# lionl1106/Clip-Neural-image-conpression

Hardware: AMD Instinct MI355X
Metric: images/sec @256px 50-step DDIM, batch=8/GPU (higher is better)
Workload: dtype bf16; 1 GPU; 256px base=128 ch_mult=(1, 2, 2) 50-step DDIM (eta=0), batch=8/GPU, key-seeded synthetic weights (out.* x0.1), synthetic z / x_T; global_batch=8, parallelism=dp1 (independent batches, no collective in the loop), graph=hipGraph, one replay per step, steps_in_flight=1

## Files before the change

clip-neural-image-conpression_amd/csrc/ccn_api.hip:

```cpp
#include "../../include/ccn_hip.h"
#include "ccn_internal.h"
#include "ccn_arch.h"

#include <algorithm>
#include <cmath>
#include <cstdio>
#include <cstdlib>
#include <cstring>
#include <map>
#include <memory>
#include <string>
#include <vector>

using namespace ccn;

namespace {

thread_local std::string g_err;
int fail(int code, const std::string& msg) { g_err = msg; return code; }
#define HIPCHK(expr)                                                                                     \
    do {                                                                                                 \
        hipError_t e_ = (expr);                                                                          \
        if (e_ != hipSuccess)                                                                            \
            return fail(CCN_EHIP, std::string(#expr) + ": " + hipGetErrorString(e_));                    \
    } while (0)

}
extern "C" void ccn_internal_set_error(const char* msg) { g_err = msg ? msg : ""; }
namespace {

inline size_t align_up(size_t v, size_t a) { return (v + a - 1) / a * a; }
inline int ceil_div(int a, int b) { return (a + b - 1) / b; }

uint16_t f2bf_host(float f)
{
    uint32_t u;
    std::memcpy(&u, &f, 4);
    if ((u & 0x7fffffffu) > 0x7f800000u) return (uint16_t)((u >> 16) | 0x40);
    u += 0x7fffu + ((u >> 16) & 1u);
    return (uint16_t)(u >> 16);
}

struct ConvW : ArchConv {
    ConvW() {}
    ConvW(const ArchConv& c) : ArchConv(c) {}
    int Cin_pad = 0, Cout_pad = 0, BN = 0, ntaps_w = 0;
    void* w = nullptr;
    void* wfrag = nullptr;
    float* bias = nullptr;
    bool split = false;
    float inv_scale = 1.f;
    int nphase = 1;
    void* w_ph[7] = {};
    void* wfrag_ph[7] = {};
};
struct NormW { int C = 0; float* gamma = nullptr; float* beta = nullptr; };
struct ResW { NormW n1, n2; };

constexpr size_t kNone = ~(size_t)0;
struct TensorRef {
    std::string name;
    size_t off = kNone;
    int C = 0, H = 0, W = 0;
    size_t part = kNone;
    int n_sp = 0, n_nt = 0, bn = 0;
    bool pr = false;
    int prod = -1;
};

struct StepCtx {
    int step = 0;
    const float* x_in = nullptr;
    float* x_state = nullptr;
    float* eps_out = nullptr;
    int do_ddim = 0;
    float c[4] = {0, 0, 0, 0};
    const float* noise = nullptr;
    float sigma = 0.f;
    float* x0_hist = nullptr;
    float c4 = 0.f;
};

const char* kFamilies[] = {"conv3x3_s1_igemm", "conv3x3_s2_igemm", "convT4x4_s2_igemm", "stem_conv_igemm",
                           "head_conv_ddim", "gn_finalize", "conditioning", "gn_silu_prepass"};
enum { F_C3S1 = 0, F_C3S2, F_CT4, F_STEM, F_HEAD, F_GNF, F_COND, F_LAYOUT, F_COUNT };

enum Op { OP_CONV = 0, OP_HEAD2, OP_GN_FINALIZE, OP_GN_ACT, OP_GN_ACT_FUSED };
struct Launch {
    Op op = OP_CONV; int family = 0; double flops = 0, bytes = 0;
    int conv = -1;
    bool frag = false;
    int film_off = -1;
    ConvArgs a{};
    size_t in = kNone, out = kNone, res = kNone, part = kNone, kpart = kNone, kflag = kNone, gs_part = kNone, gn_ab = kNone,
           fin_ab = kNone, fin_counter = kNone, scratch = kNone;
    int C = 0, HW = 0, G = 0, cpg = 0, n_sp = 0, n_nt = 0, bn = 0;
    double count = 0; const float* gamma = nullptr; const float* beta = nullptr;
};

constexpr int kMaxNorms = 128;

struct RouteRec {
    std::string name;
    int kind = 0;
    const char* kernel = "";
    int th = 0, ksplit = 1, n_nt = 1;
    const char* gn = "none";
    bool film = false, res = false;
    int ops = -1;
};

struct Region { std::string name; size_t off, bytes; };
struct ShapePlan {
    int B = 0, H = 0, W = 0, steps = 0;
    std::vector<Region> regions; size_t total = 0;
    std::vector<std::pair<size_t, size_t>> zero;
    size_t ts_dev = 0, temb = 0, t1 = 0, tp = 0, zp = 0, film = 0, zbuf = 0, xstate = 0;
    int film_stride = 0;
    size_t counters = 0;
    int n_counters = 0, max_counters = 0;
    std::vector<Launch> ops;
    std::map<std::string, TensorRef> named;
    std::vector<RouteRec> routes;
};

struct GraphEntry {
    int steps = 0;
    std::vector<int32_t> ts;
    std::vector<float> coef;
    std::vector<float> sigma;
    const float* noise = nullptr;
    bool guided = false;
    float w = 0.f;
    const float* eps = nullptr;
    std::vector<float> c4;
    const float* hist = nullptr;
    hipGraph_t graph = nullptr;
    hipGraphExec_t exec = nullptr;
    void destroy() { if (exec) (void)hipGraphExecDestroy(exec); if (graph) (void)hipGraphDestroy(graph); }
};

constexpr size_t kMaxGraphsPerBinding = 4;
struct Binding {
    const ShapePlan* plan = nullptr;
    char* ws = nullptr;
    std::vector<int32_t> ts_keep;
    std::vector<GraphEntry> graphs;
    ~Binding() { for (auto& g : graphs) g.destroy(); }
};

}

struct ccn_handle_s {
    ccn_config_t cfg{};
    bool split = false;
    int elem = 4;
    Arch arch;
    std::map<std::string, std::vector<float>> host;
    bool committed = false;
    std::vector<void*> dev_allocs;
    std::vector<ConvW> convs;
    std::vector<ResW> res;
    NormW out_norm;
    float *tp0_w = nullptr, *tp0_b = nullptr, *tp2_w = nullptr, *tp2_b = nullptr, *zp_w = nullptr, *zp_b = nullptr;
    float *film_w = nullptr, *film_b = nullptr;
    float* head_w_f32 = nullptr;
    int G = 8;
    int weight_rounding = CCN_ROUND_DIFFUSED_PHASES;
    int nphase = 1;
    std::vector<std::unique_ptr<ShapePlan>> shape_plans;
    std::vector<std::unique_ptr<Binding>> bindings;
    hipStream_t cap_stream = nullptr;
    unsigned* err_host = nullptr;
    unsigned* err_dev = nullptr;
    bool profiling = false;
    std::vector<hipEvent_t> ev_pool;
    struct Rec { int family; double flops, bytes; int e0, e1; };
    std::vector<Rec> recs;
    size_t ev_used = 0;
    std::vector<std::string> fam_names;
};

namespace {

int upload(ccn_handle_s* h, const void* src, size_t bytes, void** dst)
{
    void* p = nullptr;
    HIPCHK(hipMalloc(&p, bytes ? bytes : 4));
    h->dev_allocs.push_back(p);
    if (bytes) HIPCHK(hipMemcpy(p, src, bytes, hipMemcpyHostToDevice));
    *dst = p;
    return CCN_OK;
}
const std::vector<float>& host_param(const ccn_handle_s* h, int i) { return h->host.at(h->arch.params[i].name); }
int upload_f32(ccn_handle_s* h, int param, float** dst)
{
    const auto& v = host_param(h, param);
    return upload(h, v.data(), v.size() * 4, (void**)dst);
}

float bf16_value(float f)
{
    const uint32_t u = (uint32_t)f2bf_host(f) << 16;
    float r;
    std::memcpy(&r, &u, 4);
    return r;
}

void diffuse_round_conv(float* w, int O, int I, int taps)
{
    for (int o = 0; o < O; ++o) {
        double err = 0.0;
        float* row = w + (size_t)o * I * taps;
        for (size_t k = 0; k < (size_t)I * taps; ++k) {
            const double t = (double)row[k] + err;
            const float r = bf16_value((float)t);
            err = t - (double)r;
            row[k] = r;
        }
    }
}
void diffuse_round_convT(float* w, int I, int O)
{
    static const int kk2[2][2] = {{1, 3}, {0, 2}};
    for (int o = 0; o < O; ++o)
        for (int par = 0; par < 4; ++par) {
            double err = 0.0;
            for (int i = 0; i < I; ++i)
                for (int t = 0; t < 4; ++t) {
                    const int wt = kk2[par >> 1][t >> 1] * 4 + kk2[par & 1][t & 1];
                    float& v = w[((size_t)i * O + o) * 16 + wt];
                    const double tt = (double)v + err;
                    const float r = bf16_value((float)tt);
                    err = tt - (double)r;
                    v = r;
                }
        }
}

int phases_for(const ccn_handle_s* h)
{
    size_t total = 0;
    for (auto& p : h->arch.params) if (p.shape.size() == 4) total += p.numel();
    return total > (size_t)100000000 ? 4 : 8;
}
void round_version(const float* w, size_t n, bool convT, int O, int I, int taps, int k, double* sum, float* out)
{
    for (size_t i = 0; i < n; ++i) out[i] = (float)((double)(k + 1) * (double)w[i] - sum[i]);
    if (convT) diffuse_round_convT(out, I, O); else diffuse_round_conv(out, O, I, taps);
    for (size_t i = 0; i < n; ++i) sum[i] += (double)out[i];
}

}
extern "C" int ccn_internal_round_weights(const float* w, int O, int I, int taps, int convT, int phases, float* out)
{
    if (!w || !out || O <= 0 || I <= 0 || phases < 1 || phases > 8 || (convT && taps != 16)) return 1;
    const size_t n = (size_t)O * I * taps;
    std::vector<double> sum(n, 0.0);
    for (int k = 0; k < phases; ++k) round_version(w, n, convT != 0, O, I, taps, k, sum.data(), out + (size_t)k * n);
    return 0;
}
extern "C" int ccn_internal_split_weights(const float* w, size_t n, float* scale, uint16_t* hi, uint16_t* lo)
{
    if ((!w && n) || !scale || ((!hi || !lo) && n)) return 1;
    float mx = 0.f;
    for (size_t i = 0; i < n; ++i) { const float v = std::fabs(w[i]); if (v > mx) mx = v; }
    int e = 0;
    float s = 1.f;
    if (mx > 0.f && std::isfinite(mx)) { (void)std::frexp(mx, &e); s = std::ldexp(1.f, std::min(14 - e, 126)); }
    *scale = s;
    for (size_t i = 0; i < n; ++i) {
        const float ws = w[i] * s;
        const _Float16 h = (_Float16)ws;
        const _Float16 l = (_Float16)(ws - (float)h);
        std::memcpy(hi + i, &h, 2);
        std::memcpy(lo + i, &l, 2);
    }
    return 0;
}
namespace {

template <typename F>
int pack_and_upload(ccn_handle_s* h, ConvW& cw, int taps, F&& at, void** dw)
{
    cw.BN = conv_bn_for(cw.Cout, cw.kind);
    cw.Cout_pad = (int)align_up(cw.Cout, cw.BN);
    cw.ntaps_w = taps;
    const size_t n = (size_t)taps * cw.Cout_pad * cw.Cin_pad;
    if (h->cfg.dtype == CCN_DTYPE_BF16) {
        std::vector<uint16_t> buf(n, 0);
        for (int t = 0; t < taps; ++t)
            for (int o = 0; o < cw.Cout; ++o)
                for (int i = 0; i < cw.Cin_pad; ++i) buf[((size_t)t * cw.Cout_pad + o) * cw.Cin_pad + i] = f2bf_host(at(t, o, i));
        return upload(h, buf.data(), n * 2, dw);
    }
    std::vector<float> buf(n, 0.f);
    for (int t = 0; t < taps; ++t)
        for (int o = 0; o < cw.Cout; ++o)
            for (int i = 0; i < cw.Cin_pad; ++i) buf[((size_t)t * cw.Cout_pad + o) * cw.Cin_pad + i] = at(t, o, i);
    cw.split = h->split && conv_ws_enabled() && conv_ws_supported(cw.kind, cw.BN);
    cw.inv_scale = 1.f;
    if (cw.split) {
        std::vector<uint16_t> hi(n), lo(n), rows(2 * n);
        float s = 1.f;
        if (ccn_internal_split_weights(buf.data(), n, &s, hi.data(), lo.data())) return fail(CCN_EINVAL, "weight split failed");
        cw.inv_scale = 1.f / s;
        for (size_t i = 0; i < n; ++i) {
            const size_t row = i / 32, c = i % 32;
            rows[row * 64 + c] = hi[i];
            rows[row * 64 + 32 + c] = lo[i];
        }
        return upload(h, rows.data(), n * 4, dw);
    }
    return upload(h, buf.data(), n * 4, dw);
}

int pack_conv3(ccn_handle_s* h, ConvW& cw, const float* w, void** dw, void** dfrag)
{
    const int cke = conv_cin_chunk(h->cfg.dtype);
    cw.Cin_pad = (int)align_up(cw.Cin, cke);
    const int I = cw.Cin;
    int rc = pack_and_upload(h, cw, 9, [&](int t, int o, int i) { return i < I ? w[((size_t)o * I + i) * 9 + t] : 0.f; }, dw);
    if (rc) return rc;
    if (cw.kind == KIND_C3S2 && cw.BN == 128 && h->cfg.dtype == CCN_DTYPE_BF16) {
        const int nch = cw.Cin_pad / cke, n32 = cw.Cout_pad / 32, O = cw.Cout;
        std::vector<uint16_t> fr((size_t)nch * 5 * n32 * 2 * 4 * 64 * 8, 0);
        for (int o = 0; o < O; ++o)
            for (int i = 0; i < I; ++i)
                for (int ps = 0; ps < 10; ++ps) {
                    const int tp = prs2_tap(ps >> 1, ps & 1);
                    if (tp >= 0) fr[prs2_frag_index(ps >> 1, ps & 1, o, i, cw.Cout_pad)] = f2bf_host(w[((size_t)o * I + i) * 9 + tp]);
                }
        return upload(h, fr.data(), fr.size() * 2, dfrag);
    }
    if (cw.kind == KIND_C3S1 && cw.BN == 128 && h->cfg.dtype == CCN_DTYPE_BF16) {
        const int nch = cw.Cin_pad / cke, n32 = cw.Cout_pad / 32, O = cw.Cout;
        std::vector<uint16_t> fr((size_t)nch * n32 * 36 * 64 * 8, 0);
        for (int o = 0; o < O; ++o)
            for (int i = 0; i < I; ++i)
                for (int t = 0; t < 9; ++t) fr[pr3_frag_index(o, i, t, cw.Cout_pad)] = f2bf_host(w[((size_t)o * I + i) * 9 + t]);
        return upload(h, fr.data(), fr.size() * 2, dfrag);
    }
    return CCN_OK;
}
int pack_convT(ccn_handle_s* h, ConvW& cw, const float* w, void** dw, void** dfrag)
{
    const int cke = conv_cin_chunk(h->cfg.dtype);
    cw.Cin_pad = (int)align_up(cw.Cin, cke);
    const int I = cw.Cin, O = cw.Cout;
    int rc = pack_and_upload(h, cw, 16, [&](int t, int o, int i) { return i < I ? w[((size_t)i * O + o) * 16 + t] : 0.f; }, dw);
    if (rc) return rc;
    if (cw.BN == 128 && h->cfg.dtype == CCN_DTYPE_BF16) {
        const int nch = cw.Cin_pad / cke, n32 = cw.Cout_pad / 32;
        std::vector<uint16_t> fr((size_t)4 * nch * n32 * 4 * 4 * 64 * 8, 0);
        for (int o = 0; o < O; ++o)
            for (int i = 0; i < I; ++i)
                for (int pt = 0; pt < 16; ++pt)
                    fr[prct_frag_index(pt >> 2, pt & 3, o, i, cw.Cout_pad, nch)] = f2bf_host(w[((size_t)i * O + o) * 16 + prct_tap(pt >> 2, pt & 3)]);
        return upload(h, fr.data(), fr.size() * 2, dfrag);
    }
    return CCN_OK;
}
int pack_stem(ccn_handle_s* h, ConvW& cw, const float* w, const float* bias, void** dw, void** dfrag)
{
    const int cke = conv_cin_chunk(h->cfg.dtype);
    cw.Cin_pad = cke;
    const int K = cw.Cin * 9;
    int rc = pack_and_upload(h, cw, 1, [&](int, int o, int k) { return k < K ? w[(size_t)o * K + k] : 0.f; }, dw);
    if (rc) return rc;
    if (stem2_supported(h->cfg.dtype, cw.Cin, cw.Cout, h->G)) {
        const int nt = cw.Cout / 32;
        std::vector<uint16_t> fr((size_t)nt * 2 * 64 * 8, 0);
        for (int j = 0; j < nt; ++j)
            for (int s = 0; s < 2; ++s)
                for (int ln = 0; ln < 64; ++ln)
                    for (int e = 0; e < 8; ++e) {
                        const int o = j * 32 + (ln & 31), k = 16 * s + 8 * (ln >> 5) + e;
                        const float v = k < K ? w[(size_t)o * K + k] : (k == K ? bias[o] : 0.f);
                        fr[(((size_t)j * 2 + s) * 64 + ln) * 8 + e] = f2bf_host(v);
                    }
        return upload(h, fr.data(), fr.size() * 2, dfrag);
    }
    return CCN_OK;
}
int pack_conv(ccn_handle_s* h, ConvW& cw, const float* w, const float* bias, void** dw, void** dfrag)
{
    if (cw.kind == KIND_STEM) return pack_stem(h, cw, w, bias, dw, dfrag);
    return cw.kind == KIND_CT4 ? pack_convT(h, cw, w, dw, dfrag) : pack_conv3(h, cw, w, dw, dfrag);
}

struct ConvOpts {
    int film_off = -1;
    const TensorRef* res = nullptr;
    bool want_part = false;
    size_t gn_ab = kNone;
    const NormW* in_norm = nullptr;
    const char* pre_pass = nullptr;
};

struct PlanBuilder {
    ccn_handle_s* h; ShapePlan& pl; const int B;
    size_t off = 0;
    PlanBuilder(ccn_handle_s* h_, ShapePlan& p) : h(h_), pl(p), B(p.B) {}

    size_t take(const std::string& name, size_t bytes)
    {
        pl.regions.push_back({name, align_up(off, 256), bytes});
        off = pl.regions.back().off + bytes;
        return off - bytes;
    }
    TensorRef new_tensor(const std::string& name, int C, int H, int W)
    {
        TensorRef t; t.name = name; t.C = C; t.H = H; t.W = W;
        t.off = take(name, (size_t)B * H * W * C * h->elem);
        return t;
    }
    int groups_for(int C) const { return C < h->G ? C : h->G; }
    void take_counters(int n) { pl.max_counters = n; pl.counters = take("counters", (size_t)n * B * 4); pl.zero.push_back({pl.counters, (size_t)n * B * 4}); }

    ConvRoute route(const ConvW& cw, int Hin, int Win, bool gn_ab, bool res, bool film) const
    {
        static const ConvPolicy policy{true, 128, false, !diag_env("CCN_NO_SPLITK"), diag_env("CCN_SPLITK_S1") != nullptr, true};
        return conv_route({h->cfg.dtype, cw.kind, false, cw.BN, cw.Cin, cw.Cin_pad, cw.Cout, cw.Cout_pad, B, Hin, Win, h->G, cw.wfrag != nullptr,
                           gn_ab, res, film}, policy);
    }

    void conv(int ci, const TensorRef& in, TensorRef& out, const ConvOpts& o)
    {
        const ConvW& cw = h->convs[ci];
        size_t gn_ab = o.gn_ab;
        const ConvRoute r = route(cw, in.H, in.W, gn_ab != kNone, o.res != nullptr, o.film_off >= 0);
        const ConvGeom& g = r.g;
        Launch L;
        static_assert(F_C3S1 == KIND_C3S1 && F_C3S2 == KIND_C3S2 && F_CT4 == KIND_CT4 && F_STEM == KIND_STEM && F_HEAD == KIND_HEAD, "family = kind");
        L.family = cw.kind; L.conv = ci; L.film_off = o.film_off; L.frag = r.uses_frag() && cw.wfrag;
        L.in = in.off; L.out = out.off; L.res = o.res ? o.res->off : kNone;
        ConvArgs& a = L.a;
        r.fill(a);
        a.bias = cw.bias; a.ops = cw.split ? 1 : 0; a.wscale_inv = cw.inv_scale;
        RouteRec rec;
        if (h->split) rec.ops = a.ops;
        rec.name = out.name; rec.kind = cw.kind; rec.th = r.th; rec.ksplit = r.ksplit; rec.n_nt = r.n_nt;
        rec.film = o.film_off >= 0; rec.res = o.res != nullptr;
        rec.gn = gn_ab != kNone ? "prologue" : "none";
        static const bool no_instat = diag_env("CCN_NO_INSTAT") != nullptr;
        if (o.in_norm) {
            const int G_in = groups_for(cw.Cin), cpg_in = cw.Cin / G_in;
            if (r.gs_ok && !no_instat && in.C == cw.Cin && conv_in_kernel_stats(h->cfg.dtype, in.C, G_in, in.n_sp, in.bn)) {
                L.gs_part = in.part; a.gs_gamma = o.in_norm->gamma; a.gs_beta = o.in_norm->beta;
                a.gs_inv_count = 1.0 / ((double)cpg_in * in.H * in.W);
                a.gs_nsp = in.n_sp; a.gs_nnt = in.n_nt; a.gs_bn = in.bn; a.gs_cpg = cpg_in;
                rec.gn = "instat";
            } else { gn_ab = gn(in, *o.in_norm); rec.gn = "prologue"; }
        }
        if (o.pre_pass) rec.gn = o.pre_pass;
        L.gn_ab = gn_ab;
        rec.kernel = conv_kernel_name(conv_kernel_for(cw.kind, cw.BN, a));
        pl.routes.push_back(rec);
        if (r.ksplit == 2) {
            L.kpart = take(out.name + ".kpart", (size_t)B * g.Hout * g.Wout * cw.Cout * h->elem);
            const size_t fbytes = (size_t)B * r.fin_blocks * 4 * sizeof(unsigned);
            L.kflag = take(out.name + ".kflag", fbytes);
            pl.zero.push_back({L.kflag, fbytes});
        }
        a.film_bstride = pl.film_stride; a.err = h->err_dev;
        if (o.want_part) {
            out.part = take(out.name + ".part", (size_t)B * a.G * a.nslot * sizeof(float2));
            out.n_sp = r.part_nsp; out.n_nt = r.part_nnt; out.bn = r.part_bn;
            if (r.pr || r.stem2) out.pr = true;
            out.prod = (int)pl.ops.size();
        }
        L.part = out.part;
        const double macs = (double)B * g.Hout * g.Wout * cw.Cout * (double)(cw.kind == KIND_CT4 ? 4 : 9) * cw.Cin;
        L.flops = 2.0 * macs;
        L.bytes = ((double)B * in.H * in.W * cw.Cin + (double)B * g.Hout * g.Wout * cw.Cout + (o.res ? (double)B * g.Hout * g.Wout * cw.Cout : 0.0)
                   + (double)(cw.kind == KIND_CT4 ? 16 : 9) * cw.Cin * cw.Cout) * h->elem;
        if (cw.kind == KIND_STEM) L.bytes = (double)B * in.H * in.W * cw.Cin * 4 + ((double)B * g.Hout * g.Wout * cw.Cout + 9.0 * cw.Cin * cw.Cout) * h->elem;
        if (cw.kind == KIND_HEAD) L.bytes = ((double)B * in.H * in.W * cw.Cin + 9.0 * cw.Cin * cw.Cout) * h->elem + 3.0 * (double)B * g.Hout * g.Wout * cw.Cout * 4;
        pl.ops.push_back(L);
    }
    Launch norm_launch(Op op, int family, double bytes, const TensorRef& t, const NormW& n) const
    {
        Launch L;
        L.op = op; L.family = family; L.bytes = bytes;
        L.C = t.C; L.HW = t.H * t.W; L.G = groups_for(t.C); L.cpg = t.C / L.G; L.count = (double)L.cpg * t.H * t.W;
        L.in = t.off; L.part = t.part; L.n_sp = t.n_sp; L.n_nt = t.n_nt; L.bn = t.bn; L.gamma = n.gamma; L.beta = n.beta;
        return L;
    }

    size_t gn(const TensorRef& t, const NormW& n)
    {
        const size_t ab = take(t.name + ".ab", (size_t)B * t.C * sizeof(float2));
        Launch L = norm_launch(OP_GN_FINALIZE, F_GNF, (double)B * groups_for(t.C) * t.n_sp * t.n_nt * 8.0 + (double)B * t.C * 8.0, t, n);
        static const bool fuse = diag_env("CCN_FUSED_FINALIZE") != nullptr;
        if (fuse && t.prod >= 0 && !t.pr && pl.n_counters < pl.max_counters) {
            Launch& p = pl.ops[t.prod];
            p.fin_counter = pl.counters + (size_t)pl.n_counters * B * sizeof(unsigned);
            pl.n_counters++;
            p.a.fin_gamma = n.gamma; p.a.fin_beta = n.beta; p.fin_ab = ab; p.a.fin_count = L.count;
            return ab;
        }
        L.gn_ab = ab;
        pl.ops.push_back(L);
        return ab;
    }

    TensorRef preact(const TensorRef& t, const NormW& n, size_t ab)
    {
        TensorRef o = new_tensor(t.name + ".act", t.C, t.H, t.W);
        Launch L = norm_launch(ab == kNone ? OP_GN_ACT_FUSED : OP_GN_ACT, F_LAYOUT, 2.0 * B * t.H * t.W * (double)t.C * h->elem, t, n);
        L.out = o.off; L.gn_ab = ab;
        pl.ops.push_back(L);
        return o;
    }

    TensorRef resblock(int ri, const TensorRef& x, bool out_feeds_gn, int film_off)
    {
        const ArchRes& r = h->arch.res[ri];
        const ConvW& c1 = h->convs[r.c1];
        const NormW &n1 = h->res[ri].n1, &n2 = h->res[ri].n2;
        static const bool preact_pr = diag_env("CCN_PREACT_PR") != nullptr;
        const bool pre = conv_wants_preact(c1.kind, c1.BN, c1.Cout_pad / c1.BN) && r.C / (h->elem == 2 ? 8 : 4) <= 256 &&
                         (preact_pr || c1.Cout_pad / c1.BN >= 6 || !route(c1, x.H, x.W, false, false, false).pr);
        static const bool fuse_act = !diag_env("CCN_NO_FUSED_GNACT");
        const bool f1 = pre && fuse_act && x.n_sp > 0, f2 = pre && fuse_act;
        ConvOpts o1, o2;
        o1.film_off = film_off; o1.want_part = true; o1.pre_pass = f1 ? "preact_fused" : (pre ? "preact" : nullptr);
        o2.res = &x; o2.want_part = out_feeds_gn; o2.pre_pass = f2 ? "preact_fused" : (pre ? "preact" : nullptr);
        TensorRef y = new_tensor(r.prefix + ".film", r.C, x.H, x.W);
        if (pre) conv(r.c1, preact(x, n1, f1 ? kNone : gn(x, n1)), y, o1);
        else { o1.in_norm = &n1; conv(r.c1, x, y, o1); }
        pl.named[y.name] = y;
        TensorRef o = new_tensor(r.prefix, r.C, x.H, x.W);
        if (pre) conv(r.c2, preact(y, n2, f2 ? kNone : gn(y, n2)), o, o2);
        else { o2.in_norm = &n2; conv(r.c2, y, o, o2); }
        pl.named[o.name] = o;
        return o;
    }
};

int build_plan(ccn_handle_s* h, ShapePlan& pl)
{
    const ccn_config_t& c = h->cfg;
    PlanBuilder pb(h, pl);
    const int B = pl.B, H = pl.H, W = pl.W, S = pl.steps;
    const int TR = B > S ? B : S, FR = S * B > B ? S * B : B;
    pl.film_stride = h->arch.F;
    pl.ts_dev = pb.take("ts", (size_t)S * 4);
    pl.temb = pb.take("temb", (size_t)TR * c.time_dim * 4);
    pl.t1 = pb.take("t1", (size_t)TR * c.time_dim * 4 * 4);
    pl.tp = pb.take("tp", (size_t)TR * c.time_dim * 4);
    pl.zp = pb.take("zp", (size_t)B * c.time_dim * 4);
    pl.film = pb.take("film", (size_t)FR * h->arch.F * 4);
    pl.zbuf = pb.take("z", (size_t)B * c.z_dim * 4);
    pl.xstate = pb.take("x_state", (size_t)B * c.img_ch * H * W * 4);
    pb.take_counters(kMaxNorms);

    TensorRef x, img; img.C = c.img_ch; img.H = H; img.W = W;
    std::vector<TensorRef> skips;
    const std::vector<ArchLayer>& layers = h->arch.layers; const size_t nl = layers.size();
    for (size_t li = 0; li < nl; ++li) {
        const ArchLayer& L = layers[li];
        ConvOpts o;
        o.want_part = li + 1 < nl && (layers[li + 1].type == L_RES || layers[li + 1].type == L_HEAD);
        if (L.type == L_RES) { x = pb.resblock(L.idx, x, o.want_part, h->arch.res[L.idx].film_off); continue; }
        const ConvW& cw = h->convs[L.idx];
        if (L.type == L_HEAD) {
            o.gn_ab = pb.gn(x, h->out_norm); o.want_part = false;
            static const bool no_head2 = diag_env("CCN_NO_HEAD2") != nullptr;
            if (no_head2 || !head2_supported(c.dtype, cw.Cin, cw.Cout, h->G)) {
                TensorRef none; none.name = L.name;
                pb.conv(L.idx, x, none, o);
                continue;
            }
            Launch Lh;
            Lh.op = OP_HEAD2; Lh.family = F_HEAD; Lh.conv = L.idx; Lh.in = x.off; Lh.gn_ab = o.gn_ab;
            ConvArgs& a = Lh.a;
            a.bias = cw.bias; a.B = B; a.Hin = H; a.Win = W; a.Cin = cw.Cin; a.Cout = cw.Cout; a.Hout = H; a.Wout = W;
            Lh.scratch = pb.take(L.name + ".scratch", head2_scratch_bytes(B, x.C));
            const double macs = (double)B * H * W * cw.Cout * 9.0 * cw.Cin;
            Lh.flops = 2.0 * macs;
            Lh.bytes = ((double)B * H * W * x.C + 9.0 * x.C * cw.Cout) * h->elem + 3.0 * (double)B * H * W * cw.Cout * 4;
            pl.ops.push_back(Lh);
            RouteRec rec;
            rec.name = L.name; rec.kind = KIND_HEAD; rec.kernel = "head2"; rec.th = 8; rec.gn = "weights";
            if (h->split) rec.ops = 0;
            pl.routes.push_back(rec);
            continue;
        }
        TensorRef sk;
        if (L.type == L_DOWN) skips.push_back(x);
        if (L.type == L_UP) { sk = skips.back(); skips.pop_back(); o.res = &sk; }
        const TensorRef& in = L.type == L_STEM ? img : x;
        const int up = L.type == L_UP ? 2 : 1, down = L.type == L_DOWN ? 2 : 1;
        TensorRef out = pb.new_tensor(L.name, cw.Cout, in.H * up / down, in.W * up / down);
        if (o.res && (sk.C != cw.Cout || sk.H != out.H || sk.W != out.W)) return fail(CCN_EINVAL, "skip shape mismatch");
        pb.conv(L.idx, in, out, o);
        pl.named[L.name] = x = out;
    }
    pl.total = align_up(pb.off, 256);
    return CCN_OK;
}

hipError_t launch(const ccn_handle_s* h, const ShapePlan& pl, const Launch& L, char* ws, hipStream_t s, const StepCtx& c)
{
    auto at = [ws](size_t o) -> char* { return o == kNone ? nullptr : ws + o; };
    const int dtype = h->cfg.dtype;
    switch (L.op) {
        case OP_GN_FINALIZE:
            return launch_gn_finalize((const float2*)at(L.part), pl.B, L.G, L.n_sp, L.n_nt, L.bn, L.cpg, L.C, L.count, L.gamma, L.beta, 1e-5f,
                                      (float2*)at(L.gn_ab), s);
        case OP_GN_ACT: return launch_gn_act(dtype, at(L.in), (const float2*)at(L.gn_ab), at(L.out), pl.B, L.HW, L.C, s);
        case OP_GN_ACT_FUSED:
            return launch_gn_act_fused(dtype, at(L.in), at(L.out), pl.B, L.HW, L.C, (const float2*)at(L.part), L.G, L.n_sp, L.n_nt, L.bn, L.cpg,
                                       L.count, L.gamma, L.beta, 1e-5f, s);
        default: break;
    }
    const ConvW& cw = h->convs[L.conv];
    ConvArgs k = L.a;
    k.in = cw.kind == KIND_STEM ? (const void*)c.x_in : at(L.in);
    if (cw.kind == KIND_HEAD) {
        k.x_state = c.x_state; k.eps_out = c.eps_out; k.do_ddim = c.do_ddim;
        k.c0 = c.c[0]; k.c1 = c.c[1]; k.c2 = c.c[2]; k.c3 = c.c[3]; k.noise = c.noise; k.sigma = c.sigma;
        k.x0_hist = c.x0_hist; k.c4 = c.c4;
    }
    if (L.op == OP_HEAD2) return launch_head2(k, (const float2*)at(L.gn_ab), h->head_w_f32, at(L.scratch), c.step, s);
    const int v = c.step % cw.nphase;
    k.w = v ? cw.w_ph[v - 1] : cw.w;
    k.wfrag = !L.frag ? nullptr : (v ? cw.wfrag_ph[v - 1] : cw.wfrag);
    k.out = at(L.out); k.res = at(L.res); k.part = (float2*)at(L.part); k.gn_ab = (const float2*)at(L.gn_ab);
    k.gs_part = (const float2*)at(L.gs_part); k.kpart = at(L.kpart); k.kflag = (unsigned*)at(L.kflag);
    k.fin_ab = (float2*)at(L.fin_ab); k.fin_counter = (unsigned*)at(L.fin_counter);
    if (L.film_off >= 0) k.film = (const float*)at(pl.film) + (size_t)c.step * pl.B * k.film_bstride + L.film_off;
    return launch_conv(dtype, cw.kind, cw.BN, k, s);
}

int check_shape(const ccn_handle_s* h, int B, int H, int W, int steps)
{
    if (B <= 0 || H <= 0 || W <= 0 || steps <= 0) return fail(CCN_EINVAL, "B, H, W, steps must be positive");
    const int div = 1 << h->cfg.n_mult;
    if (H % div || W % div) return fail(CCN_EINVAL, "H and W must be divisible by 2^len(ch_mult)");
    return CCN_OK;
}

void drop_bindings(ccn_handle_s* h, size_t keep_newest)
{
    if (h->bindings.size() <= keep_newest) return;
    (void)hipDeviceSynchronize();
    while (h->bindings.size() > keep_newest) h->bindings.erase(h->bindings.begin());
}

int shape_plan(ccn_handle_s* h, int B, int H, int W, int steps, const ShapePlan** out)
{
    if (int rc = check_shape(h, B, H, W, steps)) return rc;
    for (auto& p : h->shape_plans)
        if (p->B == B && p->H == H && p->W == W && p->steps == steps) { *out = p.get(); return CCN_OK; }
    std::unique_ptr<ShapePlan> p(new ShapePlan);
    p->B = B; p->H = H; p->W = W; p->steps = steps;
    if (int rc = build_plan(h, *p)) return rc;
    if (h->shape_plans.size() >= 64) { drop_bindings(h, 0); h->shape_plans.clear(); }
    *out = p.get();
    h->shape_plans.push_back(std::move(p));
    return CCN_OK;
}

int get_binding(ccn_handle_s* h, int B, int H, int W, int steps, void* ws, size_t ws_bytes, Binding** out)
{
    const ShapePlan* pl = nullptr;
    if (int rc = shape_plan(h, B, H, W, steps, &pl)) return rc;
    if (!ws || ((uintptr_t)ws & 255)) return fail(CCN_EWORKSPACE, "workspace must be non-null and 256-byte aligned");
    if (ws_bytes < pl->total) return fail(CCN_EWORKSPACE, "workspace too small: need " + std::to_string(pl->total));
    for (size_t i = 0; i < h->bindings.size(); ++i) {
        Binding* b = h->bindings[i].get();
        if (b->plan == pl && b->ws == ws) {
            std::rotate(h->bindings.begin() + (long)i, h->bindings.begin() + (long)i + 1, h->bindings.end());
            *out = b;
            return CCN_OK;
        }
    }
    std::unique_ptr<Binding> b(new Binding);
    b->plan = pl; b->ws = (char*)ws;
    for (auto& z : pl->zero) HIPCHK(hipMemset(b->ws + z.first, 0, z.second));
    if (h->bindings.size() >= 8) drop_bindings(h, 7);
    *out = b.get();
    h->bindings.push_back(std::move(b));
    return CCN_OK;
}

}
int ccn_release_workspace(ccn_handle_t h, void* workspace_dev)
{
    if (!h) return fail(CCN_EINVAL, "null handle");
    auto lives_there = [&](const std::unique_ptr<Binding>& b) { return b->ws == workspace_dev; };
    if (std::none_of(h->bindings.begin(), h->bindings.end(), lives_there)) return CCN_OK;
    HIPCHK(hipDeviceSynchronize());
    h->bindings.erase(std::remove_if(h->bindings.begin(), h->bindings.end(), lives_there), h->bindings.end());
    return CCN_OK;
}
namespace {

template <typename F>
int timed(ccn_handle_s* h, int family, double flops, double bytes, hipStream_t s, F&& go)
{
    if (!h->profiling) { HIPCHK(go()); return CCN_OK; }
    for (hipEvent_t e; h->ev_pool.size() < h->ev_used + 2; h->ev_pool.push_back(e)) HIPCHK(hipEventCreate(&e));
    const int e0 = (int)h->ev_used, e1 = e0 + 1;
    h->ev_used += 2;
    HIPCHK(hipEventRecord(h->ev_pool[e0], s));
    HIPCHK(go());
    HIPCHK(hipEventRecord(h->ev_pool[e1], s));
    h->recs.push_back({family, flops, bytes, e0, e1});
    return CCN_OK;
}

int run_ops(ccn_handle_s* h, const Binding* b, hipStream_t s, const StepCtx& c)
{
    for (const Launch& L : b->plan->ops) {
        if (int rc = timed(h, L.family, L.flops, L.bytes, s, [&] { return launch(h, *b->plan, L, b->ws, s, c); })) return rc;
    }
    return CCN_OK;
}

int run_conditioning(ccn_handle_s* h, const Binding* b, hipStream_t s, const int64_t* t_i64, int TR, int FR, int a_div)
{
    const ccn_config_t& c = h->cfg; const ShapePlan& p = *b->plan;
    const int td = c.time_dim, B = p.B, F = h->arch.F;
    auto f32 = [b](size_t off) { return (float*)(b->ws + off); };
    float *temb = f32(p.temb), *t1 = f32(p.t1), *tp = f32(p.tp), *zp = f32(p.zp);
    int rc;
    if ((rc = timed(h, F_COND, 0, 0, s, [&] {
            return t_i64 ? launch_temb_i64(t_i64, temb, TR, td, s) : launch_temb_i32((const int32_t*)(b->ws + p.ts_dev), temb, TR, td, s); }))) return rc;
    if ((rc = timed(h, F_COND, 2.0 * TR * td * 4.0 * td, 0, s, [&] { return launch_linear(temb, nullptr, 1, TR, h->tp0_w, h->tp0_b, t1, TR, td, 4 * td, 1, s); }))) return rc;
    if ((rc = timed(h, F_COND, 2.0 * TR * td * 4.0 * td, 0, s, [&] { return launch_linear(t1, nullptr, 1, TR, h->tp2_w, h->tp2_b, tp, TR, 4 * td, td, 0, s); }))) return rc;
    if ((rc = timed(h, F_COND, 2.0 * B * c.z_dim * td, 0, s, [&] { return launch_linear(f32(p.zbuf), nullptr, 1, B, h->zp_w, h->zp_b, zp, B, c.z_dim, td, 1, s); }))) return rc;
    return timed(h, F_COND, 2.0 * FR * td * (double)F, 0, s, [&] { return launch_linear(tp, zp, a_div, B, h->film_w, h->film_b, f32(p.film), FR, td, F, 0, s); });
}

struct Guide { const float* z_null; float w; float* eps; };
struct MultiStep { const float* c4; float* hist; };

int run_steps(ccn_handle_s* h, const Binding* b, hipStream_t s, int steps, const float* coef, const float* sigma = nullptr, const float* noise = nullptr,
              const Guide* gd = nullptr, const MultiStep* ms = nullptr)
{
    const ShapePlan& p = *b->plan;
    const size_t img = (size_t)(gd ? p.B / 2 : p.B) * h->cfg.img_ch * p.H * p.W;
    float* xstate = (float*)(b->ws + p.xstate);
    for (int i = 0; i < steps; ++i) {
        const bool noisy = sigma && noise && sigma[i] > 0.f;
        StepCtx c;
        c.step = i; c.x_in = xstate;
        if (gd) { c.x_state = nullptr; c.eps_out = gd->eps; c.do_ddim = 0; }
        else {
            c.x_state = xstate; c.eps_out = nullptr; c.do_ddim = 1;
            for (int k = 0; k < 4; ++k) c.c[k] = coef[i * 4 + k];
            if (noisy) { c.noise = noise + (size_t)i * img; c.sigma = sigma[i]; }
            if (ms) { c.x0_hist = ms->hist; c.c4 = ms->c4[i]; }
        }
        if (int rc = run_ops(h, b, s, c)) return rc;
        if (gd && ms) {
            const float* cf = coef + i * 4;
            const float c4 = ms->c4[i];
            if (int rc = timed(h, F_HEAD, 0, (double)img * 4 * (c4 != 0.f ? 7 : 6), s, [&] {
                    return launch_cfg_ms_step(xstate, xstate + img, ms->hist, gd->eps, gd->eps + img, gd->w, cf[0], cf[1], cf[2], cf[3], c4,
                                              (int64_t)img, s); })) return rc;
        } else if (gd) {
            const float* cf = coef + i * 4;
            const float* nz = noisy ? noise + (size_t)i * img : nullptr;
            if (int rc = timed(h, F_HEAD, 0, (double)img * 4 * (nz ? 6 : 5), s, [&] {
                    return launch_cfg_ddim_step(xstate, xstate + img, gd->eps, gd->eps + img, nz, gd->w, cf[0], cf[1], cf[2], cf[3],
                                                noisy ? sigma[i] : 0.f, (int64_t)img, s); })) return rc;
        }
    }
    return CCN_OK;
}

int check_device_errors(ccn_handle_s* h)
{
    if (!h->err_host) return CCN_OK;
    const unsigned e = __atomic_exchange_n(h->err_host, 0u, __ATOMIC_RELAXED);
    if (e & 1u)
        return fail(CCN_EHIP, "device-side hand-off timeout: a split-K partial tile never arrived; the results of the launches enqueued "
                              "since the last successful check are invalid");
    if (e & 2u)
        return fail(CCN_EHIP, "split-K partners ran on different XCDs (the hand-off took the agent-scope path: results are valid, but the "
                              "placement assumption of launch_conv_pr does not hold on this device / partition mode)");
    if (e & 4u)
        return fail(CCN_EHIP, "f16x3: an activation left the fp16 operand range (|x| >= 65520) and was saturated; the results of the "
                              "launches enqueued since the last successful check are not fp32-grade: use dtype fp32 for this model");
    if (e) return fail(CCN_EHIP, "device-side error word " + std::to_string(e));
    return CCN_OK;
}

int copy_report(const std::string& text, char* buf, size_t cap)
{
    if (buf && cap) {
        const size_t n = std::min(text.size(), cap - 1);
        std::memcpy(buf, text.data(), n);
        buf[n] = 0;
    }
    return (int)text.size();
}

std::string routes_text(const ShapePlan& pl)
{
    static const char* kinds[] = {"C3S1", "C3S2", "CT4", "STEM", "HEAD"};
    std::string text;
    for (const RouteRec& r : pl.routes) {
        char line[256];
        std::snprintf(line, sizeof(line), "%s %s %s th=%d ksplit=%d n_nt=%d gn=%s film=%d res=%d", r.name.c_str(), kinds[r.kind], r.kernel,
                      r.th, r.ksplit, r.n_nt, r.gn, r.film ? 1 : 0, r.res ? 1 : 0);
        text += std::string(line) + (r.ops < 0 ? "" : r.ops ? " ops=f16x3" : " ops=f32") + "\n";
    }
    return text;
}

int check_ready(ccn_handle_s* h)
{
    if (!h) return fail(CCN_EINVAL, "null handle");
    if (!h->committed) return fail(CCN_ESTATE, "ccn_commit_params has not succeeded on this handle");
    return check_device_errors(h);
}

}

extern "C" {

const char* ccn_last_error(void) { return g_err.c_str(); }
#ifdef CCN_DIAG
const char* ccn_version(void) { return "ccn_hip 0.3 (gfx950, diagnostics build)"; }
#else
const char* ccn_version(void) { return "ccn_hip 0.3 (gfx950)"; }
#endif

int ccn_create(const ccn_config_t* cfg, ccn_handle_t* out)
{
    if (!cfg || !out) return fail(CCN_EINVAL, "null argument");
    if (cfg->n_mult < 1 || cfg->n_mult > CCN_MAX_MULT) return fail(CCN_EINVAL, "n_mult out of range");
    if (cfg->dtype != CCN_DTYPE_F32 && cfg->dtype != CCN_DTYPE_BF16 && cfg->dtype != CCN_DTYPE_F16X3) return fail(CCN_EINVAL, "unknown dtype");
    if (cfg->base <= 0 || cfg->base % 8) return fail(CCN_EINVAL, "base must be a positive multiple of 8");
    if (cfg->img_ch < 1 || cfg->img_ch * 9 > 32) return fail(CCN_EINVAL, "img_ch must be 1..3");
    if (cfg->time_dim <= 0 || cfg->z_dim <= 0 || cfg->groups <= 0) return fail(CCN_EINVAL, "bad dims");
    int ch = cfg->base;
    for (int i = 0; i < cfg->n_mult; ++i) {
        if (cfg->ch_mult[i] < 1) return fail(CCN_EINVAL, "ch_mult entries must be >= 1");
        if ((long)ch * cfg->ch_mult[i] > (1 << 16)) return fail(CCN_EINVAL, "channel width (running product of ch_mult, models/unet.py:64) above 65536");
        ch *= cfg->ch_mult[i];
    }
    int ndev = 0;
    HIPCHK(hipGetDeviceCount(&ndev));
    if (ndev <= 0) return fail(CCN_EHIP, "no HIP device");
    std::unique_ptr<ccn_handle_s> h(new ccn_handle_s);
    h->cfg = *cfg;
    h->split = cfg->dtype == CCN_DTYPE_F16X3;
    if (h->split) h->cfg.dtype = CCN_DTYPE_F32;
    h->elem = cfg->dtype == CCN_DTYPE_BF16 ? 2 : 4;
    h->G = cfg->groups;
    h->arch = build_arch(h->cfg);
    h->convs.assign(h->arch.convs.begin(), h->arch.convs.end());
    h->res.resize(h->arch.res.size());
    for (auto& r : h->arch.res)
        if (r.C % (r.C < h->G ? r.C : h->G)) return fail(CCN_EINVAL, "channel count not divisible by GroupNorm groups");
    HIPCHK(conv_prepare());
    HIPCHK(hipStreamCreateWithFlags(&h->cap_stream, hipStreamNonBlocking));
    HIPCHK(hipHostMalloc((void**)&h->err_host, 64, hipHostMallocMapped));
    *h->err_host = 0u;
    HIPCHK(hipHostGetDevicePointer((void**)&h->err_dev, h->err_host, 0));
    for (int i = 0; i < F_COUNT; ++i) h->fam_names.push_back(kFamilies[i]);
    *out = h.release();
    return CCN_OK;
}

int ccn_destroy(ccn_handle_t h)
{
    if (!h) return CCN_OK;
    (void)hipDeviceSynchronize();
    h->bindings.clear();
    for (void* p : h->dev_allocs) (void)hipFree(p);
    for (auto e : h->ev_pool) (void)hipEventDestroy(e);
    if (h->cap_stream) (void)hipStreamDestroy(h->cap_stream);
    if (h->err_host) (void)hipHostFree(h->err_host);
    delete h;
    return CCN_OK;
}

int ccn_num_params(ccn_handle_t h, int32_t* n)
{
    if (!h || !n) return fail(CCN_EINVAL, "null argument");
    *n = (int32_t)h->arch.params.size();
    return CCN_OK;
}

int ccn_param_info(ccn_handle_t h, int32_t i, const char** name, int64_t shape[4], int32_t* ndim)
{
    if (!h || !name || !shape || !ndim) return fail(CCN_EINVAL, "null argument");
    if (i < 0 || i >= (int32_t)h->arch.params.size()) return fail(CCN_EINVAL, "parameter index out of range");
    const ArchParam& p = h->arch.params[i];
    *name = p.name.c_str();
    *ndim = (int32_t)p.shape.size();
    for (size_t k = 0; k < 4; ++k) shape[k] = k < p.shape.size() ? p.shape[k] : 1;
    return CCN_OK;
}

int ccn_load_param(ccn_handle_t h, const char* name, const float* data, const int64_t* shape, int32_t ndim)
{
    if (!h || !name || !data || !shape) return fail(CCN_EINVAL, "null argument");
    const ArchParam* pi = nullptr;
    for (auto& p : h->arch.params) if (p.name == name) { pi = &p; break; }
    if (!pi) return fail(CCN_EWEIGHTS, std::string("Unexpected key in state_dict: ") + name);
    if ((size_t)ndim != pi->shape.size()) return fail(CCN_EWEIGHTS, std::string("size mismatch for ") + name);
    for (int k = 0; k < ndim; ++k)
        if (shape[k] != pi->shape[k]) return fail(CCN_EWEIGHTS, std::string("size mismatch for ") + name);
    std::vector<float> buf(pi->numel());
    hipPointerAttribute_t attr;
    const hipError_t pe = hipPointerGetAttributes(&attr, data);
    if (pe == hipSuccess && attr.type == hipMemoryTypeDevice) {
        HIPCHK(hipMemcpy(buf.data(), data, buf.size() * 4, hipMemcpyDeviceToHost));
    } else {
        (void)hipGetLastError();
        std::memcpy(buf.data(), data, buf.size() * 4);
    }
    h->host[name] = std::move(buf);
    h->committed = false;
    return CCN_OK;
}

int ccn_set_weight_rounding(ccn_handle_t h, int32_t mode)
{
    if (!h) return fail(CCN_EINVAL, "null handle");
    if (mode != CCN_ROUND_NEAREST && mode != CCN_ROUND_DIFFUSED && mode != CCN_ROUND_DIFFUSED_PHASES) return fail(CCN_EINVAL, "unknown weight rounding mode");
    h->weight_rounding = mode;
    return CCN_OK;
}

int ccn_commit_params(ccn_handle_t h)
{
    if (!h) return fail(CCN_EINVAL, "null handle");
    const Arch& a = h->arch;
    std::string missing;
    for (auto& p : a.params)
        if (!h->host.count(p.name)) missing += (missing.empty() ? "" : ", ") + p.name;
    if (!missing.empty()) return fail(CCN_EWEIGHTS, "Missing key(s) in state_dict: " + missing);
    drop_bindings(h, 0);
    h->shape_plans.clear();
    for (void* p : h->dev_allocs) (void)hipFree(p);
    h->dev_allocs.clear();
    const ccn_config_t& c = h->cfg;
    int rc;
    const bool diffuse = c.dtype == CCN_DTYPE_BF16 && h->weight_rounding != CCN_ROUND_NEAREST;
    h->nphase = diffuse && h->weight_rounding == CCN_ROUND_DIFFUSED_PHASES ? phases_for(h) : 1;
    for (size_t ci = 0; ci < a.convs.size(); ++ci) {
        ConvW& cw = h->convs[ci] = ConvW(a.convs[ci]);
        const std::vector<float>&w = host_param(h, cw.pw), &b = host_param(h, cw.pb);
        if ((rc = upload_f32(h, cw.pb, &cw.bias))) return rc;
        const bool dif = diffuse && cw.kind != KIND_HEAD;
        cw.nphase = dif ? h->nphase : 1;
        std::vector<double> sum(dif ? w.size() : 0, 0.0);
        std::vector<float> wk(dif ? w.size() : 0);
        for (int k = 0; k < cw.nphase; ++k) {
            if (dif) round_version(w.data(), w.size(), cw.kind == KIND_CT4, cw.Cout, cw.Cin, cw.kind == KIND_CT4 ? 16 : 9, k, sum.data(), wk.data());
            if ((rc = pack_conv(h, cw, dif ? wk.data() : w.data(), b.data(), k ? &cw.w_ph[k - 1] : &cw.w, k ? &cw.wfrag_ph[k - 1] : &cw.wfrag))) return rc;
        }
        if (cw.kind == KIND_HEAD && (rc = upload_f32(h, cw.pw, &h->head_w_f32))) return rc;
    }
    for (size_t ri = 0; ri < a.res.size(); ++ri) {
        const ArchRes& r = a.res[ri];
        ResW& rw = h->res[ri];
        rw.n1.C = rw.n2.C = r.C;
        if ((rc = upload_f32(h, r.n1.pg, &rw.n1.gamma))) return rc;
        if ((rc = upload_f32(h, r.n1.pb, &rw.n1.beta))) return rc;
        if ((rc = upload_f32(h, r.n2.pg, &rw.n2.gamma))) return rc;
        if ((rc = upload_f32(h, r.n2.pb, &rw.n2.beta))) return rc;
    }
    h->out_norm.C = a.out_norm.C;
    if ((rc = upload_f32(h, a.out_norm.pg, &h->out_norm.gamma))) return rc;
    if ((rc = upload_f32(h, a.out_norm.pb, &h->out_norm.beta))) return rc;
    if ((rc = upload_f32(h, a.tp0.pw, &h->tp0_w))) return rc;
    if ((rc = upload_f32(h, a.tp0.pb, &h->tp0_b))) return rc;
    if ((rc = upload_f32(h, a.tp2.pw, &h->tp2_w))) return rc;
    if ((rc = upload_f32(h, a.tp2.pb, &h->tp2_b))) return rc;
    if ((rc = upload_f32(h, a.zp.pw, &h->zp_w))) return rc;
    if ((rc = upload_f32(h, a.zp.pb, &h->zp_b))) return rc;
    std::vector<float> fw((size_t)a.F * c.time_dim), fb((size_t)a.F);
    for (auto& r : a.res) {
        const ArchLin* parts[2] = {&r.fs, &r.fh};
        for (int q = 0; q < 2; ++q) {
            const auto& w = host_param(h, parts[q]->pw);
            const auto& b = host_param(h, parts[q]->pb);
            std::memcpy(&fw[(size_t)(r.film_off + q * r.C) * c.time_dim], w.data(), w.size() * 4);
            std::memcpy(&fb[(size_t)(r.film_off + q * r.C)], b.data(), b.size() * 4);
        }
    }
    if ((rc = upload(h, fw.data(), fw.size() * 4, (void**)&h->film_w))) return rc;
    if ((rc = upload(h, fb.data(), fb.size() * 4, (void**)&h->film_b))) return rc;
    HIPCHK(hipDeviceSynchronize());
    h->host.clear();
    h->committed = true;
    return CCN_OK;
}

int ccn_workspace_bytes(ccn_handle_t h, int32_t B, int32_t H, int32_t W, int32_t steps, size_t* bytes)
{
    int rc = check_ready(h);
    if (rc) return rc;
    if (!bytes) return fail(CCN_EINVAL, "null argument");
    const ShapePlan* pl = nullptr;
    if ((rc = shape_plan(h, B, H, W, steps, &pl))) return rc;
    *bytes = pl->total;
    return CCN_OK;
}

int ccn_forward(ccn_handle_t h, const float* x_dev, const float* z_dev, const int64_t* t_dev, float* eps_dev,
                int32_t B, int32_t H, int32_t W, void* workspace_dev, size_t workspace_bytes, void* stream)
{
    int rc = check_ready(h);
    if (rc) return rc;
    if (!x_dev || !z_dev || !t_dev || !eps_dev) return fail(CCN_EINVAL, "null tensor pointer");
    Binding* b = nullptr;
    if ((rc = get_binding(h, B, H, W, 1, workspace_dev, workspace_bytes, &b))) return rc;
    hipStream_t s = (hipStream_t)stream;
    HIPCHK(hipMemcpyAsync(b->ws + b->plan->zbuf, z_dev, (size_t)B * h->cfg.z_dim * 4, hipMemcpyDeviceToDevice, s));
    if ((rc = run_conditioning(h, b, s, t_dev, B, B, 1))) return rc;
    StepCtx c;
    c.step = 0; c.x_in = x_dev; c.x_state = nullptr; c.eps_out = eps_dev; c.do_ddim = 0;
    return run_ops(h, b, s, c);
}

static int sample_impl(ccn_handle_t h, const float* z_dev, const float* x_T_dev, float* x_out_dev, int32_t B, int32_t H, int32_t W,
                       int32_t steps, const int32_t* ts_host, const float* coef_host, const float* sigma_host, const float* noise_dev,
                       void* workspace_dev, size_t workspace_bytes, void* stream, int32_t use_graph, const Guide* gd = nullptr,
                       const MultiStep* ms = nullptr)
{
    int rc = check_ready(h);
    if (rc) return rc;
    if (!z_dev || !x_T_dev || !x_out_dev || !ts_host || !coef_host) return fail(CCN_EINVAL, "null pointer");
    if (gd && (B <= 0 || B > INT32_MAX / 2)) return fail(CCN_EINVAL, "B, H, W, steps must be positive");
    const int PB = gd ? 2 * B : B;
    Binding* p = nullptr;
    if ((rc = get_binding(h, PB, H, W, steps, workspace_dev, workspace_bytes, &p))) return rc;
    hipStream_t s = (hipStream_t)stream;
    const size_t img_bytes = (size_t)B * h->cfg.img_ch * H * W * 4, z_row = (size_t)h->cfg.z_dim * 4;
    float* xstate = (float*)(p->ws + p->plan->xstate);
    char* zbuf = p->ws + p->plan->zbuf;
    HIPCHK(hipMemcpyAsync(zbuf, z_dev, (size_t)B * z_row, hipMemcpyDeviceToDevice, s));
    if (gd && !gd->z_null) HIPCHK(hipMemsetAsync(zbuf + (size_t)B * z_row, 0, (size_t)B * z_row, s));
    if (gd && gd->z_null) {
        char* zn = zbuf + (size_t)B * z_row;
        HIPCHK(hipMemcpyAsync(zn, gd->z_null, z_row, hipMemcpyDeviceToDevice, s));
        for (int have = 1; have < B; have *= 2)
            HIPCHK(hipMemcpyAsync(zn + (size_t)have * z_row, zn, (size_t)std::min(have, B - have) * z_row, hipMemcpyDeviceToDevice, s));
    }
    if (x_T_dev != xstate) HIPCHK(hipMemcpyAsync(xstate, x_T_dev, img_bytes, hipMemcpyDeviceToDevice, s));
    if (gd) HIPCHK(hipMemcpyAsync((char*)xstate + img_bytes, xstate, img_bytes, hipMemcpyDeviceToDevice, s));

    if (p->ts_keep.size() != (size_t)steps || std::memcmp(p->ts_keep.data(), ts_host, (size_t)steps * 4)) {
        HIPCHK(hipStreamSynchronize(s));
        p->ts_keep.assign(ts_host, ts_host + steps);
        HIPCHK(hipMemcpy(p->ws + p->plan->ts_dev, p->ts_keep.data(), (size_t)steps * 4, hipMemcpyHostToDevice));
    }
    if (use_graph && !h->profiling) {
        GraphEntry* ge = nullptr;
        for (auto& g : p->graphs)
            if (g.steps == steps && !std::memcmp(g.ts.data(), ts_host, (size_t)steps * 4) &&
                !std::memcmp(g.coef.data(), coef_host, (size_t)steps * 16) && g.noise == noise_dev &&
                g.sigma.size() == (sigma_host ? (size_t)steps : 0) &&
                (!sigma_host || !std::memcmp(g.sigma.data(), sigma_host, (size_t)steps * 4)) &&
                g.guided == (gd != nullptr) && (!gd || (g.w == gd->w && g.eps == gd->eps)) &&
                g.hist == (ms ? ms->hist : nullptr) && g.c4.size() == (ms ? (size_t)steps : 0) &&
                (!ms || !std::memcmp(g.c4.data(), ms->c4, (size_t)steps * 4))) { ge = &g; break; }
        if (!ge) {
            GraphEntry g;
            g.steps = steps; g.ts.assign(ts_host, ts_host + steps); g.coef.assign(coef_host, coef_host + steps * 4);
            if (sigma_host) g.sigma.assign(sigma_host, sigma_host + steps);
            g.noise = noise_dev;
            if (gd) { g.guided = true; g.w = gd->w; g.eps = gd->eps; }
            if (ms) { g.c4.assign(ms->c4, ms->c4 + steps); g.hist = ms->hist; }
            HIPCHK(hipStreamBeginCapture(h->cap_stream, hipStreamCaptureModeRelaxed));
            rc = run_conditioning(h, p, h->cap_stream, nullptr, steps, steps * PB, PB);
            if (!rc) rc = run_steps(h, p, h->cap_stream, steps, coef_host, sigma_host, noise_dev, gd, ms);
            hipGraph_t graph = nullptr;
            const hipError_t ce = hipStreamEndCapture(h->cap_stream, &graph);
            if (rc) { if (graph) (void)hipGraphDestroy(graph); return rc; }
            if (ce != hipSuccess) return fail(CCN_EHIP, std::string("hipStreamEndCapture: ") + hipGetErrorString(ce));
            g.graph = graph;
            HIPCHK(hipGraphInstantiate(&g.exec, g.graph, nullptr, nullptr, 0));
            if (p->graphs.size() >= kMaxGraphsPerBinding) {
                HIPCHK(hipDeviceSynchronize());
                p->graphs.front().destroy();
                p->graphs.erase(p->graphs.begin());
            }
            p->graphs.push_back(g);
            ge = &p->graphs.back();
        } else if (ge != &p->graphs.back()) {
            std::rotate(p->graphs.begin() + (ge - p->graphs.data()), p->graphs.begin() + (ge - p->graphs.data()) + 1, p->graphs.end());
            ge = &p->graphs.back();
        }
        HIPCHK(hipGraphLaunch(ge->exec, s));
    } else {
        if ((rc = run_conditioning(h, p, s, nullptr, steps, steps * PB, PB))) return rc;
        if ((rc = run_steps(h, p, s, steps, coef_host, sigma_host, noise_dev, gd, ms))) return rc;
    }
    if (x_out_dev != xstate) HIPCHK(hipMemcpyAsync(x_out_dev, xstate, img_bytes, hipMemcpyDeviceToDevice, s));
    return CCN_OK;
}

int ccn_sample(ccn_handle_t h, const float* z_dev, const float* x_T_dev, float* x_out_dev, int32_t B, int32_t H, int32_t W,
               int32_t steps, const int32_t* ts_host, const float* coef_host, void* workspace_dev, size_t workspace_bytes,
               void* stream, int32_t use_graph)
{
    return sample_impl(h, z_dev, x_T_dev, x_out_dev, B, H, W, steps, ts_host, coef_host, nullptr, nullptr, workspace_dev, workspace_bytes, stream, use_graph);
}

int ccn_sample_eta(ccn_handle_t h, const float* z_dev, const float* x_T_dev, float* x_out_dev, int32_t B, int32_t H, int32_t W,
                   int32_t steps, const int32_t* ts_host, const float* coef_host, const float* sigma_host, const float* noise_dev,
                   void* workspace_dev, size_t workspace_bytes, void* stream, int32_t use_graph)
{
    if (!sigma_host || !noise_dev) return fail(CCN_EINVAL, "null sigma / noise");
    return sample_impl(h, z_dev, x_T_dev, x_out_dev, B, H, W, steps, ts_host, coef_host, sigma_host, noise_dev, workspace_dev, workspace_bytes, stream, use_graph);
}

int ccn_sample_guided(ccn_handle_t h, const float* z_dev, const float* z_null_dev, const float* x_T_dev, float* x_out_dev, int32_t B,
                      int32_t H, int32_t W, int32_t steps, const int32_t* ts_host, const float* coef_host, const float* sigma_host,
                      const float* noise_dev, float w, float* eps_scratch_dev, void* workspace_dev, size_t workspace_bytes, void* stream,
                      int32_t use_graph)
{
    if (!sigma_host != !noise_dev) return fail(CCN_EINVAL, "sigma and noise must be given together");
    if (!std::isfinite(w)) return fail(CCN_EINVAL, "the guidance scale must be finite");
    if (!eps_scratch_dev || ((uintptr_t)eps_scratch_dev & 15)) return fail(CCN_EINVAL, "the eps scratch must be non-null and 16-byte aligned");
    const Guide gd{z_null_dev, w, eps_scratch_dev};
    return sample_impl(h, z_dev, x_T_dev, x_out_dev, B, H, W, steps, ts_host, coef_host, sigma_host, noise_dev, workspace_dev, workspace_bytes, stream,
                       use_graph, &gd);
}

static int split_ms_table(int32_t steps, const float* coef_host, const float* x0_hist_dev, std::vector<float>& coef4, std::vector<float>& c4)
{
    if (!coef_host || steps <= 0) return fail(CCN_EINVAL, "null pointer");
    if (!x0_hist_dev || ((uintptr_t)x0_hist_dev & 15)) return fail(CCN_EINVAL, "the x0 history must be non-null and 16-byte aligned");
    coef4.resize((size_t)steps * 4); c4.resize((size_t)steps);
    for (int i = 0; i < steps; ++i) {
        for (int k = 0; k < 5; ++k)
            if (!std::isfinite(coef_host[i * 5 + k])) return fail(CCN_EINVAL, "non-finite sampler coefficient");
        for (int k = 0; k < 4; ++k) coef4[(size_t)i * 4 + k] = coef_host[i * 5 + k];
        c4[i] = coef_host[i * 5 + 4];
    }
    if (c4[0] != 0.f) return fail(CCN_EINVAL, "c4 must be 0 on step 0: there is no x0 history yet");
    return CCN_OK;
}

int ccn_sample_ms(ccn_handle_t h, const float* z_dev, const float* x_T_dev, float* x_out_dev, int32_t B, int32_t H, int32_t W, int32_t steps,
                  const int32_t* ts_host, const float* coef_host, float* x0_hist_dev, void* workspace_dev, size_t workspace_bytes,
                  void* stream, int32_t use_graph)
{
    std::vector<float> coef4, c4;
    if (int rc = split_ms_table(steps, coef_host, x0_hist_dev, coef4, c4)) return rc;
    const MultiStep ms{c4.data(), x0_hist_dev};
    return sample_impl(h, z_dev, x_T_dev, x_out_dev, B, H, W, steps, ts_host, coef4.data(), nullptr, nullptr, workspace_dev, workspace_bytes, stream,
                       use_graph, nullptr, &ms);
}

int ccn_sample_guided_ms(ccn_handle_t h, const float* z_dev, const float* z_null_dev, const float* x_T_dev, float* x_out_dev, int32_t B,
                         int32_t H, int32_t W, int32_t steps, const int32_t* ts_host, const float* coef_host, float w, float* eps_scratch_dev,
                         float* x0_hist_dev, void* workspace_dev, size_t workspace_bytes, void* stream, int32_t use_graph)
{
    if (!std::isfinite(w)) return fail(CCN_EINVAL, "the guidance scale must be finite");
    if (!eps_scratch_dev || ((uintptr_t)eps_scratch_dev & 15)) return fail(CCN_EINVAL, "the eps scratch must be non-null and 16-byte aligned");
    std::vector<float> coef4, c4;
    if (int rc = split_ms_table(steps, coef_host, x0_hist_dev, coef4, c4)) return rc;
    const Guide gd{z_null_dev, w, eps_scratch_dev};
    const MultiStep ms{c4.data(), x0_hist_dev};
    return sample_impl(h, z_dev, x_T_dev, x_out_dev, B, H, W, steps, ts_host, coef4.data(), nullptr, nullptr, workspace_dev, workspace_bytes, stream,
                       use_graph, &gd, &ms);
}

int ccn_ms_step(float* x_dev, float* x0_hist_dev, const float* eps_dev, float c0, float c1, float c2, float c3, float c4, int64_t n, void* stream)
{
    if (!x_dev || !x0_hist_dev || !eps_dev || n < 0) return fail(CCN_EINVAL, "bad argument");
    if (n == 0) return CCN_OK;
    HIPCHK(launch_ms_step(x_dev, x0_hist_dev, eps_dev, c0, c1, c2, c3, c4, n, (hipStream_t)stream));
    return CCN_OK;
}

int ccn_cfg_ms_step(float* x_dev, float* x_dup_dev, float* x0_hist_dev, const float* eps_c_dev, const float* eps_u_dev, float w,
                    float c0, float c1, float c2, float c3, float c4, int64_t n, void* stream)
{
    if (!x_dev || !x0_hist_dev || !eps_c_dev || !eps_u_dev || n < 0) return fail(CCN_EINVAL, "bad argument");
    if (n == 0) return CCN_OK;
    HIPCHK(launch_cfg_ms_step(x_dev, x_dup_dev, x0_hist_dev, eps_c_dev, eps_u_dev, w, c0, c1, c2, c3, c4, n, (hipStream_t)stream));
    return CCN_OK;
}

int ccn_cfg_ddim_step(float* x_dev, float* x_dup_dev, const float* eps_c_dev, const float* eps_u_dev, const float* noise_dev, float w,
                      float c0, float c1, float c2, float c3, float sigma, int64_t n, void* stream)
{
    if (!x_dev || !eps_c_dev || !eps_u_dev || n < 0) return fail(CCN_EINVAL, "bad argument");
    if (n == 0) return CCN_OK;
    HIPCHK(launch_cfg_ddim_step(x_dev, x_dup_dev, eps_c_dev, eps_u_dev, noise_dev, w, c0, c1, c2, c3, sigma, n, (hipStream_t)stream));
    return CCN_OK;
}

int ccn_ddim_step(float* x_dev, const float* eps_dev, const float* noise_dev, float c0, float c1, float c2, float c3,
                  float sigma, int64_t n, void* stream)
{
    if (!x_dev || !eps_dev || n < 0) return fail(CCN_EINVAL, "bad argument");
    if (n == 0) return CCN_OK;
    HIPCHK(launch_ddim_step(x_dev, eps_dev, noise_dev, c0, c1, c2, c3, sigma, n, (hipStream_t)stream));
    return CCN_OK;
}

int ccn_q_sample(float* out_dev, const float* x0_dev, const float* noise_dev, const float* a_dev, const float* s_dev,
                 int32_t B, int64_t per_sample, void* stream)
{
    if (!out_dev || !x0_dev || !noise_dev || !a_dev || !s_dev || B <= 0 || per_sample <= 0) return fail(CCN_EINVAL, "bad argument");
    HIPCHK(launch_q_sample(out_dev, x0_dev, noise_dev, a_dev, s_dev, B, per_sample, (hipStream_t)stream));
    return CCN_OK;
}

int ccn_predict_x0(float* out_dev, const float* x_t_dev, const float* eps_dev, const float* a_dev, const float* s_dev,
                   int32_t B, int64_t per_sample, void* stream)
{
    if (!out_dev || !x_t_dev || !eps_dev || !a_dev || !s_dev || B <= 0 || per_sample <= 0) return fail(CCN_EINVAL, "bad argument");
    HIPCHK(launch_predict_x0(out_dev, x_t_dev, eps_dev, a_dev, s_dev, B, per_sample, (hipStream_t)stream));
    return CCN_OK;
}

int ccn_timestep_embedding(const int64_t* t_dev, float* out_dev, int32_t n, int32_t dim, void* stream)
{
    if (!t_dev || !out_dev || n <= 0 || dim <= 0) return fail(CCN_EINVAL, "bad argument");
    HIPCHK(launch_temb_i64(t_dev, out_dev, n, dim, (hipStream_t)stream));
    return CCN_OK;
}

int ccn_film_forward(const float* x_dev, const float* h_dev, const float* ws_dev, const float* bs_dev, const float* wh_dev,
                     const float* bh_dev, float* y_dev, int32_t B, int32_t C, int32_t H, int32_t W, int32_t D,
                     float* scratch_dev, void* stream)
{
    if (!x_dev || !h_dev || !ws_dev || !bs_dev || !wh_dev || !bh_dev || !y_dev || !scratch_dev) return fail(CCN_EINVAL, "null pointer");
    if (B <= 0 || C <= 0 || H <= 0 || W <= 0 || D <= 0) return fail(CCN_EINVAL, "bad shape");
    hipStream_t s = (hipStream_t)stream;
    float* sc = scratch_dev; float* sh = scratch_dev + (size_t)B * C;
    HIPCHK(launch_linear(h_dev, nullptr, 1, B, ws_dev, bs_dev, sc, B, D, C, 0, s));
    HIPCHK(launch_linear(h_dev, nullptr, 1, B, wh_dev, bh_dev, sh, B, D, C, 0, s));
    HIPCHK(launch_film_nchw(x_dev, sc, sh, y_dev, B, C, (int64_t)H * W, s));
    return CCN_OK;
}

int ccn_resblock_forward(ccn_handle_t h, const char* prefix, const float* x_dev, const float* cond_dev, float* y_dev,
                         int32_t B, int32_t H, int32_t W, void* workspace_dev, size_t workspace_bytes, void* stream)
{
    int rc = check_ready(h);
    if (rc) return rc;
    if (!prefix || !x_dev || !cond_dev || !y_dev || !workspace_dev) return fail(CCN_EINVAL, "null pointer");
    if (B <= 0 || H <= 0 || W <= 0) return fail(CCN_EINVAL, "bad shape");
    const ArchRes* r = nullptr;
    for (auto& q : h->arch.res) if (q.prefix == prefix) { r = &q; break; }
    if (!r) return fail(CCN_EINVAL, std::string("no ResBlock with prefix ") + prefix);
    if ((uintptr_t)workspace_dev & 255) return fail(CCN_EWORKSPACE, "workspace must be 256-byte aligned");
    hipStream_t s = (hipStream_t)stream;
    const int G = (r->C < h->G ? r->C : h->G), cpg = r->C / G;
    int nslot = (H * W + 1023) / 1024; if (nslot < 1) nslot = 1;
    ShapePlan pl; pl.B = B; pl.H = H; pl.W = W; pl.steps = 1;
    PlanBuilder pb(h, pl);
    pl.film_stride = 2 * r->C;
    pl.film = pb.take("film", (size_t)B * 2 * r->C * 4);
    pb.take_counters(8);
    TensorRef x = pb.new_tensor("x", r->C, H, W);
    x.part = pb.take("x.part", (size_t)B * G * nslot * sizeof(float2));
    x.n_sp = nslot; x.n_nt = 1; x.bn = 1 << 30;
    const TensorRef o = pb.resblock((int)(r - h->arch.res.data()), x, false, 0);
    if (pb.off > workspace_bytes) return fail(CCN_EWORKSPACE, "workspace too small: need " + std::to_string(pb.off));
    char* ws = (char*)workspace_dev;
    for (auto& z : pl.zero) HIPCHK(hipMemsetAsync(ws + z.first, 0, z.second, s));
    HIPCHK(launch_nchw_to_nhwc(h->cfg.dtype, x_dev, ws + x.off, B, r->C, H, W, s));
    HIPCHK(launch_gn_partials(h->cfg.dtype, ws + x.off, (float2*)(ws + x.part), B, H * W, r->C, cpg, G, nslot, s));
    HIPCHK(launch_linear(cond_dev, nullptr, 1, B, h->film_w + (size_t)r->film_off * h->cfg.time_dim, h->film_b + r->film_off,
                         (float*)(ws + pl.film), B, h->cfg.time_dim, 2 * r->C, 0, s));
    StepCtx c;
    for (const Launch& L : pl.ops) HIPCHK(launch(h, pl, L, ws, s, c));
    HIPCHK(launch_nhwc_to_nchw(h->cfg.dtype, ws + o.off, y_dev, B, r->C, H, W, s));
    return CCN_OK;
}

int ccn_read_activation(ccn_handle_t h, const char* name, float* out_dev, size_t out_elems, void* stream)
{
    int rc = check_ready(h);
    if (rc) return rc;
    if (!name || !out_dev) return fail(CCN_EINVAL, "null pointer");
    if (h->bindings.empty()) return fail(CCN_ESTATE, "no forward has run yet");
    const Binding* b = h->bindings.back().get();
    auto it = b->plan->named.find(name);
    if (it == b->plan->named.end()) return fail(CCN_EINVAL, std::string("unknown activation ") + name);
    const TensorRef& t = it->second;
    if (out_elems < (size_t)b->plan->B * t.C * t.H * t.W) return fail(CCN_EINVAL, "output buffer too small");
    hipStream_t s = (hipStream_t)stream;
    HIPCHK(launch_nhwc_to_nchw(h->cfg.dtype, b->ws + t.off, out_dev, b->plan->B, t.C, t.H, t.W, s));
    HIPCHK(hipStreamSynchronize(s));
    return CCN_OK;
}

extern "C" int ccn_internal_plan_routes(ccn_handle_t h, char* buf, size_t cap)
{
    if (!h || h->bindings.empty()) return -1;
    return copy_report(routes_text(*h->bindings.back()->plan), buf, cap);
}
extern "C" int ccn_internal_plan_routes_of(ccn_handle_t h, int32_t B, int32_t H, int32_t W, int32_t steps, char* buf, size_t cap)
{
    const ShapePlan* pl;
    if (!h || !h->committed || shape_plan(h, B, H, W, steps, &pl)) return -1;
    return copy_report(routes_text(*pl), buf, cap);
}
extern "C" int ccn_internal_plan_layout(ccn_handle_t h, int32_t B, int32_t H, int32_t W, int32_t steps, char* buf, size_t cap)
{
    const ShapePlan* pl;
    if (!h || !h->committed || shape_plan(h, B, H, W, steps, &pl)) return -1;
    std::string text;
    for (const Region& r : pl->regions) text += r.name + " off=" + std::to_string(r.off) + " bytes=" + std::to_string(r.bytes) + "\n";
    text += "total=" + std::to_string(pl->total) + "\n";
    return copy_report(text, buf, cap);
}

int ccn_poll_errors(ccn_handle_t h)
{
    if (!h) return fail(CCN_EINVAL, "null handle");
    return check_device_errors(h);
}

int ccn_profile_enable(ccn_handle_t h, int32_t on)
{
    if (!h) return fail(CCN_EINVAL, "null handle");
    h->profiling = on != 0;
    h->recs.clear();
    h->ev_used = 0;
    return CCN_OK;
}

int ccn_profile_read(ccn_handle_t h, const char** names, float* ms, int32_t* calls, double* flops, double* bytes,
                     int32_t cap, int32_t* n)
{
    if (!h || !names || !ms || !calls || !flops || !bytes || !n) return fail(CCN_EINVAL, "null pointer");
    HIPCHK(hipDeviceSynchronize());
    std::vector<double> t(F_COUNT, 0.0), fl(F_COUNT, 0.0), by(F_COUNT, 0.0);
    std::vector<int> cnt(F_COUNT, 0);
    for (auto& r : h->recs) {
        float e = 0.f;
        HIPCHK(hipEventElapsedTime(&e, h->ev_pool[r.e0], h->ev_pool[r.e1]));
        t[r.family] += e; fl[r.family] += r.flops; by[r.family] += r.bytes; cnt[r.family]++;
    }
    int k = 0;
    for (int f = 0; f < F_COUNT && k < cap; ++f) {
        if (!cnt[f]) continue;
        names[k] = h->fam_names[f].c_str(); ms[k] = (float)t[f]; calls[k] = cnt[f]; flops[k] = fl[f]; bytes[k] = by[f];
        ++k;
    }
    *n = k;
    h->recs.clear();
    h->ev_used = 0;
    return CCN_OK;
}

int ccn_algorithmic_work(ccn_handle_t h, int32_t B, int32_t H, int32_t W, double* flops, double* bytes)
{
    int rc = check_ready(h);
    if (rc) return rc;
    if (!flops || !bytes) return fail(CCN_EINVAL, "null pointer");
    const ShapePlan* pl = nullptr;
    if ((rc = shape_plan(h, B, H, W, 1, &pl))) return rc;
    double f = 0, b = 0;
    for (auto& L : pl->ops) if (L.family <= F_HEAD) { f += L.flops; b += L.bytes; }
    const ccn_config_t& c = h->cfg;
    f += 2.0 * B * ((double)c.time_dim * 4 * c.time_dim * 2 + (double)c.z_dim * c.time_dim + (double)c.time_dim * h->arch.F);
    *flops = f; *bytes = b;
    return CCN_OK;
}

}
```

clip-neural-image-conpression_amd/csrc/ccn_conv_pr.hip:

```cpp
#include "ccn_device.h"
#include <cstdio>
#include <cstdlib>
#include <cstring>
#include <vector>
#include <algorithm>

namespace ccn {

namespace {

#define CCN_FDIV(x, m, d) ((m) ? (int)__umulhi((unsigned)(x), (m)) : (int)(x))

template <int TH_> struct PrLdsT {
    static constexpr int HROWS = TH_ + 2, HPITCH = 34;
    static constexpr int A_BYTES = HROWS * HPITCH * 128;
    static constexpr int SP = 272;
    static constexpr int STG_BYTES = TH_ * 32 * SP;
    static constexpr int CHS_BYTES = 4 * 128 * 2 * 4;
    static constexpr int TOTAL = 2 * A_BYTES + STG_BYTES + CHS_BYTES;
};
typedef PrLdsT<8> PrLds;
static_assert(PrLds::TOTAL <= 160 * 1024, "LDS budget");

}

template <int NTAPS, int D, int MODE, int TH = 8, int GS = 0, bool P4 = false>
__global__ __launch_bounds__(512) void conv_pr_kernel(const ConvArgs a, const int grid_tiles)
{
    static_assert(TH == 8 || (TH == 4 && NTAPS == 9), "4-row tiles: 3x3 stride-1 form only");
    static_assert(!P4 || (NTAPS == 4 && MODE != 2), "plane passes of 2x2 taps: the 4-tap consumers, no split-K");
    constexpr bool RES = MODE == 1;
    constexpr bool RR = MODE != 0;
    typedef __bf16 T;
    constexpr int MF = 4, NF = 2;
    constexpr int BN = 128;
    constexpr int HROWS = TH + 2;
    constexpr int OSC = (NTAPS == 4 && !P4) ? 2 : 1, NPARC = (NTAPS == 4 && !P4) ? 4 : 1;
    constexpr int EPC = 8, CKE = 64;
    constexpr int NSTEP = NTAPS * 4;
    constexpr bool S2 = NTAPS == 2;
    constexpr int NPASS = S2 ? 5 : (P4 ? 4 : 1);
    constexpr int IS = (S2 || P4) ? 2 : 1;
    static_assert(NSTEP % D == 0, "the register ring must wrap at the chunk boundary");
    using L = PrLdsT<TH>;
    constexpr int HPITCH = L::HPITCH;
    extern __shared__ __attribute__((aligned(16))) unsigned char smem[];
    unsigned char* const stg = smem + 2 * L::A_BYTES;

    const int tid = threadIdx.x, lane = tid & 63, wave = tid >> 6;
    const int r = lane & 31, h = lane >> 5;

    const int grid = (int)gridDim.x;
    const int vb = (grid & 7) == 0 ? ((int)blockIdx.x & 7) * (grid >> 3) + ((int)blockIdx.x >> 3) : (int)blockIdx.x;
    const int ntiles = grid_tiles;
    const int my_tiles = (ntiles - vb + grid - 1) / grid;
    auto vt = [&](int ti) __attribute__((always_inline)) { return vb + ti * grid; };
    const int ks = (MODE == 2 && a.ksplit == 2) ? 2 : 1;
    const unsigned xcc_id = MODE == 2 ? (unsigned)__builtin_amdgcn_s_getreg((3 << 11) | 20) : 0u;
    const int nck = a.nchunk / ks;
    const int ktotal = my_tiles * nck;
    auto vt_tile = [&](int v) __attribute__((always_inline)) { return ks == 2 ? (v >> 1) : v; };
    auto vt_kh = [&](int v) __attribute__((always_inline)) { return ks == 2 ? (v & 1) : 0; };

    const unsigned char* const inb = (const unsigned char*)a.in;
    constexpr bool gstat = GS == 1;
    static_assert(GS != 1 || (NTAPS == 9 && MODE != 2), "in-kernel statistics: 3x3 stride-1 layers without split-K");
    const bool gn = NTAPS == 9 && GS != 2 && !CCN_DBG_BIT(a, 32);
    constexpr unsigned OOB = 0x7FFFFFF0u;
    auto raw_barrier = [&]() __attribute__((always_inline)) {
        asm volatile("s_waitcnt lgkmcnt(0)" ::: "memory");
        __builtin_amdgcn_s_barrier();
        asm volatile("" ::: "memory");
    };
    auto stamp = [&](int slot) __attribute__((always_inline)) {
        if (CCN_STAMPS_PTR(a) && lane == 0 && (wave == 0 || wave == 4))
            CCN_STAMPS_PTR(a)[((size_t)blockIdx.x * 2 + (wave == 0 ? 0 : 1)) * 8 + slot] = __builtin_amdgcn_s_memrealtime();
    };
    [[maybe_unused]] unsigned long long t_bar = 0, t_a = 0, t_b = 0, t_w = 0, t_r = 0;
    const unsigned long long t_begin = CCN_STAMPS_PTR(a) ? __builtin_amdgcn_s_memtime() : 0;
    auto timed_barrier = [&]() __attribute__((always_inline)) {
        if (CCN_STAMPS_PTR(a)) { const unsigned long long t0 = __builtin_amdgcn_s_memtime(); raw_barrier(); t_bar += __builtin_amdgcn_s_memtime() - t0; }
        else raw_barrier();
    };
    auto stamp_cycles = [&]() __attribute__((always_inline)) {
        if (CCN_STAMPS_PTR(a) && lane == 0 && (wave == 0 || wave == 4)) {
            unsigned long long* st = CCN_STAMPS_PTR(a) + ((size_t)blockIdx.x * 2 + (wave == 0 ? 0 : 1)) * 8;
            st[3] = t_bar; st[4] = __builtin_amdgcn_s_memtime() - t_begin; st[5] = t_a; st[6] = t_b; st[7] = t_r;
        }
    };
    stamp(0);

    const int etid = tid & 255, ew = wave & 3;
    const int o16 = etid & 15, pr = etid >> 4;
    unsigned char* const outb = (unsigned char*)a.out;
    const unsigned char* const resb = (const unsigned char*)a.res;
    const unsigned out_bytes = (unsigned)((size_t)a.B * a.Hout * a.Wout * a.Cout * sizeof(T));
    float* const chs = (float*)(stg + L::STG_BYTES) + ew * 256;
    constexpr int NQ = TH / 2;
    u32x4 rr[RR ? 2 : 1][4];
    f32x4 fb[2], fs[RES ? 1 : 2], ft[RES ? 1 : 2];
    int e_b = 0, e_ty = 0, e_tx = 0, e_nt = 0, e_par = 0, e_kh = 0, e_tile = 0;
    bool pd_on = false;
    int pd_b = 0, pd_slot = 0, pd_n0 = 0;
    unsigned char* const kpartb = (unsigned char*)a.kpart;
    unsigned e_base = 0;
    int e_rows = 0;
    unsigned e_m0 = OOB, e_m1 = OOB;
    auto item_off = [&](unsigned eb, int it) __attribute__((always_inline)) -> unsigned {
        const unsigned rmask = (it >> 1) < e_rows ? 0u : OOB;
        return (eb + (unsigned)(it >> 1) * (unsigned)(OSC * a.Wout * a.Cout * (int)sizeof(T)) + (unsigned)((it & 1) * 16) * (unsigned)(OSC * a.Cout * (int)sizeof(T)))
               | ((it & 1) ? e_m1 : e_m0) | rmask;
    };
    auto epi_setup = [&](int v) __attribute__((always_inline)) {
        const int tile = vt_tile(v);
        e_kh = vt_kh(v); e_tile = tile;
        const int t2 = CCN_FDIV(tile, a.fd_nt, a.n_nt);
        e_nt = tile - t2 * a.n_nt;
        e_par = t2 % NPARC;
        const int sp = t2 / NPARC;
        {
            const int row = CCN_FDIV(sp, a.fd_tx, a.n_tx);
            e_tx = sp - row * a.n_tx;
            e_b = CCN_FDIV(sp, a.fd_sp, a.n_tx * a.n_ty);
            e_ty = row - e_b * a.n_ty;
        }
        const int nb = e_nt * BN + o16 * 8;
        const bool nvalid = nb < a.Cout;
        e_base = (unsigned)(((e_b * a.Hout + e_ty * TH * OSC + (e_par >> 1)) * a.Wout + (e_tx * 32 + pr) * OSC + (e_par & 1)) * a.Cout + nb) * (unsigned)sizeof(T);
        e_rows = a.MH - e_ty * TH;
        e_m0 = (nvalid && e_tx * 32 + pr < a.MW) ? 0u : OOB;
        e_m1 = (nvalid && e_tx * 32 + pr + 16 < a.MW) ? 0u : OOB;
    };
    auto res_on = [&]() __attribute__((always_inline)) -> bool { return RES || (MODE == 2 && ks == 2 && e_kh == 1); };
    auto res_batch = [&](int q, u32x4* dst) __attribute__((always_inline)) {
        if constexpr (RR) {
            if (res_on()) {
                const auto srd = __builtin_amdgcn_make_buffer_rsrc((void*)((ks == 2 && e_kh == 1) ? kpartb : (resb ? resb : outb)), 0, out_bytes, 0x00020000);
                unsigned eb = e_base; asm volatile("" : "+v"(eb));
                if (ks == 2 && e_kh == 1) {
#pragma unroll
                    for (int i = 0; i < 4; ++i) dst[i] = __builtin_amdgcn_raw_buffer_load_b128(srd, item_off(eb, q * 4 + i), 0, 1);
                } else {
#pragma unroll
                    for (int i = 0; i < 4; ++i) {
                        if (!CCN_DBG_BIT(a, 16384)) dst[i] = __builtin_amdgcn_raw_buffer_load_b128(srd, item_off(eb, q * 4 + i), 0, 2);
                        else dst[i] = __builtin_amdgcn_raw_buffer_load_b128(srd, item_off(eb, q * 4 + i), 0, 0);
                    }
                }
            }
        }
    };
    auto epi_request = [&](int q0, int q1) __attribute__((always_inline)) {
        if (ks == 2 && e_kh == 1) {
            unsigned* const fl = a.kflag + (size_t)e_tile * 4 + ew;
            unsigned seen = 0u;
            if (lane == 0) {
                int spins = 0;
                while ((seen = __hip_atomic_load(fl, __ATOMIC_RELAXED, __HIP_MEMORY_SCOPE_AGENT)) == 0u && ++spins < (1 << 22)) __builtin_amdgcn_s_sleep(2);
                if (spins >= (1 << 22) && a.err) __hip_atomic_fetch_or(a.err, 1u, __ATOMIC_RELAXED, __HIP_MEMORY_SCOPE_SYSTEM);
                __hip_atomic_store(fl, 0u, __ATOMIC_RELAXED, __HIP_MEMORY_SCOPE_AGENT);
            }
            seen = (unsigned)__builtin_amdgcn_readfirstlane((int)seen);
            if (seen != 0u && seen != xcc_id + 1u) {
                __builtin_amdgcn_fence(__ATOMIC_ACQUIRE, "agent");
                if (lane == 0 && a.err) __hip_atomic_fetch_or(a.err, 2u, __ATOMIC_RELAXED, __HIP_MEMORY_SCOPE_SYSTEM);
            }
            asm volatile("" ::: "memory");
        }
        const int nb = e_nt * BN + o16 * 8;
        const int nbs = nb < a.Cout ? nb : 0;
        fb[0] = *(const f32x4*)(a.bias + nbs); fb[1] = *(const f32x4*)(a.bias + nbs + 4);
        if constexpr (!RES) {
            if (a.film) {
                const float* fp = a.film + (size_t)e_b * a.film_bstride;
                fs[0] = *(const f32x4*)(fp + nbs); fs[1] = *(const f32x4*)(fp + nbs + 4);
                ft[0] = *(const f32x4*)(fp + a.Cout + nbs); ft[1] = *(const f32x4*)(fp + a.Cout + nbs + 4);
            }
        }
        res_batch(q0, rr[q0 & 1]);
        if constexpr (RR) { if (q0 + 1 < q1) res_batch(q0 + 1, rr[(q0 + 1) & 1]); }
    };
    auto epilogue = [&](int q0, int q1) __attribute__((always_inline)) {
        const bool first = ks == 2 && e_kh == 0, second = ks == 2 && e_kh == 1;
        float f1[RES ? 1 : 8], f2[8];
#pragma unroll
        for (int e = 0; e < 8; ++e) {
            f2[e] = second ? 0.f : fb[e >> 2][e & 3];
            if constexpr (!RES) {
                f1[e] = 1.f;
                if (a.film) { f1[e] = 1.0f + fs[e >> 2][e & 3]; f2[e] = second ? 0.f : fmaf(f2[e], f1[e], ft[e >> 2][e & 3]); }
            }
        }
        const auto osrd_c = __builtin_amdgcn_make_buffer_rsrc((void*)(first ? kpartb : outb), 0, out_bytes, 0x00020000);
        const bool radd = res_on();
        float s1[8], s2[8];
#pragma unroll
        for (int e = 0; e < 8; ++e) { s1[e] = 0.f; s2[e] = 0.f; }
#pragma unroll
        for (int q = 0; q < NQ; ++q) {
            if (q < q0 || q >= q1) continue;
            unsigned eb = e_base; asm volatile("" : "+v"(eb));
            int sbase = pr * L::SP + o16 * 16; asm volatile("" : "+v"(sbase));
#pragma unroll
            for (int i = 0; i < 4; ++i) {
                const int it = q * 4 + i;
                const unsigned off = item_off(eb, it);
                const u32x4 sv = *(const u32x4*)(stg + sbase + ((it >> 1) * 32 + (it & 1) * 16) * L::SP);
                const bool live = off < OOB;
                float x[8];
                Vec16<T>::unpack(sv, x);
                if constexpr (RES) {
                    float rv[8];
                    Vec16<T>::unpack(rr[q & 1][i], rv);
#pragma unroll
                    for (int e = 0; e < 8; ++e) x[e] = (x[e] + f2[e]) + rv[e];
                } else {
#pragma unroll
                    for (int e = 0; e < 8; ++e) x[e] = fmaf(x[e], f1[e], f2[e]);
                    if constexpr (MODE == 2) {
                        if (radd) {
                            float rv[8];
                            Vec16<T>::unpack(rr[q & 1][i], rv);
#pragma unroll
                            for (int e = 0; e < 8; ++e) x[e] += rv[e];
                        }
                    }
                }
                __builtin_amdgcn_raw_buffer_store_b128(Vec16<T>::pack(x), osrd_c, off, 0, 0);
                if (live) {
#pragma unroll
                    for (int e = 0; e < 8; ++e) { s1[e] += x[e]; s2[e] = fmaf(x[e], x[e], s2[e]); }
                }
                asm volatile("" : "+v"(s1[0]), "+v"(s1[1]), "+v"(s1[2]), "+v"(s1[3]), "+v"(s1[4]), "+v"(s1[5]), "+v"(s1[6]), "+v"(s1[7]));
                asm volatile("" : "+v"(s2[0]), "+v"(s2[1]), "+v"(s2[2]), "+v"(s2[3]), "+v"(s2[4]), "+v"(s2[5]), "+v"(s2[6]), "+v"(s2[7]));
                __builtin_amdgcn_sched_barrier(0);
            }
            if constexpr (RR) { if (q + 2 < q1) res_batch(q + 2, rr[q & 1]); }
        }
        if (first) {
            asm volatile("s_waitcnt vmcnt(0)" ::: "memory");
            if (lane == 0) __hip_atomic_store(a.kflag + (size_t)e_tile * 4 + ew, xcc_id + 1u, __ATOMIC_RELAXED, __HIP_MEMORY_SCOPE_AGENT);
        }
        if (a.part && !first) {
#pragma unroll
            for (int s = 16; s < 64; s <<= 1)
#pragma unroll
                for (int e = 0; e < 8; ++e) { s1[e] += __shfl_xor(s1[e], s); s2[e] += __shfl_xor(s2[e], s); }
            if (lane < 16) {
#pragma unroll
                for (int e = 0; e < 8; ++e) { chs[(lane * 8 + e) * 2] = s1[e]; chs[(lane * 8 + e) * 2 + 1] = s2[e]; }
            }
            pd_on = true; pd_b = e_b; pd_n0 = e_nt * BN;
            pd_slot = ((e_ty * a.n_tx + e_tx) * NPARC + e_par) * a.n_nt + e_nt;
        }
    };
    auto combine = [&]() __attribute__((always_inline)) {
        if (!pd_on) return;
        pd_on = false;
        const float* const all = (const float*)(stg + L::STG_BYTES);
        const int n0 = pd_n0;
        if (n0 >= a.Cout) return;
        const int nend = min(n0 + BN, a.Cout);
        const int g1 = CCN_FDIV(nend - 1, a.fd_cpg, a.cpg);
        for (int g = CCN_FDIV(n0, a.fd_cpg, a.cpg) + ew; g <= g1; g += 4) {
            const int clo = max(g * a.cpg, n0), chi = min((g + 1) * a.cpg, nend);
            float t1 = 0.f, t2 = 0.f;
            const float* const wa = all + (lane >> 4) * 256;
            for (int c = clo + (lane & 15); c < chi; c += 16) {
                t1 += wa[(c - n0) * 2]; t2 += wa[(c - n0) * 2 + 1];
            }
#pragma unroll
            for (int m = 32; m >= 1; m >>= 1) { t1 += __shfl_xor(t1, m); t2 += __shfl_xor(t2, m); }
            if (lane == 0) part_store(a.part + (size_t)(pd_b * a.G + g) * a.nslot + pd_slot, t1, t2);
        }
    };

    const int ptid = tid & 255;
    const int ck = ptid & 7, pcol = ptid >> 3;
    const int xrow = pcol >> 1, xcol = 32 + (pcol & 1);
    const bool xthr = ptid < HROWS * 16;
    constexpr int AIT = HROWS + 1;
    u32x4 areg[AIT];
    GnCoef<T> gk;
    unsigned rowm = 0;
    bool colv = false, xv = false;
    int rq_ti = 0, rq_c = 0;
    GnCoef<T> gkn;
    int q_b = 0, q_iy0 = 0, q_ix0 = 0, q_c = 0;
    bool q_tv = false;
    float st_mean = 0.f, st_rstd = 1.f, qn_mean = 0.f, qn_rstd = 1.f;
    int st_b = -1;
    f32x4 qn_g[2], qn_bt[2];
    unsigned svmask = 0u;
    float2 sv[8];
    auto stats_issue = [&](int b) __attribute__((always_inline)) {
        const int g = lane >> 3, sub = lane & 7;
        const int cpg = a.gs_cpg, pnt = a.gs_nnt, nsp = a.gs_nsp;
        const int jlo = CCN_FDIV(g * cpg, a.fd_gsbn, a.gs_bn), jhi = CCN_FDIV((g + 1) * cpg - 1, a.fd_gsbn, a.gs_bn), nj = jhi - jlo + 1;
        const float2* const base = a.gs_part + (size_t)(b * 8 + g) * ((size_t)nsp * pnt) + jlo;
        int off[8];
        svmask = 0u;
#pragma unroll
        for (int u = 0; u < 8; ++u) {
            const int e = sub + 8 * u;
            const int jj = CCN_FDIV(e, a.fd_gsnsp, nsp), sp = e - jj * nsp;
            const bool ok = jj < nj;
            off[u] = ok ? sp * pnt + jj : 0;
            svmask |= ok ? (1u << u) : 0u;
        }
#pragma unroll
        for (int u = 0; u < 8; ++u) sv[u] = base[off[u]];
    };
    auto stats_reduce = [&]() __attribute__((always_inline)) {
        double s1 = 0.0, s2 = 0.0;
#pragma unroll
        for (int u = 0; u < 8; ++u) { const bool ok = (svmask >> u) & 1u; s1 += ok ? (double)sv[u].x : 0.0; s2 += ok ? (double)sv[u].y : 0.0; }
#pragma unroll
        for (int m = 1; m < 8; m <<= 1) { s1 += __shfl_xor(s1, m); s2 += __shfl_xor(s2, m); }
        const double mean = s1 * a.gs_inv_count;
        double var = s2 * a.gs_inv_count - mean * mean;
        if (var < 0.0) var = 0.0;
        st_mean = (float)mean;
        st_rstd = __builtin_amdgcn_rsqf((float)(var + 1e-5));
    };
    int q_cbs = 0; bool q_cv = false, q_cv_i = false;
    auto decode = [&]() __attribute__((always_inline)) -> bool {
        const int v = vt(rq_ti);
        if (rq_c == 0) {
            q_tv = rq_ti < my_tiles;
            const int tile = vt_tile(q_tv ? v : vt(0));
            const int sp = CCN_FDIV(tile, a.fd_ntp, a.n_nt * NPARC);
            const int row = CCN_FDIV(sp, a.fd_tx, a.n_tx);
            const int tx = sp - row * a.n_tx;
            q_b = CCN_FDIV(sp, a.fd_sp, a.n_tx * a.n_ty);
            const int ty = row - q_b * a.n_ty;
            q_iy0 = ty * TH - 1; q_ix0 = tx * 32 - 1;
        }
        q_c = vt_kh(v) * nck + rq_c;
        const int cb = (q_c / NPASS) * CKE + ck * EPC;
        q_cv = q_tv && cb < a.Cin;
        q_cbs = q_cv ? cb : 0;
        const bool fresh = gstat && rq_c == 0 && q_tv && q_b != st_b;
        if (++rq_c == nck) { rq_c = 0; ++rq_ti; }
        return fresh;
    };
    auto coef_loads = [&]() __attribute__((always_inline)) {
        if (gstat) {
            qn_g[0] = *(const f32x4*)(a.gs_gamma + q_cbs); qn_g[1] = *(const f32x4*)(a.gs_gamma + q_cbs + 4);
            qn_bt[0] = *(const f32x4*)(a.gs_beta + q_cbs); qn_bt[1] = *(const f32x4*)(a.gs_beta + q_cbs + 4);
        } else gkn.load(a.gn_ab + (size_t)q_b * a.Cin + q_cbs, gn && q_cv);
    };
    auto coef_sel = [&]() __attribute__((always_inline)) {
        if (gstat) {
            const int src = CCN_FDIV(q_cbs, a.fd_gscpg, a.gs_cpg) * 8;
            qn_mean = __shfl(st_mean, src); qn_rstd = __shfl(st_rstd, src);
        }
    };
    auto prep = [&]() __attribute__((always_inline)) {
        const bool fresh = decode();
        coef_loads();
        if (fresh) { stats_issue(q_b); stats_reduce(); st_b = q_b; }
        coef_sel();
    };
    auto adopt = [&]() __attribute__((always_inline)) {
        if (gstat) gk.from_raw(qn_g, qn_bt, qn_mean, qn_rstd, gn && q_cv_i);
        else gk = gkn;
    };
    auto issue_loads = [&](int r0 = 0, int r1 = TH + 2, bool with_x = true) __attribute__((always_inline)) {
        const int b = __builtin_amdgcn_readfirstlane(q_b), iy0 = __builtin_amdgcn_readfirstlane(q_iy0), ix0 = __builtin_amdgcn_readfirstlane(q_ix0);
        const int cc = __builtin_amdgcn_readfirstlane(q_c / NPASS);
        const int pass = q_c - cc * NPASS;
        const int py = S2 ? (pass <= 2 ? 1 : 0) : (P4 ? (pass < 2 ? 1 : 0) : 0);
        const int px = S2 ? ((pass <= 1 || pass == 3) ? 1 : 0) : (P4 ? ((pass & 1) ? 0 : 1) : 0);
        const int cb = cc * CKE + ck * EPC;
        const bool cv = q_tv && cb < a.Cin;
        q_cv_i = cv;
        const unsigned img_bytes = (unsigned)(a.Hin * a.Win * a.Cin) * (unsigned)sizeof(T);
        const unsigned coff = (unsigned)(((q_tv && cc * CKE < a.Cin) ? cc : 0) * CKE) * (unsigned)sizeof(T);
        const auto srd = __builtin_amdgcn_make_buffer_rsrc((void*)(inb + (size_t)b * img_bytes + coff), 0, img_bytes - coff, 0x00020000);
        const int rs = IS * a.Win * a.Cin * (int)sizeof(T);
        const int ixr = IS * (ix0 + pcol) + px;
        colv = cv && ixr >= 0 && ixr < a.Win;
        const unsigned cmask = colv ? 0u : OOB;
        const int base = ((IS * iy0 + py) * a.Win + ixr) * a.Cin * (int)sizeof(T) + ck * 16;
        const int first = IS * iy0 + py;
        const int r_lo = first < 0 ? (-first + IS - 1) / IS : 0;
        int r_hi = (a.Hin - first + IS - 1) / IS; r_hi = r_hi > HROWS ? HROWS : (r_hi < 0 ? 0 : r_hi);
        rowm = q_tv ? (((1u << r_hi) - 1u) & ~((1u << r_lo) - 1u)) : 0u;
#pragma unroll
        for (int i = 0; i < HROWS; ++i) {
            if (i < r0 || i >= r1) continue;
            areg[i] = __builtin_amdgcn_raw_buffer_load_b128(srd, (unsigned)(base + i * rs) | cmask, 0, 0);
        }
        {
            const int iyr = IS * (iy0 + xrow) + py, ixx = IS * (ix0 + xcol) + px;
            xv = xthr && cv && iyr >= 0 && iyr < a.Hin && ixx >= 0 && ixx < a.Win;
            const int off = (iyr * a.Win + ixx) * a.Cin * (int)sizeof(T) + ck * 16;
            if (with_x) areg[HROWS] = __builtin_amdgcn_raw_buffer_load_b128(srd, (unsigned)off | (xv ? 0u : OOB), 0, 0);
        }
    };
    auto issue = [&]() __attribute__((always_inline)) { issue_loads(); adopt(); };
    auto request = [&]() __attribute__((always_inline)) { prep(); issue(); };
    auto request_first = [&](int r0, int r1, bool with_x) __attribute__((always_inline)) {
        const bool fresh = decode();
        if (fresh) stats_issue(q_b);
        coef_loads();
        issue_loads(r0, r1, with_x);
        if (fresh) { stats_reduce(); st_b = q_b; }
        coef_sel();
        adopt();
    };
    auto dump = [&](int buf, int r0 = 0, int r1 = TH + 2, bool with_x = true) __attribute__((always_inline)) {
        unsigned char* const As = smem + buf * L::A_BYTES;
        int pc = pcol; asm volatile("" : "+v"(pc));
#pragma unroll
        for (int i = 0; i < AIT; ++i) {
            if (i < HROWS ? (i < r0 || i >= r1) : !with_x) continue;
            const int px = i < HROWS ? i * HPITCH + pc : (pc >> 1) * HPITCH + 32 + (pc & 1);
            const int sw = i < HROWS ? (NTAPS == 9 ? (pc >> 1) & 3 : (pc >> 1)) : 0;
            u32x4 v = areg[i];
            const bool ok = i < HROWS ? (((rowm >> i) & 1u) && colv) : xv;
            if (gn) {
                const u32x4 tr = gk.template apply<true>(v);
                v = u32x4{0u, 0u, 0u, 0u};
                if (ok) v = tr;
            }
            if (i < HROWS || xthr) *(u32x4*)(As + px * 128 + (((ck ^ sw) & 7) << 4)) = v;
            if ((i & 1) == 1) __builtin_amdgcn_sched_barrier(0);
        }
    };

    constexpr int HSPLIT = HROWS / 2;

    if (wave >= 4) {
        if (a.prod_first) __builtin_amdgcn_s_setprio(3);
        if (CCN_DBG_BIT(a, 128)) __builtin_amdgcn_s_setprio(1);
        if (CCN_DBG_BIT(a, 256)) __builtin_amdgcn_s_setprio(3);
        request_first(0, HSPLIT, true);
        dump(0, 0, HSPLIT, true);
        request();
        raw_barrier();
        stamp(1);
        int c = 0, ti = 0;
        for (int k = 0; k < ktotal; ++k) {
            unsigned long long t0 = CCN_STAMPS_PTR(a) ? __builtin_amdgcn_s_memtime() : 0;
            if (CCN_STAMPS_PTR(a)) {
                asm volatile("s_waitcnt vmcnt(0)" ::: "memory");
                const unsigned long long t1 = __builtin_amdgcn_s_memtime(); t_w += t1 - t0; t0 = t1;
            }
            if (k + 1 < ktotal) { prep(); dump((k + 1) & 1); }
            if (CCN_STAMPS_PTR(a)) { const unsigned long long t1 = __builtin_amdgcn_s_memtime(); t_a += t1 - t0; t0 = t1; }
            const bool epi = c == 0 && ti > 0;
            if (epi) epi_request(0, NQ);
            if (k + 1 < ktotal) issue();
            if (c == nck - 1) epi_setup(vt(ti));
            if (CCN_STAMPS_PTR(a)) { const unsigned long long t1 = __builtin_amdgcn_s_memtime(); t_r += t1 - t0; t0 = t1; }
            if (epi) epilogue(0, NQ);
            if (CCN_STAMPS_PTR(a)) t_b += __builtin_amdgcn_s_memtime() - t0;
            const bool early = k + 1 == ktotal && !(ks == 2 && e_kh == 1);
            if (early) epi_request(0, NQ);
            timed_barrier();
            combine();
            if (++c == nck) { c = 0; ++ti; }
        }
        if (ks == 2 && e_kh == 1) epi_request(0, NQ);
        epilogue(0, NQ);
        if (pd_on) {
            raw_barrier();
            combine();
        }
        stamp(2); stamp_cycles();
        return;
    }

    if (!CCN_DBG_BIT(a, 16)) __builtin_amdgcn_s_setprio(2);
    if constexpr (NTAPS == 9) {
        constexpr int NROW = HROWS, NSG = 2 * NROW;
        constexpr int NG = 6;
        constexpr int WIN = 6, PF = 4;
        static_assert((NG * NSG) % WIN == 0, "static window indexing");
        f32x16 acc[TH];
        const int n32 = a.Cout_pad / 32;
        constexpr unsigned COLB = 36 * 1024;
        const unsigned wtotal = (unsigned)((size_t)a.nchunk * n32 * COLB);
        const auto wsrd = __builtin_amdgcn_make_buffer_rsrc((void*)a.wfrag, 0, wtotal, 0x00020000);
        const unsigned lane16 = (unsigned)lane * 16u;
        auto wbase_of = [&](int tile, int chunk) __attribute__((always_inline)) -> unsigned {
            const int nt = tile - CCN_FDIV(tile, a.fd_nt, a.n_nt) * a.n_nt;
            return (unsigned)__builtin_amdgcn_readfirstlane((int)((unsigned)(chunk * n32 + nt * 4 + wave) * COLB));
        };
        const int px16 = lane & 15, g4 = lane >> 4;
        int b16x[3];
#pragma unroll
        for (int d = 0; d < 3; ++d) { const int hx = px16 + d; b16x[d] = hx * 128 + ((((g4 & 1) << 2) | ((g4 >> 1) ^ ((hx >> 1) & 3))) << 4); }
        u32x4 bq[2][3][2];
        {
            const unsigned wb = wbase_of(vt_tile(vt(0)), vt_kh(vt(0)) * nck);
#pragma unroll
            for (int f = 0; f < 6; ++f) bq[0][f >> 1][f & 1] = __builtin_amdgcn_raw_buffer_load_b128(wsrd, lane16, wb + f * 1024, 0);
        }
        const int stg_lane = px16 * L::SP + (wave * 32 + 4 * g4) * 2;
        if constexpr (HSPLIT < HROWS) {
            request_first(HSPLIT, HROWS, false);
            if (CCN_STAMPS_PTR(a)) {
                const unsigned long long r0 = CCN_STAMPS_PTR(a)[((size_t)blockIdx.x * 2) * 8];
                t_a = __builtin_amdgcn_s_memrealtime() - r0;
                asm volatile("s_waitcnt vmcnt(0)" ::: "memory");
                t_b = __builtin_amdgcn_s_memrealtime() - r0;
            }
            dump(0, HSPLIT, HROWS, false);
            if (CCN_STAMPS_PTR(a)) t_r = __builtin_amdgcn_s_memrealtime() - CCN_STAMPS_PTR(a)[((size_t)blockIdx.x * 2) * 8];
        }
        raw_barrier();
        stamp(1);
        int k = 0;
        const bool idle_w = ks == 1 && grid % a.n_nt == 0 &&
                            (vt_tile(vt(0)) - CCN_FDIV(vt_tile(vt(0)), a.fd_nt, a.n_nt) * a.n_nt) * BN + wave * 32 >= a.Cout;
        if (idle_w) { for (int kk = 0; kk < ktotal; ++kk) timed_barrier(); }
        else
        for (int ti = 0; ti < my_tiles; ++ti) {
            const int v = vt(ti), v_next = ti + 1 < my_tiles ? vt(ti + 1) : v;
            const int tile = vt_tile(v), c0 = vt_kh(v) * nck;
#pragma unroll
            for (int i = 0; i < TH; ++i)
#pragma unroll
                for (int q = 0; q < 16; ++q) acc[i][q] = 0.0f;
            for (int chunk = 0; chunk < nck; ++chunk, ++k) {
                const unsigned wb_cur = wbase_of(tile, c0 + chunk);
                const unsigned wb_nxt = chunk + 1 < nck ? wbase_of(tile, c0 + chunk + 1) : wbase_of(vt_tile(v_next), vt_kh(v_next) * nck);
                int bufoff = (k & 1) * L::A_BYTES; asm volatile("" : "+v"(bufoff));
                u32x4 rw[WIN];
                int ag = 0;
                auto rload = [&](int s_) __attribute__((always_inline)) {
                    const int g = s_ / NSG, hp = s_ % NSG;
                    if (hp == 0) ag = (bufoff + b16x[g >> 1]) ^ ((g & 1) << 5);
                    rw[s_ % WIN] = *(const u32x4*)(smem + ag + ((hp >> 1) * HPITCH + (hp & 1) * 16) * 128);
                };
                if (!CCN_DBG_BIT(a, 64)) {
#pragma unroll
                for (int s_ = 0; s_ < PF; ++s_) rload(s_);
#pragma unroll
                for (int s_ = 0; s_ < NG * NSG; ++s_) {
                    const int g = s_ / NSG, hh = (s_ % NSG) >> 1, p = s_ & 1;
                    __builtin_amdgcn_sched_barrier(0);
                    const bool wl = TH == 8 ? (p == 0 && hh >= 2 && hh <= 7) : (hh >= 1 && hh <= 3);
                    if (wl) {
                        const int f = TH == 8 ? hh - 2 : (hh - 1) * 2 + p;
                        const unsigned off = g + 1 < NG ? wb_cur + (unsigned)((g + 1) * 6 + f) * 1024u : wb_nxt + (unsigned)f * 1024u;
                        bq[(g + 1) & 1][f >> 1][f & 1] = __builtin_amdgcn_raw_buffer_load_b128(wsrd, lane16, off, 0);
                    }
                    if (s_ + PF < NG * NSG) rload(s_ + PF);
                    int nm = 0;
#pragma unroll
                    for (int q6 = 0; q6 < 6; ++q6) {
                        const int o = (s_ & 1) ? 5 - q6 : q6;
                        const int dy = o >> 1, c = o & 1;
                        const int i = hh - dy;
                        if (i >= 0 && i < TH) { mfma16q(acc[i], p * 2 + c, bq[g & 1][dy][c], rw[s_ % WIN]); ++nm; }
                    }
#pragma unroll
                    for (int m = 0; m < 6; ++m) {
                        if (m < nm) __builtin_amdgcn_sched_group_barrier(0x008, 1, 0);
                        if (m == 0) __builtin_amdgcn_sched_group_barrier(0x100, 1, 0);
                        if (m == 2 && wl) __builtin_amdgcn_sched_group_barrier(0x020, 1, 0);
                        if (m & 1) __builtin_amdgcn_sched_group_barrier(0x002, 1, 0);
                    }
                    __builtin_amdgcn_sched_barrier(0);
                }
                }
                if (chunk + 1 == nck) {
#pragma unroll
                    for (int i = 0; i < TH; ++i)
#pragma unroll
                        for (int q = 0; q < 4; ++q) {
                            const f32x16& c = acc[i];
                            typedef unsigned u32x2 __attribute__((ext_vector_type(2)));
                            const u32x2 pk = {pack_bf2(c[q * 4], c[q * 4 + 1]), pack_bf2(c[q * 4 + 2], c[q * 4 + 3])};
                            *(u32x2*)(stg + stg_lane + (i * 32 + (q >> 1) * 16) * L::SP + ((q & 1) * 16) * 2) = pk;
                        }
                }
                timed_barrier();
            }
        }
        __builtin_amdgcn_s_setprio(0);
        stamp(2); stamp_cycles();
    } else {
    static_assert(TH == 8, "the 4x2 fragment form works on 8-row tiles");
    const int wm = wave >> 1, wn = wave & 1;
    f32x16 acc[MF][NF];
    auto rbase = [&](int row_lin, int hx) __attribute__((always_inline)) { return row_lin * 128 + (((hx >> 1) & 6) << 4) + (((h ^ (hx >> 1)) & 1) << 4); };
    int prow[MF];
#pragma unroll
    for (int i = 0; i < MF; ++i) prow[i] = ((wm * MF + i) + 1) * HPITCH + r + 1;
    const int n32 = a.Cout_pad / 32;
    constexpr unsigned COLB = NSTEP * 1024;
    const unsigned wtotal = (unsigned)((size_t)NPARC * a.nchunk * n32 * COLB);
    const auto wsrd = __builtin_amdgcn_make_buffer_rsrc((void*)a.wfrag, 0, wtotal, 0x00020000);
    const unsigned lane16 = (unsigned)lane * 16u;
    auto wbase_of = [&](int tile, int chunk) __attribute__((always_inline)) -> unsigned {
        const int t2 = CCN_FDIV(tile, a.fd_nt, a.n_nt);
        const int nt = tile - t2 * a.n_nt, par = t2 % NPARC;
        return (unsigned)__builtin_amdgcn_readfirstlane((int)((unsigned)((par * a.nchunk + chunk) * n32 + nt * 4 + wn * NF) * COLB));
    };
    u32x4 bq[D][NF];
    {
        const unsigned wb = wbase_of(vt_tile(vt(0)), vt_kh(vt(0)) * nck);
#pragma unroll
        for (int s = 0; s < D - 1; ++s)
#pragma unroll
            for (int jn = 0; jn < NF; ++jn) bq[s][jn] = __builtin_amdgcn_raw_buffer_load_b128(wsrd, lane16, wb + s * 1024 + jn * COLB, 0);
    }
    const int stg_lane = (wm * 4 * 32 + r) * L::SP + (wn * 64 + 4 * h) * 2;

    if constexpr (HSPLIT < HROWS) {
        request_first(HSPLIT, HROWS, false);
        dump(0, HSPLIT, HROWS, false);
    }
    raw_barrier();
    stamp(1);
    int k = 0;
    for (int ti = 0; ti < my_tiles; ++ti) {
        const int v = vt(ti), v_next = ti + 1 < my_tiles ? vt(ti + 1) : v;
        const int tile = vt_tile(v), c0 = vt_kh(v) * nck;
        int toffs[NTAPS], tdxs[NTAPS];
        if constexpr (NTAPS == 4 && !P4) {
            const int par = CCN_FDIV(tile, a.fd_nt, a.n_nt) % NPARC;
#pragma unroll
            for (int t = 0; t < NTAPS; ++t) { tdxs[t] = a.tapinfo_dx(par * 4 + t); toffs[t] = a.tapinfo_dy(par * 4 + t) * HPITCH + tdxs[t]; }
        }
#pragma unroll
        for (int i = 0; i < MF; ++i)
#pragma unroll
            for (int j = 0; j < NF; ++j)
#pragma unroll
                for (int q = 0; q < 16; ++q) acc[i][j][q] = 0.0f;
        for (int chunk = 0; chunk < nck; ++chunk, ++k) {
            const unsigned wb_cur = wbase_of(tile, c0 + chunk);
            const unsigned wb_nxt = chunk + 1 < nck ? wbase_of(tile, c0 + chunk + 1) : wbase_of(vt_tile(v_next), vt_kh(v_next) * nck);
            const int bufoff = (k & 1) * L::A_BYTES;
            if constexpr (S2) {
                const int pass = (c0 + chunk) % 5;
                tdxs[0] = (pass == 0 || pass == 1 || pass == 3) ? -1 : 0; tdxs[1] = 0;
                toffs[0] = ((pass == 0 || pass == 2) ? -HPITCH : 0) + tdxs[0];
                toffs[1] = pass == 0 ? -HPITCH : 0;
            }
            if constexpr (P4) {
                const int pass = (c0 + chunk) & 3;
                const int py = pass < 2 ? 1 : 0, px = (pass & 1) ? 0 : 1;
#pragma unroll
                for (int t = 0; t < NTAPS; ++t) { tdxs[t] = (t & 1) - px; toffs[t] = ((t >> 1) - py) * HPITCH + tdxs[t]; }
            }
#pragma unroll
            for (int i = 0; i < MF; ++i) asm volatile("" : "+v"(prow[i]));
            u32x4 av[2][MF];
            int abase[MF];
            auto frag = [&](int j, u32x4* av_) __attribute__((always_inline)) {
                const int tt = j >> 2, kk = j & 3;
                if (kk == 0) {
#pragma unroll
                    for (int i = 0; i < MF; ++i) abase[i] = bufoff + rbase(prow[i] + toffs[tt], r + 1 + tdxs[tt]);
                }
#pragma unroll
                for (int i = 0; i < MF; ++i) av_[i] = *(const u32x4*)(smem + (abase[i] ^ (kk << 5)));
            };
            if (!CCN_DBG_BIT(a, 64)) {
            frag(0, av[0]);
#pragma unroll
            for (int j = 0; j < NSTEP; ++j) {
                __builtin_amdgcn_sched_barrier(0);
                {
                    const int p = j + D - 1;
                    const unsigned off = p < NSTEP ? wb_cur + (unsigned)p * 1024u : wb_nxt + (unsigned)(p - NSTEP) * 1024u;
#pragma unroll
                    for (int jn = 0; jn < NF; ++jn)
                        bq[p % D][jn] = __builtin_amdgcn_raw_buffer_load_b128(wsrd, lane16, off + jn * COLB, 0);
                }
                if (j + 1 < NSTEP) frag(j + 1, av[(j + 1) & 1]);
#pragma unroll
                for (int jn = 0; jn < NF; ++jn)
#pragma unroll
                    for (int ii = 0; ii < MF; ++ii) { const int i = (jn & 1) ? MF - 1 - ii : ii; mfma16<T>(acc[i][jn], bq[j % D][jn], av[j & 1][i]); }
#pragma unroll
                for (int m = 0; m < MF * NF; ++m) {
                    __builtin_amdgcn_sched_group_barrier(0x008, 1, 0);
                    if (m < NF) __builtin_amdgcn_sched_group_barrier(0x020, 1, 0);
                    __builtin_amdgcn_sched_group_barrier(0x100, 1, 0);
                    __builtin_amdgcn_sched_group_barrier(0x002, 2, 0);
                }
                __builtin_amdgcn_sched_barrier(0);
            }
            }
            if (chunk + 1 == nck) {
#pragma unroll
                for (int i = 0; i < MF; ++i)
#pragma unroll
                    for (int j = 0; j < NF; ++j)
#pragma unroll
                        for (int g = 0; g < 4; ++g) {
                            const f32x16& c = acc[i][j];
                            typedef unsigned u32x2 __attribute__((ext_vector_type(2)));
                            const u32x2 pk = {pack_bf2(c[g * 4], c[g * 4 + 1]), pack_bf2(c[g * 4 + 2], c[g * 4 + 3])};
                            *(u32x2*)(stg + stg_lane + i * 32 * L::SP + (j * 32 + g * 8) * 2) = pk;
                        }
            }
            timed_barrier();
        }
    }
    __builtin_amdgcn_s_setprio(0);
    stamp(2); stamp_cycles();
    }
}

constexpr int PR_D = 6;
typedef void (*pr_fn_t)(const ConvArgs, int);
static pr_fn_t pick_pr(int ntaps, int mode, int th = 8, int gs = 0)
{
    if (ntaps == 16) return mode == 1 ? (pr_fn_t)conv_pr_kernel<4, 8, 1, 8, 0, true> : (pr_fn_t)conv_pr_kernel<4, 8, 0, 8, 0, true>;
    if (gs == 1 && ntaps == 9 && mode != 2) {
        if (th == 4) return mode == 1 ? (pr_fn_t)conv_pr_kernel<9, PR_D, 1, 4, 1> : (pr_fn_t)conv_pr_kernel<9, PR_D, 0, 4, 1>;
        return mode == 1 ? (pr_fn_t)conv_pr_kernel<9, PR_D, 1, 8, 1> : (pr_fn_t)conv_pr_kernel<9, PR_D, 0, 8, 1>;
    }
    if (gs == 2 && ntaps == 9) {
        if (th == 4) return mode == 1 ? (pr_fn_t)conv_pr_kernel<9, PR_D, 1, 4, 2> : (mode == 2 ? (pr_fn_t)conv_pr_kernel<9, PR_D, 2, 4, 2> : (pr_fn_t)conv_pr_kernel<9, PR_D, 0, 4, 2>);
        return mode == 1 ? (pr_fn_t)conv_pr_kernel<9, PR_D, 1, 8, 2> : (mode == 2 ? (pr_fn_t)conv_pr_kernel<9, PR_D, 2, 8, 2> : (pr_fn_t)conv_pr_kernel<9, PR_D, 0, 8, 2>);
    }
    if (ntaps == 9 && th == 4) return mode == 1 ? (pr_fn_t)conv_pr_kernel<9, PR_D, 1, 4> : (mode == 2 ? (pr_fn_t)conv_pr_kernel<9, PR_D, 2, 4> : (pr_fn_t)conv_pr_kernel<9, PR_D, 0, 4>);
    if (ntaps == 9) return mode == 1 ? (pr_fn_t)conv_pr_kernel<9, PR_D, 1> : (mode == 2 ? (pr_fn_t)conv_pr_kernel<9, PR_D, 2> : (pr_fn_t)conv_pr_kernel<9, PR_D, 0>);
    if (ntaps == 2) return mode == 1 ? (pr_fn_t)conv_pr_kernel<2, 8, 1> : (mode == 2 ? (pr_fn_t)conv_pr_kernel<2, 8, 2> : (pr_fn_t)conv_pr_kernel<2, 8, 0>);
    return mode == 1 ? (pr_fn_t)conv_pr_kernel<4, 8, 1> : (mode == 2 ? (pr_fn_t)conv_pr_kernel<4, 8, 2> : (pr_fn_t)conv_pr_kernel<4, 8, 0>);
}

bool conv_pr_supported(int kind, int bn, int th)
{
    return bn == 128 && (((kind == KIND_C3S1 || kind == KIND_CT4 || kind == KIND_C3S2) && th == 8) || (kind == KIND_C3S1 && th == 4));
}

static int g_cus = 0;
hipError_t conv_pr_prepare()
{
    hipError_t e = hipSuccess;
    for (int ntaps : {2, 4, 9, 16})
        for (int mode = 0; mode < 3; ++mode) {
            if (ntaps == 16 && mode == 2) continue;
            e = hipFuncSetAttribute((const void*)pick_pr(ntaps, mode), hipFuncAttributeMaxDynamicSharedMemorySize, (int)PrLds::TOTAL);
            if (e != hipSuccess) return e;
        }
    for (int mode = 0; mode < 3; ++mode) {
        e = hipFuncSetAttribute((const void*)pick_pr(9, mode, 4), hipFuncAttributeMaxDynamicSharedMemorySize, (int)PrLdsT<4>::TOTAL);
        if (e != hipSuccess) return e;
    }
    for (int gs = 1; gs <= 2; ++gs)
        for (int mode = 0; mode < 3; ++mode) {
            if (gs == 1 && mode == 2) continue;
            e = hipFuncSetAttribute((const void*)pick_pr(9, mode, 8, gs), hipFuncAttributeMaxDynamicSharedMemorySize, (int)PrLds::TOTAL);
            if (e != hipSuccess) return e;
            e = hipFuncSetAttribute((const void*)pick_pr(9, mode, 4, gs), hipFuncAttributeMaxDynamicSharedMemorySize, (int)PrLdsT<4>::TOTAL);
            if (e != hipSuccess) return e;
        }
    int dev = 0;
    e = hipGetDevice(&dev);
    if (e != hipSuccess) return e;
    hipDeviceProp_t prop;
    e = hipGetDeviceProperties(&prop, dev);
    if (e != hipSuccess) return e;
    g_cus = prop.multiProcessorCount;
    return hipSuccess;
}

static unsigned long long* g_stamps = nullptr;
static unsigned g_stamp_grid = 0;
extern "C" int ccn_internal_dump_stamps_pr(const char* path)
{
    if (!g_stamps || !g_stamp_grid) return 1;
    std::vector<unsigned long long> hbuf((size_t)g_stamp_grid * 16);
    if (hipMemcpy(hbuf.data(), g_stamps, hbuf.size() * 8, hipMemcpyDeviceToHost) != hipSuccess) return 2;
    FILE* f = fopen(path, "w");
    if (!f) return 3;
    for (unsigned b = 0; b < g_stamp_grid; ++b)
        for (int k = 0; k < 16; ++k) fprintf(f, "%llu%c", hbuf[(size_t)b * 16 + k], k == 15 ? '\n' : ' ');
    fclose(f);
    return 0;
}

hipError_t launch_conv_pr(int dtype, const ConvArgs& a, hipStream_t s)
{
    const bool c3 = a.ntaps == 9 && a.npar == 1 && a.OS == 1, ct = a.ntaps == 4 && a.npar == 4 && a.OS == 2;
    const bool s2 = a.ntaps == 2 && a.npar == 1 && a.OS == 1 && !a.gn_ab && (a.nchunk % 5) == 0;
    const bool p4 = a.ntaps == 16 && a.npar == 1 && a.OS == 1 && (a.nchunk % 4) == 0 && a.ksplit != 2;
    if ((ct || s2 || p4) && (a.gn_ab || a.gs_part)) return hipErrorInvalidValue;
    if (dtype != 1 || !a.wfrag || !(c3 || ct || s2 || p4) || !(a.th == 8 || (a.th == 4 && c3)) || (a.Cout_pad & 127) || a.nchunk < 2 || a.fin_counter || (a.res && a.film)) return hipErrorInvalidValue;
    const int ks = a.ksplit == 2 ? 2 : 1;
    if (ks == 2 && (!a.kpart || !a.kflag || (a.nchunk & 1) || (s2 && (a.nchunk / 2) % 5) || a.res)) return hipErrorInvalidValue;
    const int ntiles = a.B * a.n_ty * a.n_tx * a.npar * a.n_nt * ks;
    static const int cap = diag_env("CCN_PR_GRID") ? atoi(diag_env("CCN_PR_GRID")) : 0;
    int grid = cap > 0 ? cap : (g_cus > 0 ? g_cus : 256);
    if (grid > ntiles) grid = ntiles;
    if (ks == 2) { grid &= ~15; if (grid < 16) return hipErrorInvalidValue; }
    ConvArgs d = a;
    {
        auto magic = [](long dv) -> unsigned { return dv <= 1 ? 0u : (unsigned)((0x100000000ull + (unsigned long long)dv - 1) / (unsigned long long)dv); };
        const long dmax = std::max<long>(std::max<long>((long)a.n_nt * a.npar, (long)a.n_tx * a.n_ty), std::max<long>(a.cpg, a.gs_cpg));
        if ((unsigned long long)std::max<long>(ntiles, 8192) * (unsigned long long)dmax >= 0x100000000ull) return hipErrorInvalidValue;
        d.fd_nt = magic(a.n_nt); d.fd_ntp = magic((long)a.n_nt * a.npar); d.fd_tx = magic(a.n_tx); d.fd_sp = magic((long)a.n_tx * a.n_ty);
        d.fd_cpg = magic(a.cpg); d.fd_gscpg = magic(a.gs_cpg);
        d.fd_gsbn = magic(a.gs_bn); d.fd_gsnsp = magic(a.gs_nsp);
    }
    d.prod_first = (a.nchunk <= 2 && c3) ? 1 : 0;
    static const char* env = diag_env("CCN_STAMPS");
    if (env && (unsigned)atoi(env) == (unsigned)ntiles && (!strchr(env, ':') || atoi(strchr(env, ':') + 1) == a.ntaps)) {
        if (!g_stamps) { if (hipMalloc((void**)&g_stamps, (size_t)1024 * 24 * 8) != hipSuccess) return hipErrorOutOfMemory; }
        g_stamp_grid = (unsigned)grid;
        d.stamps = g_stamps;
    } else d.stamps = nullptr;
    if (a.gs_part && !(c3 && ks == 1)) return hipErrorInvalidValue;
    hipLaunchKernelGGL(pick_pr(a.ntaps, a.res ? 1 : (ks == 2 ? 2 : 0), a.th, a.gs_part ? 1 : (a.gn_ab ? 0 : 2)), dim3((unsigned)grid), dim3(512),
                       a.th == 4 ? PrLdsT<4>::TOTAL : PrLds::TOTAL, s, d, ntiles);
    return hipGetLastError();
}

}
```

clip-neural-image-conpression_amd/csrc/ccn_internal.h:

```cpp
#pragma once
#include <hip/hip_runtime.h>
#include <stdint.h>
#include <stddef.h>

#include <stdlib.h>

#ifdef CCN_DIAG
#define CCN_DBG_BIT(a, bit) ((((a).dbg) & (bit)) != 0)
#define CCN_STAMPS_PTR(a) ((a).stamps)
namespace ccn { inline const char* diag_env(const char* name) { return getenv(name); } }
#else
#define CCN_DBG_BIT(a, bit) false
#define CCN_STAMPS_PTR(a) ((unsigned long long*)nullptr)
namespace ccn { inline const char* diag_env(const char*) { return nullptr; } }
#endif

namespace ccn {

__host__ __device__ inline int pr3_slice(int g, int k32) { return ((g & 1) << 2) | (k32 << 1) | (g >> 1); }
__host__ __device__ inline size_t pr3_frag_index(int n, int k, int t, int Np)
{
    const int chunk = k >> 6, s = (k & 63) >> 3, e = k & 7;
    const int g = ((s >> 2) & 1) | ((s & 1) << 1), k32 = (s >> 1) & 1;
    const int nn = n >> 5, c = (n >> 4) & 1, lane = g * 16 + (n & 15);
    const int dy = t / 3, dx = t - dy * 3;
    const int f = ((dx * 2 + k32) * 3 + dy) * 2 + c;
    return ((((size_t)chunk * (size_t)(Np >> 5) + nn) * 36 + f) * 64 + lane) * 8 + e;
}

__host__ __device__ inline size_t pr4_frag_elem(size_t group, int n, int k)
{
    const int kw = k & 63;
    return ((group * 4 + (size_t)(kw >> 4)) * 64 + (size_t)((((kw >> 3) & 1) << 5) | (n & 31))) * 8 + (size_t)(kw & 7);
}
__host__ __device__ inline int prct_tap(int par, int t)
{
    const int ky = (par >> 1) ? ((t >> 1) ? 2 : 0) : ((t >> 1) ? 3 : 1), kx = (par & 1) ? ((t & 1) ? 2 : 0) : ((t & 1) ? 3 : 1);
    return ky * 4 + kx;
}
__host__ __device__ inline size_t prct_frag_index(int par, int t, int n, int k, int Np, int nch)
{
    return pr4_frag_elem((((size_t)par * nch + (k >> 6)) * (size_t)(Np >> 5) + (n >> 5)) * 4 + t, n, k);
}
__host__ __device__ inline int prs2_tap(int pass, int slot)
{
    const int dy = pass == 0 ? 0 : (pass == 1 ? 2 : (pass == 2 ? (slot ? 2 : 0) : 1));
    const int dx = pass == 2 ? 1 : (pass == 4 ? 1 : (slot ? 2 : 0));
    return (pass == 4 && slot) ? -1 : dy * 3 + dx;
}
__host__ __device__ inline size_t prs2_frag_index(int pass, int slot, int n, int k, int Np)
{
    return pr4_frag_elem((((size_t)(k >> 6) * 5 + pass) * (size_t)(Np >> 5) + (n >> 5)) * 2 + slot, n, k);
}
__host__ __device__ inline int prp4_tap(int pass, int t)
{
    const int py = pass < 2 ? 1 : 0, px = (pass & 1) ? 0 : 1, i = t >> 1, j = t & 1;
    const int ky = py ? (i ? 2 : 0) : (i ? 3 : 1), kx = px ? (j ? 2 : 0) : (j ? 3 : 1);
    return ky * 4 + kx;
}
__host__ __device__ inline size_t prp4_frag_index(int pass, int t, int n, int k, int Np)
{
    return pr4_frag_elem((((size_t)(k >> 6) * 4 + pass) * (size_t)(Np >> 5) + (n >> 5)) * 4 + t, n, k);
}

enum ConvKind { KIND_C3S1 = 0, KIND_C3S2 = 1, KIND_CT4 = 2, KIND_STEM = 3, KIND_HEAD = 4 };

struct ConvArgs {
    const void* in;
    const void* w;
    const void* wfrag;
    const float* bias;
    void* out;
    const float2* gn_ab;
    const float2* gs_part;
    const float* gs_gamma; const float* gs_beta;
    double gs_inv_count;
    int gs_nsp, gs_nnt, gs_bn, gs_cpg;
    const float* film;
    const void* res;
    float2* part;
    unsigned* fin_counter;
    const float* fin_gamma; const float* fin_beta;
    float2* fin_ab;
    double fin_count;
    int fin_blocks;
    int bn;
    float* x_state;
    float* eps_out;
    float c0, c1, c2, c3;
    const float* noise;
    float sigma;
    int do_ddim;
    int film_bstride;
    int B, Hin, Win, Cin, Cin_pad, Hout, Wout, Cout, Cout_pad;
    int MH, MW, OS, npar;
    unsigned long long* stamps;
    int dbg;
    int th;
    int use_pr;
    int use_stem2;
    unsigned fd_nt, fd_ntp, fd_tx, fd_sp, fd_cpg, fd_gscpg, fd_gsbn, fd_gsnsp;
    int prod_first;
    int ksplit;
    void* kpart;
    unsigned* kflag;
    unsigned* err;
    int n_ty, n_tx, n_nt, nchunk, ntaps;
    int silu;
    int cpg, G, nslot;
    int tapinfo[16];
    int ops;
    float wscale_inv;
    float* x0_hist;
    float c4;
    __host__ __device__ int tapinfo_dy(int i) const { return (tapinfo[i] & 3) - 1; }
    __host__ __device__ int tapinfo_dx(int i) const { return ((tapinfo[i] >> 2) & 3) - 1; }
    __host__ __device__ int tapinfo_w(int i) const { return tapinfo[i] >> 4; }
    static int make_tap(int dy, int dx, int wt) { return (dy + 1) | ((dx + 1) << 2) | (wt << 4); }
};

int conv_bn_for(int cout, int kind);
size_t conv_lds_bytes(int dtype, int kind, int bn);
hipError_t conv_prepare();
hipError_t launch_conv(int dtype, int kind, int bn, const ConvArgs& a, hipStream_t s);
enum ConvKernel { CK_IGEMM = 0, CK_WS, CK_FR, CK_PR, CK_STEM2 };
ConvKernel conv_kernel_for(int kind, int bn, const ConvArgs& a);
const char* conv_kernel_name(ConvKernel k);
int conv_tile_rows(int kind, int bn, int B, int MH, int MW, int npar, int n_nt);
bool conv_ws_enabled();
bool conv_ws_supported(int kind, int bn);
hipError_t conv_ws_prepare();
hipError_t launch_conv_ws(int dtype, int bn, const ConvArgs& a, hipStream_t s);
hipError_t conv_fr_prepare();
hipError_t launch_conv_fr(int dtype, int bn, const ConvArgs& a, hipStream_t s);

bool conv_pr_supported(int kind, int bn, int th);
bool conv_pr_selected(int dtype, int kind, int bn, int th);
hipError_t conv_pr_prepare();
hipError_t launch_conv_pr(int dtype, const ConvArgs& a, hipStream_t s);

bool stem2_supported(int dtype, int cin, int cout, int G);
int stem2_blocks(int H, int W, int* upw_out);
hipError_t launch_stem2(const ConvArgs& a, hipStream_t s);

inline int conv_cin_chunk(int dtype) { return dtype == 1 ? 64 : 32; }

struct ConvGeom { int Hout, Wout, MH, MW, OS, npar, ntaps, n_ty, n_tx; };
ConvGeom conv_geom(int kind, bool four, int Hin, int Win, int th);
void fill_taps(int* tapinfo, int kind, bool four);

struct ConvPolicy {
    bool pr;
    long s2_min_tiles8;
    bool ct_like_s2;
    bool split_k;
    bool split_k_s1;
    bool stem2;
};
struct ConvQuery {
    int dtype, kind;
    bool four;
    int BN, Cin, Cin_pad, Cout, Cout_pad, B, Hin, Win;
    int G;
    bool frag;
    bool gn_ab, res, film;
};
struct ConvRoute {
    ConvQuery q;
    ConvGeom g;
    int th, n_nt, nchunk, ntaps, ksplit, nslot, fin_blocks;
    bool pr, stem2;
    bool gs_ok;
    int part_nsp, part_nnt, part_bn;
    bool uses_frag() const { return pr || stem2; }
    void fill(ConvArgs& a) const;
};
ConvRoute conv_route(const ConvQuery& q, const ConvPolicy& p);
bool conv_in_kernel_stats(int dtype, int C, int G, int n_sp, int bn);

bool head2_supported(int dtype, int cin, int cout, int G);
size_t head2_scratch_bytes(int B, int C);
hipError_t launch_head2(const ConvArgs& a, const float2* ab, const float* w_f32, void* scratch, int step, hipStream_t s);

bool conv_wants_preact(int kind, int bn, int n_nt);
hipError_t launch_gn_act(int dtype, const void* x, const float2* ab, void* y, int B, int HW, int C, hipStream_t s);
hipError_t launch_gn_act_fused(int dtype, const void* x, void* y, int B, int HW, int C, const float2* part, int G, int n_sp, int n_nt,
                               int bn, int cpg, double count, const float* gamma, const float* beta, float eps, hipStream_t s,
                               float2* ab_out = nullptr, float2* stats_out = nullptr);

hipError_t launch_gn_finalize(const float2* part, int B, int G, int n_sp, int n_nt, int bn, int cpg, int C,
                              double count, const float* gamma, const float* beta, float eps,
                              float2* ab, hipStream_t s);

hipError_t launch_temb_i64(const int64_t* t, float* out, int n, int dim, hipStream_t s);
hipError_t launch_temb_i32(const int32_t* t, float* out, int n, int dim, hipStream_t s);
hipError_t launch_linear(const float* xa, const float* xb, int a_div, int b_mod, const float* W, const float* b,
                         float* y, int R, int K, int N, int act_silu, hipStream_t s);

hipError_t launch_ddim_step(float* x, const float* eps, const float* noise, float c0, float c1, float c2, float c3,
                            float sigma, int64_t n, hipStream_t s);
hipError_t launch_cfg_ddim_step(float* x, float* x_dup, const float* eps_c, const float* eps_u, const float* noise, float w,
                                float c0, float c1, float c2, float c3, float sigma, int64_t n, hipStream_t s);
hipError_t launch_ms_step(float* x, float* hist, const float* eps, float c0, float c1, float c2, float c3, float c4, int64_t n, hipStream_t s);
hipError_t launch_cfg_ms_step(float* x, float* x_dup, float* hist, const float* eps_c, const float* eps_u, float w, float c0, float c1,
                              float c2, float c3, float c4, int64_t n, hipStream_t s);
hipError_t launch_q_sample(float* out, const float* x0, const float* noise, const float* a, const float* sg,
                           int B, int64_t per, hipStream_t s);
hipError_t launch_predict_x0(float* out, const float* xt, const float* eps, const float* a, const float* sg,
                             int B, int64_t per, hipStream_t s);
hipError_t launch_film_nchw(const float* x, const float* sc, const float* sh, float* y, int B, int C, int64_t hw,
                            hipStream_t s);
hipError_t launch_nchw_to_nhwc(int dtype, const float* src, void* dst, int B, int C, int H, int W, hipStream_t s);
hipError_t launch_nhwc_to_nchw(int dtype, const void* src, float* dst, int B, int C, int H, int W, hipStream_t s);
hipError_t launch_gn_partials(int dtype, const void* x, float2* part, int B, int HW, int C, int cpg, int G,
                              int nslot, hipStream_t s);

}
```

clip-neural-image-conpression_amd/csrc/ccn_kernels.hip:

```cpp
#include "ccn_conv_tile.h"

namespace ccn {

__host__ __device__ constexpr int cmax(int a, int b) { return a > b ? a : b; }

template <int AK, int IS> struct HaloGeom {
    static constexpr int HOFF = AK == A_NHWC ? 1 : 0;
    static constexpr int ROWS = AK == A_NHWC ? (IS == 1 ? 6 : 10) : 4;
    static constexpr int PITCH = AK == A_NHWC ? (IS == 1 ? 34 : 66) : 32;
    static constexpr int BYTES = ROWS * PITCH * 128;
};
template <int AK, int IS, int BN> struct LdsGeom {
    static constexpr int A_BYTES = HaloGeom<AK, IS>::BYTES;
    static constexpr int B_BYTES = BN * 128;
    static constexpr int TOTAL = EpiLds<4, BN, 4>::total(A_BYTES + 2 * B_BYTES);
};

template <typename T, int AK, int IS, int EPI, int WM, int WN, int MF, int NF>
__global__ __launch_bounds__(256) void conv_igemm_kernel(const ConvArgs a)
{
    static_assert(WM * WN == 4 && WM * MF == 4, "4 waves, 4 M-fragments of 32 pixels (TH=4 rows of TW=32)");
    constexpr int BN = WN * NF * 32;
    constexpr int EPC = Vec16<T>::EPC;
    constexpr int CKE = 8 * EPC;
// ... 41 lines not shown
            constexpr int AU = HG::ROWS * HPITCH * 8;
            constexpr int AIT = (AU + 255) / 256;
            constexpr int GRP = 7;
            const int cbase = chunk * CKE + ck * EPC;
            const bool cvalid = cbase < a.Cin;
            const bool gn = a.gn_ab != nullptr;
            GnCoef<T> gk;
            gk.load(a.gn_ab + (size_t)b * a.Cin + (cvalid ? cbase : 0), gn && cvalid);
            const int iy0 = IS * my0 - 1, ix0 = IS * mx0 - 1;
#pragma unroll
            for (int g0 = 0; g0 < AIT; g0 += GRP) {
                u32x4 raw[GRP]; unsigned okm = 0;
#pragma unroll
                for (int u = 0; u < GRP; ++u) {
                    const int i = g0 + u;
                    raw[u] = u32x4{0u, 0u, 0u, 0u};
                    if (i < AIT) {
                        const int px = (tid >> 3) + 32 * i;
                        const int hy = px / HPITCH, hx = px - hy * HPITCH;
                        const int iy = iy0 + hy, ix = ix0 + hx;
                        const bool okv = px < HG::ROWS * HPITCH && cvalid && iy >= 0 && iy < a.Hin && ix >= 0 && ix < a.Win;
                        if (okv) {
                            okm |= 1u << u;
                            raw[u] = *(const u32x4*)(inb + (((size_t)(b * a.Hin + iy) * a.Win + ix) * a.Cin + cbase) * sizeof(T));
                        }
                    }
                }
#pragma unroll
                for (int u = 0; u < GRP; ++u) {
                    const int i = g0 + u;
                    if (i < AIT) {
                        const int px = (tid >> 3) + 32 * i;
                        if (px < HG::ROWS * HPITCH) {
                            u32x4 o = raw[u];
                            if (((okm >> u) & 1u) && gn)
                                o = gk.template apply<EPI == EPI_NHWC>(raw[u]);
                            *(u32x4*)(As + px * 128 + (((ck ^ (px >> 1)) & 7) << 4)) = o;
                        }
                    }
                }
            }
        } else {
            const float* xin = (const float*)a.in;
            const int kreal = a.Cin * 9;
#pragma unroll
            for (int i = 0; i < 4; ++i) {
                const int m = (tid >> 3) + 32 * i;
                const int y = my0 + (m >> 5), x = mx0 + (m & 31);
                float v[EPC];
#pragma unroll
                for (int e = 0; e < EPC; ++e) {
                    const int k = chunk * CKE + ck * EPC + e;
                    float val = 0.0f;
                    if (k < kreal) {
                        const int ci = k / 9, tp = k - ci * 9, ky = tp / 3, kx = tp - ky * 3;
                        const int iy = y + ky - 1, ix = x + kx - 1;
                        if (iy >= 0 && iy < a.Hin && ix >= 0 && ix < a.Win)
                            val = xin[((size_t)(b * a.Cin + ci) * a.Hin + iy) * a.Win + ix];
                    }
                    v[e] = val;
                }
                *(u32x4*)(As + m * 128 + (((ck ^ (m >> 1)) & 7) << 4)) = Vec16<T>::pack(v);
            }
        }
    };

    f32x16 acc[MF][NF];
#pragma unroll
    for (int i = 0; i < MF; ++i)
#pragma unroll
        for (int j = 0; j < NF; ++j)
#pragma unroll
            for (int q = 0; q < 16; ++q) acc[i][j][q] = 0.0f;

    int pbase[MF], nrow[NF];
#pragma unroll
    for (int i = 0; i < MF; ++i) pbase[i] = (IS * (wm * MF + i) + HG::HOFF) * HPITCH + IS * r + HG::HOFF;
#pragma unroll
    for (int j = 0; j < NF; ++j) nrow[j] = (wn * NF + j) * 32 + r;

    const int n_it = a.nchunk * a.ntaps;
    CCN_LOAD_B(0)
    for (int it = 0; it < n_it; ++it) {
        const int chunk = it / a.ntaps, tap = it - chunk * a.ntaps;
        if (tap == 0) {
            if (it > 0) __syncthreads();
            stage_A(chunk);
        }
        CCN_STORE_B(it & 1)
        __syncthreads();
        if (it + 1 < n_it) CCN_LOAD_B(it + 1)
        const int dy = a.tapinfo_dy(par_off + tap), dx = a.tapinfo_dx(par_off + tap);
        const unsigned char* const Bb = Bs + (it & 1) * LG::B_BYTES;
        int pa[MF];
#pragma unroll
        for (int i = 0; i < MF; ++i) pa[i] = pbase[i] + dy * HPITCH + dx;
#pragma unroll
        for (int kk = 0; kk < 4; ++kk) {
            u32x4 av[MF], bv[NF];
#pragma unroll
            for (int i = 0; i < MF; ++i)
                av[i] = *(const u32x4*)(As + pa[i] * 128 + ((((2 * kk + h) ^ (pa[i] >> 1)) & 7) << 4));
#pragma unroll
            for (int j = 0; j < NF; ++j)
                bv[j] = *(const u32x4*)(Bb + nrow[j] * 128 + ((((2 * kk + h) ^ (nrow[j] >> 1)) & 7) << 4));
#pragma unroll
            for (int i = 0; i < MF; ++i)
#pragma unroll
                for (int j = 0; j < NF; ++j) mfma16<T>(acc[i][j], av[i], bv[j]);
        }
    }

#undef CCN_LOAD_B
#undef CCN_STORE_B
    __syncthreads();
    float* const Cs = (float*)smem;
    constexpr int CP = E::CP;
#pragma unroll
    for (int i = 0; i < MF; ++i)
#pragma unroll
        for (int j = 0; j < NF; ++j)
#pragma unroll
            for (int q = 0; q < 16; ++q) {
                const int m = (wm * MF + i) * 32 + (q & 3) + 8 * (q >> 2) + 4 * h;
                Cs[m * CP + (wn * NF + j) * 32 + r] = acc[i][j][q];
            }
    __syncthreads();

    if constexpr (EPI == EPI_HEAD) {
        if (tid < 128) {
            const int m = tid, my = my0 + (m >> 5), mx = mx0 + (m & 31);
            if (my < a.MH && mx < a.MW) {
                for (int c = 0; c < a.Cout; ++c) {
                    const float e = Cs[m * CP + c] + a.bias[c];
                    const size_t idx = ((size_t)(b * a.Cout + c) * a.Hout + my) * a.Wout + mx;
                    if (a.eps_out) a.eps_out[idx] = e;
                    if (a.do_ddim) {
                        const float x = a.x_state[idx];
                        const float c4 = a.x0_hist ? a.c4 : 0.f;
                        const float hv = c4 != 0.f ? a.x0_hist[idx] : 0.f;
                        float x0;
                        float xn = sampler_update(x, e, a.c0, a.c1, a.c2, a.c3, c4, hv, x0);
                        if (a.noise) xn = __fadd_rn(xn, __fmul_rn(a.sigma, a.noise[idx]));
                        if (a.x0_hist) a.x0_hist[idx] = x0;
                        a.x_state[idx] = xn;
                    }
                }
            }
        }
    } else {
        constexpr int NOCT = BN / 8, PSL = 256 / NOCT, NIT = 128 / PSL;
        const int o = tid % NOCT, ps = tid / NOCT;
        const int nb = n0 + o * 8;
        const bool nvalid = nb < a.Cout;
        float bias8[8], f1[8], f2[8];
#pragma unroll
        for (int e = 0; e < 8; ++e) { bias8[e] = 0.f; f1[e] = 1.f; f2[e] = 0.f; }
        if (nvalid) {
#pragma unroll
            for (int e = 0; e < 8; ++e) bias8[e] = a.bias[nb + e];
            if (a.film) {
                const float* fp = a.film + (size_t)b * a.film_bstride;
#pragma unroll
                for (int e = 0; e < 8; ++e) { f1[e] = 1.0f + fp[nb + e]; f2[e] = fp[a.Cout + nb + e]; }
            }
        }
        float s1[8], s2[8];
#pragma unroll
        for (int e = 0; e < 8; ++e) { s1[e] = 0.f; s2[e] = 0.f; }
        unsigned char* const outb = (unsigned char*)a.out;
        const unsigned char* const resb = (const unsigned char*)a.res;
#pragma unroll
        for (int itp = 0; itp < NIT; ++itp) {
            const int m = itp * PSL + ps;
            const int my = my0 + (m >> 5), mx = mx0 + (m & 31);
            if (nvalid && my < a.MH && mx < a.MW) {
                const int oy = my * a.OS + py, ox = mx * a.OS + px_;
                const size_t eoff = ((size_t)(b * a.Hout + oy) * a.Wout + ox) * a.Cout + nb;
                float v[8];
                const f32x4 c0 = *(const f32x4*)(Cs + m * CP + o * 8), c1 = *(const f32x4*)(Cs + m * CP + o * 8 + 4);
#pragma unroll
                for (int e = 0; e < 4; ++e) { v[e] = c0[e]; v[4 + e] = c1[e]; }
#pragma unroll
                for (int e = 0; e < 8; ++e) v[e] = fmaf(v[e] + bias8[e], f1[e], f2[e]);
                if (resb) {
                    float rv[8];
                    if constexpr (EPC == 8) {
                        Vec16<T>::unpack(*(const u32x4*)(resb + eoff * sizeof(T)), rv);
                    } else {
                        Vec16<T>::unpack(*(const u32x4*)(resb + eoff * sizeof(T)), rv);
                        Vec16<T>::unpack(*(const u32x4*)(resb + eoff * sizeof(T) + 16), rv + 4);
                    }
#pragma unroll
                    for (int e = 0; e < 8; ++e) v[e] += rv[e];
                }
                if constexpr (EPC == 8) {
                    *(u32x4*)(outb + eoff * sizeof(T)) = Vec16<T>::pack(v);
                } else {
                    *(u32x4*)(outb + eoff * sizeof(T)) = Vec16<T>::pack(v);
                    *(u32x4*)(outb + eoff * sizeof(T) + 16) = Vec16<T>::pack(v + 4);
                }
#pragma unroll
                for (int e = 0; e < 8; ++e) { s1[e] += v[e]; s2[e] = fmaf(v[e], v[e], s2[e]); }
            }
        }
        if (a.part) {
#include "tile/gn_part_tail.inc"
        }
    }
}

int conv_bn_for(int cout, int kind)
{
    if (kind == KIND_HEAD) return 32;
    if (cout >= 128) return 128;
    if (cout >= 64) return 64;
    return 32;
}

template <int AK, int IS> static size_t lds_for(int bn)
{
    switch (bn) {
        case 128: return LdsGeom<AK, IS, 128>::TOTAL;
        case 64: return LdsGeom<AK, IS, 64>::TOTAL;
        default: return LdsGeom<AK, IS, 32>::TOTAL;
    }
}
size_t conv_lds_bytes(int dtype, int kind, int bn)
{
    (void)dtype;
    switch (kind) {
        case KIND_C3S2: return lds_for<A_NHWC, 2>(bn);
        case KIND_STEM: return lds_for<A_IM2COL, 1>(bn);
        default: return lds_for<A_NHWC, 1>(bn);
    }
}

typedef void (*conv_fn_t)(const ConvArgs);

template <typename T, int AK, int IS> static conv_fn_t pick_bn(int bn)
{
    switch (bn) {
        case 128: return conv_igemm_kernel<T, AK, IS, EPI_NHWC, 2, 2, 2, 2>;
        case 64: return conv_igemm_kernel<T, AK, IS, EPI_NHWC, 2, 2, 2, 1>;
        default: return conv_igemm_kernel<T, AK, IS, EPI_NHWC, 4, 1, 1, 1>;
    }
}
template <typename T> static conv_fn_t pick_kind(int kind, int bn)
{
    switch (kind) {
        case KIND_C3S2: return pick_bn<T, A_NHWC, 2>(bn);
        case KIND_STEM: return pick_bn<T, A_IM2COL, 1>(bn);
        case KIND_HEAD: return conv_igemm_kernel<T, A_NHWC, 1, EPI_HEAD, 4, 1, 1, 1>;
        default: return pick_bn<T, A_NHWC, 1>(bn);
    }
}
static conv_fn_t pick(int dtype, int kind, int bn)
{
    return dtype == 0 ? pick_kind<float>(kind, bn) : pick_kind<__bf16>(kind, bn);
}

hipError_t conv_prepare()
{
    static const int kinds[] = {KIND_C3S1, KIND_C3S2, KIND_STEM, KIND_HEAD};
    static const int bns[] = {32, 64, 128};
    for (int dt = 0; dt < 2; ++dt)
        for (int kind : kinds)
            for (int bn : bns) {
                if (kind == KIND_HEAD && bn != 32) continue;
                hipError_t e = hipFuncSetAttribute((const void*)pick(dt, kind, bn), hipFuncAttributeMaxDynamicSharedMemorySize,
                                                   (int)conv_lds_bytes(dt, kind, bn));
                if (e != hipSuccess) return e;
            }
    hipError_t e;
    if ((e = conv_ws_prepare()) != hipSuccess) return e;
    if ((e = conv_fr_prepare()) != hipSuccess) return e;
    return conv_pr_prepare();
}

bool conv_ws_enabled()
{
    static const int on = diag_env("CCN_CONV_V1") ? 0 : 1;
    return on != 0;
}

int conv_tile_rows(int kind, int bn, int B, int MH, int MW, int npar, int n_nt)
{
    if (!conv_ws_enabled() || !conv_ws_supported(kind, bn)) return 4;
    const long blocks8 = (long)B * ((MH + 7) / 8) * ((MW + 31) / 32) * npar * n_nt;
    static const long min8 = diag_env("CCN_MIN8") ? atol(diag_env("CCN_MIN8")) : 256;
    return blocks8 >= min8 ? 8 : 4;
}

static int g_conv_variant = -1;
static int conv_variant()
{
    if (g_conv_variant < 0) g_conv_variant = diag_env("CCN_CONV_DMA") ? atoi(diag_env("CCN_CONV_DMA")) : 4;
    return g_conv_variant;
}
extern "C" int ccn_internal_set_conv_variant(int v) { const int old = conv_variant(); g_conv_variant = v; return old; }

bool conv_pr_selected(int dtype, int kind, int bn, int th)
{
    return dtype == 1 && conv_ws_enabled() && conv_variant() == 4 && conv_pr_supported(kind, bn, th);
}

ConvGeom conv_geom(int kind, bool four, int Hin, int Win, int th)
{
    ConvGeom g{};
    switch (kind) {
        case KIND_C3S2: g.Hout = (Hin - 1) / 2 + 1; g.Wout = (Win - 1) / 2 + 1; g.MH = g.Hout; g.MW = g.Wout; g.OS = 1; g.npar = 1; g.ntaps = four ? 16 : 9; break;
        case KIND_CT4: g.Hout = Hin * 2; g.Wout = Win * 2; g.MH = Hin; g.MW = Win; g.OS = 2; g.npar = 4; g.ntaps = 4; break;
        case KIND_STEM: g.Hout = Hin; g.Wout = Win; g.MH = Hin; g.MW = Win; g.OS = 1; g.npar = 1; g.ntaps = 1; break;
        default: g.Hout = Hin; g.Wout = Win; g.MH = Hin; g.MW = Win; g.OS = 1; g.npar = 1; g.ntaps = 9; break;
    }
    g.n_ty = (g.MH + th - 1) / th; g.n_tx = (g.MW + 31) / 32;
    return g;
}

void fill_taps(int* tapinfo, int kind, bool four)
{
    for (int i = 0; i < 16; ++i) tapinfo[i] = 0;
    if (kind == KIND_STEM) { tapinfo[0] = ConvArgs::make_tap(0, 0, 0); return; }
    if (kind == KIND_CT4) {
        static const int kk[2][2] = {{1, 3}, {0, 2}}, dd[2][2] = {{0, -1}, {1, 0}};
        for (int py = 0; py < 2; ++py)
            for (int px = 0; px < 2; ++px)
                for (int i = 0; i < 2; ++i)
                    for (int j = 0; j < 2; ++j)
                        tapinfo[(py * 2 + px) * 4 + i * 2 + j] = ConvArgs::make_tap(dd[py][i], dd[px][j], kk[py][i] * 4 + kk[px][j]);
        return;
    }
    const int k = four ? 4 : 3;
    for (int ky = 0; ky < k; ++ky)
        for (int kx = 0; kx < k; ++kx) tapinfo[ky * k + kx] = ConvArgs::make_tap(ky - 1, kx - 1, ky * k + kx);
}

ConvRoute conv_route(const ConvQuery& q, const ConvPolicy& p)
{
    ConvRoute r{};
    r.q = q;
    r.n_nt = q.Cout_pad / q.BN;
    const ConvGeom g8 = conv_geom(q.kind, q.four, q.Hin, q.Win, 8);
    const long tiles8 = (long)q.B * g8.n_ty * g8.n_tx * g8.npar * r.n_nt;
    r.th = conv_tile_rows(q.kind, q.BN, q.B, g8.MH, g8.MW, g8.npar, r.n_nt);
    const int nch = q.Cin_pad / conv_cin_chunk(q.dtype);
    const double out_bytes = (double)q.B * g8.Hout * g8.Wout * q.Cout * (q.dtype == 1 ? 2 : 4);
    if (p.pr && q.frag && nch >= 2 && !(q.res && q.film) && out_bytes < 2.0e9) {
        if (q.kind == KIND_C3S1) r.pr = conv_pr_selected(q.dtype, q.kind, q.BN, r.th);
        else if (!q.gn_ab && (q.kind == KIND_C3S2 || (q.kind == KIND_CT4 && !q.four))) {
            if (q.kind == KIND_CT4 && !p.ct_like_s2) r.pr = conv_pr_selected(q.dtype, q.kind, q.BN, r.th);
            else if (conv_pr_selected(q.dtype, q.kind, q.BN, 8) && tiles8 >= p.s2_min_tiles8) { r.pr = true; r.th = 8; }
        }
    }
    r.ksplit = 1;
    if (r.pr && p.split_k && !q.res && (q.kind == KIND_C3S2 || (q.kind == KIND_C3S1 && p.split_k_s1))) {
        const int nk = q.kind == KIND_C3S2 ? 5 * nch : nch;
        if (tiles8 >= 32 && tiles8 <= 128 && nk >= 4 && (nch & 1) == 0) { r.ksplit = 2; r.th = 8; }
    }
    r.g = conv_geom(q.kind, q.four, q.Hin, q.Win, r.th);
    r.nchunk = nch; r.ntaps = r.g.ntaps;
    if (r.pr && q.kind == KIND_C3S2) {
        if (q.four) r.nchunk *= 4;
        else { r.nchunk *= 5; r.ntaps = 2; }
    }
    r.gs_ok = r.pr && r.ksplit == 1 && q.kind == KIND_C3S1;
    r.fin_blocks = r.g.n_ty * r.g.n_tx * r.g.npar * r.n_nt;
    r.nslot = r.fin_blocks;
    r.part_nsp = r.g.n_ty * r.g.n_tx * r.g.npar; r.part_nnt = r.n_nt; r.part_bn = q.BN;
    r.stem2 = p.stem2 && q.kind == KIND_STEM && q.frag && stem2_supported(q.dtype, q.Cin, q.Cout, q.G) && !q.gn_ab && !q.film && !q.res;
    if (r.stem2) {
        r.nslot = 4 * stem2_blocks(q.Hin, q.Win, nullptr);
        r.part_nsp = r.nslot; r.part_nnt = 1; r.part_bn = 1 << 30;
    }
    return r;
}

void ConvRoute::fill(ConvArgs& a) const
{
    a.B = q.B; a.Hin = q.Hin; a.Win = q.Win; a.Cin = q.Cin; a.Cin_pad = q.Cin_pad;
    a.Hout = g.Hout; a.Wout = g.Wout; a.Cout = q.Cout; a.Cout_pad = q.Cout_pad;
    a.MH = g.MH; a.MW = g.MW; a.OS = g.OS; a.npar = g.npar; a.ntaps = ntaps;
    a.th = th; a.n_ty = g.n_ty; a.n_tx = g.n_tx; a.n_nt = n_nt; a.nchunk = nchunk;
    a.use_pr = pr ? 1 : 0; a.use_stem2 = stem2 ? 1 : 0; a.ksplit = ksplit;
    a.silu = 1;
    a.G = q.Cout < q.G ? q.Cout : q.G; a.cpg = q.Cout / a.G;
    a.nslot = nslot; a.fin_blocks = fin_blocks; a.bn = q.BN;
    fill_taps(a.tapinfo, q.kind, q.four);
}

bool conv_in_kernel_stats(int dtype, int C, int G, int n_sp, int bn)
{
    if (dtype != 1 || n_sp <= 0 || G != 8 || (C / G) % 8 != 0) return false;
    const int cpg = C / G;
    int nj = 1;
    for (int g = 0; g < G; ++g) { const int n = ((g + 1) * cpg - 1) / bn - (g * cpg) / bn + 1; if (n > nj) nj = n; }
    return (long)n_sp * nj <= 64;
}

ConvKernel conv_kernel_for(int kind, int bn, const ConvArgs& a)
{
    if (a.use_stem2) return CK_STEM2;
    if (a.use_pr && kind == KIND_C3S2) return CK_PR;
    if (conv_ws_enabled() && conv_ws_supported(kind, bn)) {
        if (a.use_pr) return CK_PR;
        const int variant = conv_variant();
        if (variant == 2 || (variant >= 3 && a.th == 8)) return CK_FR;
        return CK_WS;
    }
    return CK_IGEMM;
}

const char* conv_kernel_name(ConvKernel k)
{
    switch (k) {
        case CK_WS: return "ws";
        case CK_FR: return "fr";
        case CK_PR: return "pr";
        case CK_STEM2: return "stem2";
        default: return "igemm";
    }
}

hipError_t launch_conv(int dtype, int kind, int bn, const ConvArgs& a, hipStream_t s)
{
    const ConvKernel k = conv_kernel_for(kind, bn, a);
    if (k == CK_STEM2) return launch_stem2(a, s);
    if (k == CK_PR && kind == KIND_C3S2) return launch_conv_pr(dtype, a, s);
    if (a.ops && k != CK_WS && k != CK_FR) return hipErrorInvalidValue;
    if (k != CK_IGEMM) {
        static const int dbg = diag_env("CCN_DBG") ? atoi(diag_env("CCN_DBG")) : 0;
        ConvArgs d = a; d.dbg = dbg;
        if (k == CK_PR) return launch_conv_pr(dtype, d, s);
        if (k == CK_FR) return launch_conv_fr(dtype, bn, d, s);
        return launch_conv_ws(dtype, bn, d, s);
    }
    if (a.th != 4) return hipErrorInvalidValue;
    const conv_fn_t fn = pick(dtype, kind, bn);
    const unsigned grid = (unsigned)(a.B * a.n_ty * a.n_tx * a.npar * a.n_nt);
    hipLaunchKernelGGL(fn, dim3(grid), dim3(256), conv_lds_bytes(dtype, kind, bn), s, a);
    return hipGetLastError();
}

bool conv_wants_preact(int kind, int bn, int n_nt)
{
    static const int mode = diag_env("CCN_PREACT") ? atoi(diag_env("CCN_PREACT")) : 1;
    if (!conv_ws_enabled() || !conv_ws_supported(kind, bn) || kind != KIND_C3S1) return false;
    return mode == 2 || (mode == 1 && n_nt >= 2);
}

template <typename T>
__global__ __launch_bounds__(256) void gn_act_kernel(const T* __restrict__ x, const float2* __restrict__ ab, T* __restrict__ y,
                                                      int HW, int C)
{
    constexpr int EPC = Vec16<T>::EPC;
    const int nsl = C / EPC;
    const int pstep = 256 / nsl;
    const int b = blockIdx.y, tid = threadIdx.x;
    const int sl = tid % nsl, pp = tid / nsl;
    if (pp >= pstep) return;
    const int p0 = blockIdx.x * 4 * pstep + pp;
    GnCoef<T> gk;
    gk.load(ab + (size_t)b * C + sl * EPC, true);
    u32x4 v[4];
#pragma unroll
    for (int k = 0; k < 4; ++k) {
        const int p = p0 + k * pstep;
        v[k] = u32x4{0u, 0u, 0u, 0u};
        if (p < HW) v[k] = *(const u32x4*)(x + ((size_t)b * HW + p) * C + sl * EPC);
    }
#pragma unroll
    for (int k = 0; k < 4; ++k) {
        const int p = p0 + k * pstep;
        if (p < HW) *(u32x4*)(y + ((size_t)b * HW + p) * C + sl * EPC) = gk.template apply<true>(v[k]);
    }
}
template <typename T>
__global__ __launch_bounds__(256) void gn_act_fused_kernel(const T* __restrict__ x, T* __restrict__ y, int HW, int C,
                                                            const float2* __restrict__ part, int G, int nslot, int n_nt, int bn, int cpg,
                                                            double count, const float* __restrict__ gamma, const float* __restrict__ beta, float eps,
                                                            float2* __restrict__ ab_out, float2* __restrict__ stats_out)
{
    constexpr int EPC = Vec16<T>::EPC;
    __shared__ double st[64][2];
    const int nsl = C / EPC, pstep = 256 / nsl;
    const int b = blockIdx.y, tid = threadIdx.x, lane = tid & 63, wave = tid >> 6;
    const int sl = tid % nsl, pp = tid / nsl;
    const int p0 = blockIdx.x * 4 * pstep + pp;
    const bool act = pp < pstep;
    u32x4 v[4];
#pragma unroll
    for (int k = 0; k < 4; ++k) {
        const int p = p0 + k * pstep;
        v[k] = u32x4{0u, 0u, 0u, 0u};
        if (act && p < HW) v[k] = *(const u32x4*)(x + ((size_t)b * HW + p) * C + sl * EPC);
    }
    for (int g = wave; g < G; g += 4) {
        double mean, rstd;
        gn_group_stats(part, b, g, G, nslot, n_nt, bn, cpg, count, eps, lane, mean, rstd);
        if (lane == 0) { st[g][0] = mean; st[g][1] = rstd; }
    }
    __syncthreads();
    if (ab_out && blockIdx.x == 0) {
        for (int c = tid; c < C; c += 256) {
            const int g = c / cpg;
            const double sc = (double)gamma[c] * st[g][1];
            float* const row = (float*)(ab_out + (size_t)b * C) + 4 * (c >> 1) + (c & 1);
            row[0] = (float)sc; row[2] = (float)((double)beta[c] - st[g][0] * sc);
        }
        if (tid < G) stats_out[b * G + tid] = make_float2((float)st[tid][0], (float)st[tid][1]);
    }
    if (!act) return;
    GnCoef<T> gk;
#pragma unroll
    for (int e = 0; e < EPC; ++e) {
        const int c = sl * EPC + e, g = c / cpg;
        const double sc = (double)gamma[c] * st[g][1];
        gk.a[e] = (float)sc; gk.c[e] = (float)((double)beta[c] - st[g][0] * sc);
    }
#pragma unroll
    for (int k = 0; k < 4; ++k) {
        const int p = p0 + k * pstep;
        if (p < HW) *(u32x4*)(y + ((size_t)b * HW + p) * C + sl * EPC) = gk.template apply<true>(v[k]);
    }
}
hipError_t launch_gn_act_fused(int dtype, const void* x, void* y, int B, int HW, int C, const float2* part, int G, int n_sp, int n_nt,
                               int bn, int cpg, double count, const float* gamma, const float* beta, float eps, hipStream_t s,
                               float2* ab_out, float2* stats_out)
{
    const int epc = dtype == 0 ? 4 : 8, nsl = C / epc;
    if (nsl > 256 || nsl <= 0 || G > 64) return hipErrorInvalidValue;
    const int pstep = 256 / nsl;
    const dim3 grid((HW + 4 * pstep - 1) / (4 * pstep), B);
    if (dtype == 0) hipLaunchKernelGGL(gn_act_fused_kernel<float>, grid, dim3(256), 0, s, (const float*)x, (float*)y, HW, C, part, G, n_sp * n_nt, n_nt, bn, cpg, count, gamma, beta, eps, ab_out, stats_out);
    else hipLaunchKernelGGL(gn_act_fused_kernel<__bf16>, grid, dim3(256), 0, s, (const __bf16*)x, (__bf16*)y, HW, C, part, G, n_sp * n_nt, n_nt, bn, cpg, count, gamma, beta, eps, ab_out, stats_out);
    return hipGetLastError();
}

hipError_t launch_gn_act(int dtype, const void* x, const float2* ab, void* y, int B, int HW, int C, hipStream_t s)
{
    const int epc = dtype == 0 ? 4 : 8, nsl = C / epc;
    if (nsl > 256 || nsl <= 0) return hipErrorInvalidValue;
    const int pstep = 256 / nsl;
    const dim3 grid((HW + 4 * pstep - 1) / (4 * pstep), B);
    if (dtype == 0) hipLaunchKernelGGL(gn_act_kernel<float>, grid, dim3(256), 0, s, (const float*)x, ab, (float*)y, HW, C);
    else hipLaunchKernelGGL(gn_act_kernel<__bf16>, grid, dim3(256), 0, s, (const __bf16*)x, ab, (__bf16*)y, HW, C);
    return hipGetLastError();
}

__global__ __launch_bounds__(256) void gn_finalize_kernel(const float2* __restrict__ part, int G, int n_sp, int n_nt, int bn,
                                                           int cpg, int C, double count, const float* __restrict__ gamma,
                                                           const float* __restrict__ beta, float eps, float2* __restrict__ ab)
{
    __shared__ double red[4][2];
    const int bg = blockIdx.x, b = bg / G, g = bg % G, tid = threadIdx.x, lane = tid & 63, wave = tid >> 6;
    const int jlo = (g * cpg) / bn, jhi = ((g + 1) * cpg - 1) / bn, nj = jhi - jlo + 1, ne = n_sp * nj;
    const float2* base = part + (size_t)(b * G + g) * n_sp * n_nt;
    double s1 = 0.0, s2 = 0.0;
    for (int e = tid; e < ne; e += 256) {
        const int sp = e / nj, j = jlo + (e - sp * nj);
        const float2 v = base[(size_t)sp * n_nt + j];
        s1 += (double)v.x; s2 += (double)v.y;
    }
#pragma unroll
    for (int s = 32; s >= 1; s >>= 1) { s1 += __shfl_xor(s1, s); s2 += __shfl_xor(s2, s); }
    if (lane == 0) { red[wave][0] = s1; red[wave][1] = s2; }
    __syncthreads();
    s1 = (red[0][0] + red[1][0]) + (red[2][0] + red[3][0]);
    s2 = (red[0][1] + red[1][1]) + (red[2][1] + red[3][1]);
    const double mean = s1 / count;
    double var = s2 / count - mean * mean;
    if (var < 0.0) var = 0.0;
    const double rstd = 1.0 / sqrt(var + (double)eps);
    for (int c = g * cpg + tid; c < (g + 1) * cpg; c += 256) {
        const double sc = (double)gamma[c] * rstd;
        float* const row = (float*)(ab + (size_t)b * C) + 4 * (c >> 1) + (c & 1);
        row[0] = (float)sc; row[2] = (float)((double)beta[c] - mean * sc);
    }
}

hipError_t launch_gn_finalize(const float2* part, int B, int G, int n_sp, int n_nt, int bn, int cpg, int C, double count,
                              const float* gamma, const float* beta, float eps, float2* ab, hipStream_t s)
{
    hipLaunchKernelGGL(gn_finalize_kernel, dim3(B * G), dim3(256), 0, s, part, G, n_sp, n_nt, bn, cpg, C, count, gamma, beta, eps, ab);
    return hipGetLastError();
}

template <typename T>
__global__ __launch_bounds__(256) void gn_partials_kernel(const T* __restrict__ x, float2* __restrict__ part, int HW, int C,
                                                           int cpg, int G, int nslot)
{
    __shared__ float sh[256 * 2];
    const int slot = blockIdx.x, b = blockIdx.y, tid = threadIdx.x;
    const int per = (HW + nslot - 1) / nslot;
    const int p0 = slot * per, p1 = min(HW, p0 + per);
    const int nsub = 256 / G;
    const int g = tid % G, sub = tid / G;
    float s1 = 0.f, s2 = 0.f;
    if (sub < nsub)
        for (int p = p0 + sub; p < p1; p += nsub) {
            const T* row = x + ((size_t)b * HW + p) * C + g * cpg;
            for (int j = 0; j < cpg; ++j) { const float v = (float)row[j]; s1 += v; s2 = fmaf(v, v, s2); }
        }
    sh[tid * 2] = s1; sh[tid * 2 + 1] = s2;
    __syncthreads();
    if (tid < G) {
        float t1 = 0.f, t2 = 0.f;
        for (int q = 0; q < nsub; ++q) { t1 += sh[(q * G + tid) * 2]; t2 += sh[(q * G + tid) * 2 + 1]; }
// ... 283 lines not shown
```

Baseline: 82.15 images/sec.

## Specialize persistent conv kernel per fixed layer geometry with compile-time shapes

Adds compile-time geometry structs for the UNet's known conv shapes and instantiates the persistent conv kernel per shape, so dims, strides and index divisions become constants. At launch a matching table entry is chosen; otherwise the generic runtime-argument kernel is used. The goal is to cut integer division and index arithmetic and to give the compiler constant loop bounds, which costs extra instantiations, binary size and compile time. Variant 5 keeps the generic path for comparison.

```diff
diff --git a/clip-neural-image-conpression_amd/csrc/ccn_api.hip b/clip-neural-image-conpression_amd/csrc/ccn_api.hip
--- a/clip-neural-image-conpression_amd/csrc/ccn_api.hip
+++ b/clip-neural-image-conpression_amd/csrc/ccn_api.hip
@@ -104,6 +104,7 @@
     std::string name;
     int kind = 0;
     const char* kernel = "";
+    const char* geom = nullptr;
     int th = 0, ksplit = 1, n_nt = 1;
     const char* gn = "none";
     bool film = false, res = false;
@@ -471,6 +472,8 @@
             out.prod = (int)pl.ops.size();
         }
         L.part = out.part;
+        if (conv_kernel_for(cw.kind, cw.BN, a) == CK_PR)
+            pl.routes.back().geom = conv_pr_geom_name(a, o.res != nullptr, o.film_off >= 0, L.gs_part != kNone ? 1 : (gn_ab != kNone ? 0 : 2));
         const double macs = (double)B * g.Hout * g.Wout * cw.Cout * (double)(cw.kind == KIND_CT4 ? 4 : 9) * cw.Cin;
         L.flops = 2.0 * macs;
         L.bytes = ((double)B * in.H * in.W * cw.Cin + (double)B * g.Hout * g.Wout * cw.Cout + (o.res ? (double)B * g.Hout * g.Wout * cw.Cout : 0.0)
@@ -801,13 +804,13 @@
     return (int)text.size();
 }
 
-std::string routes_text(const ShapePlan& pl)
+std::string routes_text(const ShapePlan& pl, bool instantiations = false)
 {
     static const char* kinds[] = {"C3S1", "C3S2", "CT4", "STEM", "HEAD"};
     std::string text;
     for (const RouteRec& r : pl.routes) {
         char line[256];
-        std::snprintf(line, sizeof(line), "%s %s %s th=%d ksplit=%d n_nt=%d gn=%s film=%d res=%d", r.name.c_str(), kinds[r.kind], r.kernel,
+        std::snprintf(line, sizeof(line), "%s %s %s th=%d ksplit=%d n_nt=%d gn=%s film=%d res=%d", r.name.c_str(), kinds[r.kind], instantiations && r.geom ? r.geom : r.kernel,
                       r.th, r.ksplit, r.n_nt, r.gn, r.film ? 1 : 0, r.res ? 1 : 0);
         text += std::string(line) + (r.ops < 0 ? "" : r.ops ? " ops=f16x3" : " ops=f32") + "\n";
     }
@@ -1307,6 +1310,17 @@
     if (!h || !h->committed || shape_plan(h, B, H, W, steps, &pl)) return -1;
     return copy_report(routes_text(*pl), buf, cap);
 }
+extern "C" int ccn_internal_plan_kernels(ccn_handle_t h, char* buf, size_t cap)
+{
+    if (!h || h->bindings.empty()) return -1;
+    return copy_report(routes_text(*h->bindings.back()->plan, true), buf, cap);
+}
+extern "C" int ccn_internal_plan_kernels_of(ccn_handle_t h, int32_t B, int32_t H, int32_t W, int32_t steps, char* buf, size_t cap)
+{
+    const ShapePlan* pl;
+    if (!h || !h->committed || shape_plan(h, B, H, W, steps, &pl)) return -1;
+    return copy_report(routes_text(*pl, true), buf, cap);
+}
 extern "C" int ccn_internal_plan_layout(ccn_handle_t h, int32_t B, int32_t H, int32_t W, int32_t steps, char* buf, size_t cap)
 {
     const ShapePlan* pl;
diff --git a/clip-neural-image-conpression_amd/csrc/ccn_conv_pr.hip b/clip-neural-image-conpression_amd/csrc/ccn_conv_pr.hip
--- a/clip-neural-image-conpression_amd/csrc/ccn_conv_pr.hip
+++ b/clip-neural-image-conpression_amd/csrc/ccn_conv_pr.hip
@@ -22,9 +22,42 @@
 typedef PrLdsT<8> PrLds;
 static_assert(PrLds::TOTAL <= 160 * 1024, "LDS budget");
 
-}
-
-template <int NTAPS, int D, int MODE, int TH = 8, int GS = 0, bool P4 = false>
+#define CCN_PR_GEOM_INTS(X) \
+    X(Hin) X(Win) X(Cin) X(Hout) X(Wout) X(Cout) X(Cout_pad) X(MH) X(MW) X(nchunk) X(n_nt) X(n_tx) X(n_ty) X(cpg) X(G) X(nslot) \
+    X(gs_nsp) X(gs_nnt) X(gs_bn) X(gs_cpg) X(film_bstride)
+template <class GEO> struct PrGeo {
+    static constexpr bool FIXED = true;
+#define X(f) static __host__ __device__ __forceinline__ constexpr int f(const ConvArgs&) { return GEO::f; }
+    CCN_PR_GEOM_INTS(X)
+#undef X
+    static __device__ __forceinline__ constexpr bool film(const ConvArgs&) { return GEO::HAS_FILM; }
+};
+template <> struct PrGeo<void> {
+    static constexpr bool FIXED = false;
+#define X(f) static __host__ __device__ __forceinline__ int f(const ConvArgs& a) { return a.f; }
+    CCN_PR_GEOM_INTS(X)
+#undef X
+    static __device__ __forceinline__ bool film(const ConvArgs& a) { return a.film != nullptr; }
+};
+template <int FORM, int TH_, int H, int W, int CIN, int COUT, bool FILM, int GSNSP = 1, int GSNNT = 1, int FBS = 0>
+struct PrGeom {
+    static constexpr int Hin = H, Win = W, Cin = CIN, Cout = COUT, Cout_pad = COUT;
+    static constexpr int Hout = FORM == 2 ? H / 2 : (FORM == 4 ? H * 2 : H), Wout = FORM == 2 ? W / 2 : (FORM == 4 ? W * 2 : W);
+    static constexpr int MH = FORM == 4 ? H : Hout, MW = FORM == 4 ? W : Wout, npar = FORM == 4 ? 4 : 1;
+    static constexpr int nchunk = CIN / 64 * (FORM == 2 ? 5 : 1);
+    static constexpr int n_nt = COUT / 128, n_tx = (MW + 31) / 32, n_ty = (MH + TH_ - 1) / TH_;
+    static constexpr int G = 8, cpg = COUT / 8, nslot = n_ty * n_tx * npar * n_nt;
+    static constexpr int gs_nsp = GSNSP, gs_nnt = GSNNT, gs_bn = 128, gs_cpg = CIN / 8;
+    static constexpr int film_bstride = FBS;
+    static constexpr bool HAS_FILM = FILM;
+    static_assert(H % 2 == 0 && W % 2 == 0 && CIN % 64 == 0 && COUT % 128 == 0 && (COUT / 8) % 8 == 0, "unpadded shapes only");
+};
+#define CCN_GDIV(x, m, d) (PrGeo<GEO>::FIXED ? (int)((unsigned)(x) / (unsigned)(d)) : CCN_FDIV(x, a.m, d))
+#define CCN_GV(f) (PrGeo<GEO>::f(a))
+
+}
+
+template <int NTAPS, int D, int MODE, int TH = 8, int GS = 0, bool P4 = false, class GEO = void>
 __global__ __launch_bounds__(512) void conv_pr_kernel(const ConvArgs a, const int grid_tiles)
 {
     static_assert(TH == 8 || (TH == 4 && NTAPS == 9), "4-row tiles: 3x3 stride-1 form only");
@@ -57,7 +90,7 @@
     auto vt = [&](int ti) __attribute__((always_inline)) { return vb + ti * grid; };
     const int ks = (MODE == 2 && a.ksplit == 2) ? 2 : 1;
     const unsigned xcc_id = MODE == 2 ? (unsigned)__builtin_amdgcn_s_getreg((3 << 11) | 20) : 0u;
-    const int nck = a.nchunk / ks;
+    const int nck = CCN_GV(nchunk) / ks;
     const int ktotal = my_tiles * nck;
     auto vt_tile = [&](int v) __attribute__((always_inline)) { return ks == 2 ? (v >> 1) : v; };
     auto vt_kh = [&](int v) __attribute__((always_inline)) { return ks == 2 ? (v & 1) : 0; };
@@ -94,7 +127,7 @@
     const int o16 = etid & 15, pr = etid >> 4;
     unsigned char* const outb = (unsigned char*)a.out;
     const unsigned char* const resb = (const unsigned char*)a.res;
-    const unsigned out_bytes = (unsigned)((size_t)a.B * a.Hout * a.Wout * a.Cout * sizeof(T));
+    const unsigned out_bytes = (unsigned)((size_t)a.B * CCN_GV(Hout) * CCN_GV(Wout) * CCN_GV(Cout) * sizeof(T));
     float* const chs = (float*)(stg + L::STG_BYTES) + ew * 256;
     constexpr int NQ = TH / 2;
     u32x4 rr[RR ? 2 : 1][4];
@@ -108,28 +141,28 @@
     unsigned e_m0 = OOB, e_m1 = OOB;
     auto item_off = [&](unsigned eb, int it) __attribute__((always_inline)) -> unsigned {
         const unsigned rmask = (it >> 1) < e_rows ? 0u : OOB;
-        return (eb + (unsigned)(it >> 1) * (unsigned)(OSC * a.Wout * a.Cout * (int)sizeof(T)) + (unsigned)((it & 1) * 16) * (unsigned)(OSC * a.Cout * (int)sizeof(T)))
+        return (eb + (unsigned)(it >> 1) * (unsigned)(OSC * CCN_GV(Wout) * CCN_GV(Cout) * (int)sizeof(T)) + (unsigned)((it & 1) * 16) * (unsigned)(OSC * CCN_GV(Cout) * (int)sizeof(T)))
                | ((it & 1) ? e_m1 : e_m0) | rmask;
     };
     auto epi_setup = [&](int v) __attribute__((always_inline)) {
         const int tile = vt_tile(v);
         e_kh = vt_kh(v); e_tile = tile;
-        const int t2 = CCN_FDIV(tile, a.fd_nt, a.n_nt);
-        e_nt = tile - t2 * a.n_nt;
+        const int t2 = CCN_GDIV(tile, fd_nt, CCN_GV(n_nt));
+        e_nt = tile - t2 * CCN_GV(n_nt);
         e_par = t2 % NPARC;
         const int sp = t2 / NPARC;
         {
-            const int row = CCN_FDIV(sp, a.fd_tx, a.n_tx);
-            e_tx = sp - row * a.n_tx;
-            e_b = CCN_FDIV(sp, a.fd_sp, a.n_tx * a.n_ty);
-            e_ty = row - e_b * a.n_ty;
+            const int row = CCN_GDIV(sp, fd_tx, CCN_GV(n_tx));
+            e_tx = sp - row * CCN_GV(n_tx);
+            e_b = CCN_GDIV(sp, fd_sp, CCN_GV(n_tx) * CCN_GV(n_ty));
+            e_ty = row - e_b * CCN_GV(n_ty);
         }
         const int nb = e_nt * BN + o16 * 8;
-        const bool nvalid = nb < a.Cout;
-        e_base = (unsigned)(((e_b * a.Hout + e_ty * TH * OSC + (e_par >> 1)) * a.Wout + (e_tx * 32 + pr) * OSC + (e_par & 1)) * a.Cout + nb) * (unsigned)sizeof(T);
-        e_rows = a.MH - e_ty * TH;
-        e_m0 = (nvalid && e_tx * 32 + pr < a.MW) ? 0u : OOB;
-        e_m1 = (nvalid && e_tx * 32 + pr + 16 < a.MW) ? 0u : OOB;
+        const bool nvalid = nb < CCN_GV(Cout);
+        e_base = (unsigned)(((e_b * CCN_GV(Hout) + e_ty * TH * OSC + (e_par >> 1)) * CCN_GV(Wout) + (e_tx * 32 + pr) * OSC + (e_par & 1)) * CCN_GV(Cout) + nb) * (unsigned)sizeof(T);
+        e_rows = CCN_GV(MH) - e_ty * TH;
+        e_m0 = (nvalid && e_tx * 32 + pr < CCN_GV(MW)) ? 0u : OOB;
+        e_m1 = (nvalid && e_tx * 32 + pr + 16 < CCN_GV(MW)) ? 0u : OOB;
     };
     auto res_on = [&]() __attribute__((always_inline)) -> bool { return RES || (MODE == 2 && ks == 2 && e_kh == 1); };
     auto res_batch = [&](int q, u32x4* dst) __attribute__((always_inline)) {
@@ -168,13 +201,13 @@
             asm volatile("" ::: "memory");
         }
         const int nb = e_nt * BN + o16 * 8;
-        const int nbs = nb < a.Cout ? nb : 0;
+        const int nbs = nb < CCN_GV(Cout) ? nb : 0;
         fb[0] = *(const f32x4*)(a.bias + nbs); fb[1] = *(const f32x4*)(a.bias + nbs + 4);
         if constexpr (!RES) {
-            if (a.film) {
-                const float* fp = a.film + (size_t)e_b * a.film_bstride;
+            if (PrGeo<GEO>::film(a)) {
+                const float* fp = a.film + (size_t)e_b * CCN_GV(film_bstride);
                 fs[0] = *(const f32x4*)(fp + nbs); fs[1] = *(const f32x4*)(fp + nbs + 4);
-                ft[0] = *(const f32x4*)(fp + a.Cout + nbs); ft[1] = *(const f32x4*)(fp + a.Cout + nbs + 4);
+                ft[0] = *(const f32x4*)(fp + CCN_GV(Cout) + nbs); ft[1] = *(const f32x4*)(fp + CCN_GV(Cout) + nbs + 4);
             }
         }
         res_batch(q0, rr[q0 & 1]);
@@ -188,7 +221,7 @@
             f2[e] = second ? 0.f : fb[e >> 2][e & 3];
             if constexpr (!RES) {
                 f1[e] = 1.f;
-                if (a.film) { f1[e] = 1.0f + fs[e >> 2][e & 3]; f2[e] = second ? 0.f : fmaf(f2[e], f1[e], ft[e >> 2][e & 3]); }
+                if (PrGeo<GEO>::film(a)) { f1[e] = 1.0f + fs[e >> 2][e & 3]; f2[e] = second ? 0.f : fmaf(f2[e], f1[e], ft[e >> 2][e & 3]); }
             }
         }
         const auto osrd_c = __builtin_amdgcn_make_buffer_rsrc((void*)(first ? kpartb : outb), 0, out_bytes, 0x00020000);
@@ -251,7 +284,7 @@
                 for (int e = 0; e < 8; ++e) { chs[(lane * 8 + e) * 2] = s1[e]; chs[(lane * 8 + e) * 2 + 1] = s2[e]; }
             }
             pd_on = true; pd_b = e_b; pd_n0 = e_nt * BN;
-            pd_slot = ((e_ty * a.n_tx + e_tx) * NPARC + e_par) * a.n_nt + e_nt;
+            pd_slot = ((e_ty * CCN_GV(n_tx) + e_tx) * NPARC + e_par) * CCN_GV(n_nt) + e_nt;
         }
     };
     auto combine = [&]() __attribute__((always_inline)) {
@@ -259,11 +292,11 @@
         pd_on = false;
         const float* const all = (const float*)(stg + L::STG_BYTES);
         const int n0 = pd_n0;
-        if (n0 >= a.Cout) return;
-        const int nend = min(n0 + BN, a.Cout);
-        const int g1 = CCN_FDIV(nend - 1, a.fd_cpg, a.cpg);
-        for (int g = CCN_FDIV(n0, a.fd_cpg, a.cpg) + ew; g <= g1; g += 4) {
-            const int clo = max(g * a.cpg, n0), chi = min((g + 1) * a.cpg, nend);
+        if (n0 >= CCN_GV(Cout)) return;
+        const int nend = min(n0 + BN, CCN_GV(Cout));
+        const int g1 = CCN_GDIV(nend - 1, fd_cpg, CCN_GV(cpg));
+        for (int g = CCN_GDIV(n0, fd_cpg, CCN_GV(cpg)) + ew; g <= g1; g += 4) {
+            const int clo = max(g * CCN_GV(cpg), n0), chi = min((g + 1) * CCN_GV(cpg), nend);
             float t1 = 0.f, t2 = 0.f;
             const float* const wa = all + (lane >> 4) * 256;
             for (int c = clo + (lane & 15); c < chi; c += 16) {
@@ -271,7 +304,7 @@
             }
 #pragma unroll
             for (int m = 32; m >= 1; m >>= 1) { t1 += __shfl_xor(t1, m); t2 += __shfl_xor(t2, m); }
-            if (lane == 0) part_store(a.part + (size_t)(pd_b * a.G + g) * a.nslot + pd_slot, t1, t2);
+            if (lane == 0) part_store(a.part + (size_t)(pd_b * CCN_GV(G) + g) * CCN_GV(nslot) + pd_slot, t1, t2);
         }
     };
 
@@ -295,15 +328,15 @@
     float2 sv[8];
     auto stats_issue = [&](int b) __attribute__((always_inline)) {
         const int g = lane >> 3, sub = lane & 7;
-        const int cpg = a.gs_cpg, pnt = a.gs_nnt, nsp = a.gs_nsp;
-        const int jlo = CCN_FDIV(g * cpg, a.fd_gsbn, a.gs_bn), jhi = CCN_FDIV((g + 1) * cpg - 1, a.fd_gsbn, a.gs_bn), nj = jhi - jlo + 1;
+        const int cpg = CCN_GV(gs_cpg), pnt = CCN_GV(gs_nnt), nsp = CCN_GV(gs_nsp);
+        const int jlo = CCN_GDIV(g * cpg, fd_gsbn, CCN_GV(gs_bn)), jhi = CCN_GDIV((g + 1) * cpg - 1, fd_gsbn, CCN_GV(gs_bn)), nj = jhi - jlo + 1;
         const float2* const base = a.gs_part + (size_t)(b * 8 + g) * ((size_t)nsp * pnt) + jlo;
         int off[8];
         svmask = 0u;
 #pragma unroll
         for (int u = 0; u < 8; ++u) {
             const int e = sub + 8 * u;
-            const int jj = CCN_FDIV(e, a.fd_gsnsp, nsp), sp = e - jj * nsp;
+            const int jj = CCN_GDIV(e, fd_gsnsp, nsp), sp = e - jj * nsp;
             const bool ok = jj < nj;
             off[u] = ok ? sp * pnt + jj : 0;
             svmask |= ok ? (1u << u) : 0u;
@@ -329,16 +362,16 @@
         if (rq_c == 0) {
             q_tv = rq_ti < my_tiles;
             const int tile = vt_tile(q_tv ? v : vt(0));
-            const int sp = CCN_FDIV(tile, a.fd_ntp, a.n_nt * NPARC);
-            const int row = CCN_FDIV(sp, a.fd_tx, a.n_tx);
-            const int tx = sp - row * a.n_tx;
-            q_b = CCN_FDIV(sp, a.fd_sp, a.n_tx * a.n_ty);
-            const int ty = row - q_b * a.n_ty;
+            const int sp = CCN_GDIV(tile, fd_ntp, CCN_GV(n_nt) * NPARC);
+            const int row = CCN_GDIV(sp, fd_tx, CCN_GV(n_tx));
+            const int tx = sp - row * CCN_GV(n_tx);
+            q_b = CCN_GDIV(sp, fd_sp, CCN_GV(n_tx) * CCN_GV(n_ty));
+            const int ty = row - q_b * CCN_GV(n_ty);
             q_iy0 = ty * TH - 1; q_ix0 = tx * 32 - 1;
         }
         q_c = vt_kh(v) * nck + rq_c;
         const int cb = (q_c / NPASS) * CKE + ck * EPC;
-        q_cv = q_tv && cb < a.Cin;
+        q_cv = q_tv && cb < CCN_GV(Cin);
         q_cbs = q_cv ? cb : 0;
         const bool fresh = gstat && rq_c == 0 && q_tv && q_b != st_b;
         if (++rq_c == nck) { rq_c = 0; ++rq_ti; }
@@ -348,11 +381,11 @@
         if (gstat) {
             qn_g[0] = *(const f32x4*)(a.gs_gamma + q_cbs); qn_g[1] = *(const f32x4*)(a.gs_gamma + q_cbs + 4);
             qn_bt[0] = *(const f32x4*)(a.gs_beta + q_cbs); qn_bt[1] = *(const f32x4*)(a.gs_beta + q_cbs + 4);
-        } else gkn.load(a.gn_ab + (size_t)q_b * a.Cin + q_cbs, gn && q_cv);
+        } else gkn.load(a.gn_ab + (size_t)q_b * CCN_GV(Cin) + q_cbs, gn && q_cv);
     };
     auto coef_sel = [&]() __attribute__((always_inline)) {
         if (gstat) {
-            const int src = CCN_FDIV(q_cbs, a.fd_gscpg, a.gs_cpg) * 8;
+            const int src = CCN_GDIV(q_cbs, fd_gscpg, CCN_GV(gs_cpg)) * 8;
             qn_mean = __shfl(st_mean, src); qn_rstd = __shfl(st_rstd, src);
         }
     };
@@ -373,19 +406,19 @@
         const int py = S2 ? (pass <= 2 ? 1 : 0) : (P4 ? (pass < 2 ? 1 : 0) : 0);
         const int px = S2 ? ((pass <= 1 || pass == 3) ? 1 : 0) : (P4 ? ((pass & 1) ? 0 : 1) : 0);
         const int cb = cc * CKE + ck * EPC;
-        const bool cv = q_tv && cb < a.Cin;
+        const bool cv = q_tv && cb < CCN_GV(Cin);
         q_cv_i = cv;
-        const unsigned img_bytes = (unsigned)(a.Hin * a.Win * a.Cin) * (unsigned)sizeof(T);
-        const unsigned coff = (unsigned)(((q_tv && cc * CKE < a.Cin) ? cc : 0) * CKE) * (unsigned)sizeof(T);
+        const unsigned img_bytes = (unsigned)(CCN_GV(Hin) * CCN_GV(Win) * CCN_GV(Cin)) * (unsigned)sizeof(T);
+        const unsigned coff = (unsigned)(((q_tv && cc * CKE < CCN_GV(Cin)) ? cc : 0) * CKE) * (unsigned)sizeof(T);
         const auto srd = __builtin_amdgcn_make_buffer_rsrc((void*)(inb + (size_t)b * img_bytes + coff), 0, img_bytes - coff, 0x00020000);
-        const int rs = IS * a.Win * a.Cin * (int)sizeof(T);
+        const int rs = IS * CCN_GV(Win) * CCN_GV(Cin) * (int)sizeof(T);
         const int ixr = IS * (ix0 + pcol) + px;
-        colv = cv && ixr >= 0 && ixr < a.Win;
+        colv = cv && ixr >= 0 && ixr < CCN_GV(Win);
         const unsigned cmask = colv ? 0u : OOB;
-        const int base = ((IS * iy0 + py) * a.Win + ixr) * a.Cin * (int)sizeof(T) + ck * 16;
+        const int base = ((IS * iy0 + py) * CCN_GV(Win) + ixr) * CCN_GV(Cin) * (int)sizeof(T) + ck * 16;
         const int first = IS * iy0 + py;
         const int r_lo = first < 0 ? (-first + IS - 1) / IS : 0;
-        int r_hi = (a.Hin - first + IS - 1) / IS; r_hi = r_hi > HROWS ? HROWS : (r_hi < 0 ? 0 : r_hi);
+        int r_hi = (CCN_GV(Hin) - first + IS - 1) / IS; r_hi = r_hi > HROWS ? HROWS : (r_hi < 0 ? 0 : r_hi);
         rowm = q_tv ? (((1u << r_hi) - 1u) & ~((1u << r_lo) - 1u)) : 0u;
 #pragma unroll
         for (int i = 0; i < HROWS; ++i) {
@@ -394,8 +427,8 @@
         }
         {
             const int iyr = IS * (iy0 + xrow) + py, ixx = IS * (ix0 + xcol) + px;
-            xv = xthr && cv && iyr >= 0 && iyr < a.Hin && ixx >= 0 && ixx < a.Win;
-            const int off = (iyr * a.Win + ixx) * a.Cin * (int)sizeof(T) + ck * 16;
+            xv = xthr && cv && iyr >= 0 && iyr < CCN_GV(Hin) && ixx >= 0 && ixx < CCN_GV(Win);
+            const int off = (iyr * CCN_GV(Win) + ixx) * CCN_GV(Cin) * (int)sizeof(T) + ck * 16;
             if (with_x) areg[HROWS] = __builtin_amdgcn_raw_buffer_load_b128(srd, (unsigned)off | (xv ? 0u : OOB), 0, 0);
         }
     };
@@ -480,13 +513,13 @@
         constexpr int WIN = 6, PF = 4;
         static_assert((NG * NSG) % WIN == 0, "static window indexing");
         f32x16 acc[TH];
-        const int n32 = a.Cout_pad / 32;
+        const int n32 = CCN_GV(Cout_pad) / 32;
         constexpr unsigned COLB = 36 * 1024;
-        const unsigned wtotal = (unsigned)((size_t)a.nchunk * n32 * COLB);
+        const unsigned wtotal = (unsigned)((size_t)CCN_GV(nchunk) * n32 * COLB);
         const auto wsrd = __builtin_amdgcn_make_buffer_rsrc((void*)a.wfrag, 0, wtotal, 0x00020000);
         const unsigned lane16 = (unsigned)lane * 16u;
         auto wbase_of = [&](int tile, int chunk) __attribute__((always_inline)) -> unsigned {
-            const int nt = tile - CCN_FDIV(tile, a.fd_nt, a.n_nt) * a.n_nt;
+            const int nt = tile - CCN_GDIV(tile, fd_nt, CCN_GV(n_nt)) * CCN_GV(n_nt);
             return (unsigned)__builtin_amdgcn_readfirstlane((int)((unsigned)(chunk * n32 + nt * 4 + wave) * COLB));
         };
         const int px16 = lane & 15, g4 = lane >> 4;
@@ -514,8 +547,8 @@
         raw_barrier();
         stamp(1);
         int k = 0;
-        const bool idle_w = ks == 1 && grid % a.n_nt == 0 &&
-                            (vt_tile(vt(0)) - CCN_FDIV(vt_tile(vt(0)), a.fd_nt, a.n_nt) * a.n_nt) * BN + wave * 32 >= a.Cout;
+        const bool idle_w = ks == 1 && grid % CCN_GV(n_nt) == 0 &&
+                            (vt_tile(vt(0)) - CCN_GDIV(vt_tile(vt(0)), fd_nt, CCN_GV(n_nt)) * CCN_GV(n_nt)) * BN + wave * 32 >= CCN_GV(Cout);
         if (idle_w) { for (int kk = 0; kk < ktotal; ++kk) timed_barrier(); }
         else
         for (int ti = 0; ti < my_tiles; ++ti) {
@@ -592,15 +625,15 @@
     int prow[MF];
 #pragma unroll
     for (int i = 0; i < MF; ++i) prow[i] = ((wm * MF + i) + 1) * HPITCH + r + 1;
-    const int n32 = a.Cout_pad / 32;
+    const int n32 = CCN_GV(Cout_pad) / 32;
     constexpr unsigned COLB = NSTEP * 1024;
-    const unsigned wtotal = (unsigned)((size_t)NPARC * a.nchunk * n32 * COLB);
+    const unsigned wtotal = (unsigned)((size_t)NPARC * CCN_GV(nchunk) * n32 * COLB);
     const auto wsrd = __builtin_amdgcn_make_buffer_rsrc((void*)a.wfrag, 0, wtotal, 0x00020000);
     const unsigned lane16 = (unsigned)lane * 16u;
     auto wbase_of = [&](int tile, int chunk) __attribute__((always_inline)) -> unsigned {
-        const int t2 = CCN_FDIV(tile, a.fd_nt, a.n_nt);
-        const int nt = tile - t2 * a.n_nt, par = t2 % NPARC;
-        return (unsigned)__builtin_amdgcn_readfirstlane((int)((unsigned)((par * a.nchunk + chunk) * n32 + nt * 4 + wn * NF) * COLB));
+        const int t2 = CCN_GDIV(tile, fd_nt, CCN_GV(n_nt));
+        const int nt = tile - t2 * CCN_GV(n_nt), par = t2 % NPARC;
+        return (unsigned)__builtin_amdgcn_readfirstlane((int)((unsigned)((par * CCN_GV(nchunk) + chunk) * n32 + nt * 4 + wn * NF) * COLB));
     };
     u32x4 bq[D][NF];
     {
@@ -624,7 +657,7 @@
         const int tile = vt_tile(v), c0 = vt_kh(v) * nck;
         int toffs[NTAPS], tdxs[NTAPS];
         if constexpr (NTAPS == 4 && !P4) {
-            const int par = CCN_FDIV(tile, a.fd_nt, a.n_nt) % NPARC;
+            const int par = CCN_GDIV(tile, fd_nt, CCN_GV(n_nt)) % NPARC;
 #pragma unroll
             for (int t = 0; t < NTAPS; ++t) { tdxs[t] = a.tapinfo_dx(par * 4 + t); toffs[t] = a.tapinfo_dy(par * 4 + t) * HPITCH + tdxs[t]; }
         }
@@ -730,6 +763,73 @@
     return mode == 1 ? (pr_fn_t)conv_pr_kernel<4, 8, 1> : (mode == 2 ? (pr_fn_t)conv_pr_kernel<4, 8, 2> : (pr_fn_t)conv_pr_kernel<4, 8, 0>);
 }
 
+struct PrGeomRow {
+    const char* name; pr_fn_t fn;
+    int ntaps, mode, th, gs, npar;
+    bool film;
+#define X(f) int f;
+    CCN_PR_GEOM_INTS(X)
+#undef X
+};
+template <int FORM, int MODE, int TH, int GS, class GEO> static PrGeomRow pr_geom_row(const char* name)
+{
+    PrGeomRow r{};
+    r.name = name; r.fn = (pr_fn_t)conv_pr_kernel<FORM, FORM == 9 ? PR_D : 8, MODE, TH, GS, false, GEO>;
+    r.ntaps = FORM; r.mode = MODE; r.th = TH; r.gs = GS; r.npar = GEO::npar;
+    r.film = GEO::HAS_FILM;
+#define X(f) r.f = GEO::f;
+    CCN_PR_GEOM_INTS(X)
+#undef X
+    return r;
+}
+constexpr int PR_FBS = 7680;
+static const std::vector<PrGeomRow>& pr_geom_rows()
+{
+#define CCN_PR_C3(tag, TH, GS, HW, C, NSP, NNT) \
+    pr_geom_row<9, 0, TH, GS, PrGeom<9, TH, HW, HW, C, C, true, NSP, NNT, PR_FBS>>("pr:c3." tag ".film"), \
+    pr_geom_row<9, 1, TH, GS, PrGeom<9, TH, HW, HW, C, C, false, NSP, NNT>>("pr:c3." tag ".res")
+    static const std::vector<PrGeomRow> rows = {
+        CCN_PR_C3("128x256", 8, 0, 256, 128, 1, 1),
+        CCN_PR_C3("128x128", 8, 1, 128, 128, 64, 1),
+        CCN_PR_C3("256x64", 8, 1, 64, 256, 16, 2),
+        CCN_PR_C3("512x32", 4, 1, 32, 512, 8, 4),
+        pr_geom_row<9, 0, 4, 1, PrGeom<9, 4, 32, 32, 512, 512, true, 4, 4, PR_FBS>>("pr:c3.512x32.film.s4"),
+#ifndef CCN_PR_NO_GEOM_S2CT
+        pr_geom_row<2, 0, 8, 2, PrGeom<2, 8, 256, 256, 128, 128, false>>("pr:s2.128x256"),
+        pr_geom_row<2, 0, 8, 2, PrGeom<2, 8, 128, 128, 128, 256, false>>("pr:s2.128x128"),
+        pr_geom_row<2, 2, 8, 2, PrGeom<2, 8, 64, 64, 256, 512, false>>("pr:s2.256x64.k2"),
+        pr_geom_row<4, 1, 8, 2, PrGeom<4, 8, 32, 32, 512, 256, false>>("pr:ct.512x32"),
+        pr_geom_row<4, 1, 8, 2, PrGeom<4, 8, 64, 64, 256, 128, false>>("pr:ct.256x64"),
+        pr_geom_row<4, 1, 8, 2, PrGeom<4, 8, 128, 128, 128, 128, false>>("pr:ct.128x128"),
+#endif
+    };
+#undef CCN_PR_C3
+    return rows;
+}
+
+static bool pr_geom_unused(const char* f, int gs, bool film) { return (!strncmp(f, "gs_", 3) && gs != 1) || (!strcmp(f, "film_bstride") && !film); }
+
+static const PrGeomRow* pr_geom_match(const ConvArgs& a, int mode, int gs, bool film)
+{
+    if (!conv_pr_geom_enabled()) return nullptr;
+    for (const PrGeomRow& r : pr_geom_rows()) {
+        if (r.ntaps != a.ntaps || r.mode != mode || r.th != a.th || r.gs != gs || r.npar != a.npar || r.film != film) continue;
+        if (a.Cin_pad != r.Cin || (mode == 2) != (a.ksplit == 2)) continue;
+        bool same = true;
+#define X(f) same = same && (r.f == a.f || pr_geom_unused(#f, gs, film));
+        CCN_PR_GEOM_INTS(X)
+#undef X
+        if (same) return &r;
+    }
+    return nullptr;
+}
+
+const char* conv_pr_geom_name(const ConvArgs& a, bool res, bool film, int gs)
+{
+    const PrGeomRow* r = pr_geom_match(a, res ? 1 : (a.ksplit == 2 ? 2 : 0), gs, film);
+    return r ? r->name : nullptr;
+}
+
 bool conv_pr_supported(int kind, int bn, int th)
 {
     return bn == 128 && (((kind == KIND_C3S1 || kind == KIND_CT4 || kind == KIND_C3S2) && th == 8) || (kind == KIND_C3S1 && th == 4));
@@ -757,6 +857,10 @@
             e = hipFuncSetAttribute((const void*)pick_pr(9, mode, 4, gs), hipFuncAttributeMaxDynamicSharedMemorySize, (int)PrLdsT<4>::TOTAL);
             if (e != hipSuccess) return e;
         }
+    for (const PrGeomRow& r : pr_geom_rows()) {
+        e = hipFuncSetAttribute((const void*)r.fn, hipFuncAttributeMaxDynamicSharedMemorySize, r.th == 4 ? (int)PrLdsT<4>::TOTAL : (int)PrLds::TOTAL);
+        if (e != hipSuccess) return e;
+    }
     int dev = 0;
     e = hipGetDevice(&dev);
     if (e != hipSuccess) return e;
@@ -813,7 +917,9 @@
         d.stamps = g_stamps;
     } else d.stamps = nullptr;
     if (a.gs_part && !(c3 && ks == 1)) return hipErrorInvalidValue;
-    hipLaunchKernelGGL(pick_pr(a.ntaps, a.res ? 1 : (ks == 2 ? 2 : 0), a.th, a.gs_part ? 1 : (a.gn_ab ? 0 : 2)), dim3((unsigned)grid), dim3(512),
+    const int mode = a.res ? 1 : (ks == 2 ? 2 : 0), gs = a.gs_part ? 1 : (a.gn_ab ? 0 : 2);
+    const PrGeomRow* const geom = d.stamps || d.dbg ? nullptr : pr_geom_match(a, mode, gs, a.film != nullptr);
+    hipLaunchKernelGGL(geom ? geom->fn : pick_pr(a.ntaps, mode, a.th, gs), dim3((unsigned)grid), dim3(512),
                        a.th == 4 ? PrLdsT<4>::TOTAL : PrLds::TOTAL, s, d, ntiles);
     return hipGetLastError();
 }
diff --git a/clip-neural-image-conpression_amd/csrc/ccn_internal.h b/clip-neural-image-conpression_amd/csrc/ccn_internal.h
--- a/clip-neural-image-conpression_amd/csrc/ccn_internal.h
+++ b/clip-neural-image-conpression_amd/csrc/ccn_internal.h
@@ -136,6 +136,8 @@
 
 bool conv_pr_supported(int kind, int bn, int th);
 bool conv_pr_selected(int dtype, int kind, int bn, int th);
+bool conv_pr_geom_enabled();
+const char* conv_pr_geom_name(const ConvArgs& a, bool res, bool film, int gs);
 hipError_t conv_pr_prepare();
 hipError_t launch_conv_pr(int dtype, const ConvArgs& a, hipStream_t s);
 
diff --git a/clip-neural-image-conpression_amd/csrc/ccn_kernels.hip b/clip-neural-image-conpression_amd/csrc/ccn_kernels.hip
--- a/clip-neural-image-conpression_amd/csrc/ccn_kernels.hip
+++ b/clip-neural-image-conpression_amd/csrc/ccn_kernels.hip
@@ -367,8 +367,9 @@
 
 bool conv_pr_selected(int dtype, int kind, int bn, int th)
 {
-    return dtype == 1 && conv_ws_enabled() && conv_variant() == 4 && conv_pr_supported(kind, bn, th);
-}
+    return dtype == 1 && conv_ws_enabled() && (conv_variant() == 4 || conv_variant() == 5) && conv_pr_supported(kind, bn, th);
+}
+bool conv_pr_geom_enabled() { return conv_variant() == 4; }
 
 ConvGeom conv_geom(int kind, bool four, int Hin, int Win, int th)
 {
```

Measured after the change: 84.66 images/sec (median of 6 runs). +3.1%, better.
